# viswavi/speech-anonymization

Measured on AMD Instinct MI355X. Metric: audio frames/sec (node), ConvAE+gender-adv train step, higher is better.
Workload: dtype bf16x3; 1 GPU; ConvAE recon0.1+sex0.9 adversarial train step (L1 recon + NLL), shape M: 32 utt/GPU x 161120 samples (T=1008 frames), Fbank x2 + norm + fwd + bwd + clip + Adam + Noam; batch_per_gpu=32, frames_per_utt=1008, parallelism=dp1

## Files before the change

include/sa_hip.h:

```cpp
#ifndef SA_HIP_H
#define SA_HIP_H
#ifdef __cplusplus
extern "C" {
#endif

#define SA_F32 0
#define SA_BF16 1
#define SA_BF16X3 2
#define SA_BF16X1F 3
#define SA_FP8 4
#define SA_F64 5
#define SA_MAX_TAPS 5
#define SA_COMM_ID_BYTES 128

typedef struct SaTaps {
  int ntaps[2];
  int off[2][SA_MAX_TAPS];
  int widx[2][SA_MAX_TAPS];
} SaTaps;

typedef struct SaConvArgs {
  const void* x;
  const void* wp;
  const float* bias;
  void* y;
  const float* s1; const float* t1;
  const float* s2; const float* t2;
  int swish;
  int relu;
  float* stats;
  int B, Lin, Lout, ntiles;
  int rowmin, nrows, wlo_off;
  SaTaps taps;
  int ep_mode, ep_xp_is_act, ep_bstride;
  const void* ep_x; const void* ep_g2;
  const float* ep_s1; const float* ep_t1; const float* ep_mean; const float* ep_rstd;
  void* a_out;
  const void* nb_x; const float* nb_c1; const float* nb_c2; const float* nb_c3;
  int nb_bstride, nb_relu_mask; float* nb_colsum;
  const float* ep_g2k1; const float* ep_g2k2; const float* ep_g2k3;
  float* pro_stats;
  const float* wscale;
  int tile_rows; int pad2_;
} SaConvArgs;

int sa_conv_gemm(int dtype, int cin, int cout, int sa, int u, const SaConvArgs* a, void* stream);
int sa_abi_sizeof(int which);
int sa_conv_gemm_ntiles(int cin, int cout, int u, int Lout);
int sa_conv_gemm_ntiles_tm(int tile_rows, int u, int Lout);
int sa_conv_gemm_set_tile_rows(int rows);
int sa_conv_gemm_set_impl(int impl);
int sa_conv_gemm_route(int dtype, int cin, int cout, int sa, int u, const SaConvArgs* a);

int sa_pack_weights(int dtype, const float* src, void* dst, int ntaps, int K, int N, int sk, int sn,
                    int st, void* stream);

typedef struct SaPackDesc {
  const float* src; void* dst;
  int dtype, ntaps, K, N, sk, sn, st, pad_;
  float* scale;
} SaPackDesc;
int sa_pack_weights_multi(const SaPackDesc* descs, int n, int blocks_per_image, void* stream);
int sa_pack_scales_multi(const SaPackDesc* descs, int n, void* stream);

typedef struct SaWgradArgs {
  const void* x;
  const void* dy;
  float* slabs;
  const float* s1; const float* t1; const float* s2; const float* t2; int swish;
  int B, Lin, Ldy, Mrows, chunk, nchunk;
  int ntaps; int off[SA_MAX_TAPS]; int ph[SA_MAX_TAPS];
  int x_pre;
  int dy_pre;
} SaWgradArgs;

int sa_wgrad(int dtype, int cin, int cout, int sa, int u, const SaWgradArgs* a, void* stream);
int sa_wgrad_kw(int cin, int cout);
int sa_wgrad_reduce(const float* slabs, float* dst, int nslab, int ntaps, int cin, int cout, int sk,
                    int sn, int st, int accumulate, void* stream);
#define SA_WRED_MAX 8
typedef struct SaWredDesc {
  const float* slabs; float* dst;
  int nslab, ntaps, cin, cout, sk, sn, st, accumulate, vec, pad_;
} SaWredDesc;
typedef struct SaWredMulti { int n, pad_; SaWredDesc d[SA_WRED_MAX]; } SaWredMulti;
int sa_wgrad_reduce_multi(const SaWredMulti* m, void* stream);

int sa_conv1toC(int dtype, const float* x, const float* w, const float* bias, void* y, int B, int L,
                int flip, float* stats, const void* ep_x, const float* ep_s1, const float* ep_t1,
                const float* ep_mean, const float* ep_rstd, void* stream);
int sa_conv1toC_ntiles(int L);
int sa_convCto1(int dtype, const void* x, const float* w, const float* bias, float* y, int B, int L,
                const float* s1, const float* t1, int swish, int flip, void* stream);
int sa_wgrad1C(int dtype, const float* u, const void* v, float* slabs, int B, int L, int chunk,
               int flip, const float* s1, const float* t1, int swish, void* stream);
int sa_wgrad1C_nchunk(int L, int chunk);
int sa_bwd1C(int dtype, const float* u, const void* v, const float* w, void* g, float* stats, float* slabs,
             int B, int L, int chunk, int flip, const float* s1, const float* t1, const float* mean,
             const float* rstd, void* stream);
int sa_sum_slabs(const float* slabs, float* dst, int nslab, int n, int accumulate, void* stream);

typedef struct SaEwArgs {
  const void* g; const void* g2; const void* x; void* out;
  const float* s1; const float* t1;
  const float* mean; const float* rstd;
  const float* c1; const float* c2; const float* c3;
  int actbwd, xp_is_act, relu_mask, bstride;
  float* stats;
  int B, L, ntiles;
} SaEwArgs;

int sa_ew_stats(int dtype, int C, const SaEwArgs* a, void* stream);
int sa_ew_apply(int dtype, int C, const SaEwArgs* a, void* stream);
int sa_ew_ntiles(int L);
int sa_sum_partials(const float* slabs, double* dst, int nbatch, int nslab, int n, void* stream);
int sa_sum_rows_d(const double* src, double* dst, int R, int n, void* stream);
int sa_fin_in_fwd(const double* sums, int B, int C, int n, const float* gamma, const float* beta,
                  float eps, float* mean, float* rstd, float* scale, float* shift, void* stream);
int sa_fin_bn_fwd(const double* sums, int R, int C, double count, const float* gamma, const float* beta,
                  float eps, float momentum, float* run_mean, float* run_var, float* mean,
                  float* rstd, float* scale, float* shift, const double* count_dev, void* stream);
int sa_fin_bn_eval(int C, const float* gamma, const float* beta, float eps, const float* run_mean,
                   const float* run_var, float* mean, float* rstd, float* scale, float* shift,
                   void* stream);
int sa_fin_norm_bwd(const double* sums, const double* lsums, int R, int groups, int C, double n,
                    const float* gamma, const float* mean, const float* rstd, float sign, float* c1,
                    float* c2, float* c3, float* dgamma, float* dbeta, const double* n_dev,
                    void* stream);
int sa_fin_bias(const double* sums, int B, int C, int ncomp, float* db, void* stream);

#define SA_FLATS_MAX 4
typedef struct SaFlat { float* p; long long n; } SaFlat;
typedef struct SaFlats { int n, pad_; SaFlat f[SA_FLATS_MAX]; } SaFlats;
int sa_clip_grads(const SaFlats* f, float max_norm, float eps, double* partials, float* total_norm, void* stream);
#define SA_ADAM_CHUNK 1024
typedef struct SaAdamRec {
  float* p; float* m; float* v; const float* step; const float* g;
  long long goff, n;
  int gbase, pad_;
} SaAdamRec;
int sa_adam_record_bytes(void);
int sa_adam_step(const SaAdamRec* table, int ntensors, const int* map, int nblocks, const SaFlats* bases,
                 const float* lr_dev, double lr, double beta1, double beta2, double eps, void* stream);
#define SA_BIAS_MAX 8
typedef struct SaBiasDesc {
  const float* part; double* rows; float* db;
  int nbatch, nslab, C, ncomp;
} SaBiasDesc;
typedef struct SaBiasMulti { int n, pad_; SaBiasDesc d[SA_BIAS_MAX]; } SaBiasMulti;
int sa_bias_multi(const SaBiasMulti* m, void* stream);

int sa_pool_fwd(int dtype, const void* r, const float* scale, const float* shift, float* part, int B,
                int L, int nseg, void* stream);
int sa_pool_nseg(int B);
int sa_pool_gather(const float* part, int B, int nseg, int L, double* sums, void* stream);
int sa_pool_fin(const double* sums, int B, int n, const float* noise, float eps, float* pooled,
                float* mean, float* stdraw, void* stream);
int sa_pool_gather_fin(const float* part, int B, int nseg, int L, const float* noise, int raw, float eps,
                       float* pooled, float* mean, float* stdraw, void* stream);
int sa_pool_bwd(int dtype, const void* r, const float* scale, const float* shift,
                const float* dpooled, const float* mean, const float* stdraw, void* g, int B, int L,
                const float* bn_mean, const float* bn_rstd, float* stats, void* stream);
int sa_dense(const float* X, int lda, const float* ps, const float* pt, const float* W, int sbk,
             int sbn, const float* bias, float* Y, int ldy, int M, int N, int K, int relu,
             void* stream);
int sa_colsums(const float* X, const float* H, const float* hmean, const float* hrstd, int M, int N,
               double* sums, float* out0, float* out1, void* stream);
int sa_bn2d_bwd(const float* G, const float* H, const double* sums, double count, const float* gamma,
                const float* mean, const float* rstd, int relu_mask, int M, int N, float* dH,
                const double* count_dev, void* stream);
int sa_dense_wgrad(const float* dY, const float* X, const float* ps, const float* pt, int M, int N,
                   int K, float* dW, void* stream);
int sa_log_softmax(const float* X, float* Y, int M, int N, void* stream);
int sa_log_softmax_bwd(const float* dY, const float* Y, float* dX, int M, int N, void* stream);
int sa_loss_workspace_bytes(void);
int sa_recon_loss(const float* a, const float* b, long long n, int kind, float* grad, float* loss,
                  void* workspace, void* stream);
int sa_cls_losses(const float* logp, const long long* label, int B, int NC, float* out, float* dnll,
                  float* dconf, void* stream);
int sa_cosine_loss(const float* x1, const float* x2, int B, int S, int D, float* rowloss,
                   float* loss, float* dx1, void* stream);
int sa_recon_loss_part(const float* a, const float* b, long long n, int kind, float* grad, float gscale,
                       void* workspace, void* stream);
int sa_step_loss(const void* workspace, long long n, const float* logp, const long long* label, int B, int NC,
                 float w_recon, float w_sex, float* out, float* dlogp, int* nonfinite, void* stream);

int sa_head_fwd(const float* pooled, const float* w1, const float* b1, const float* g1, const float* be1,
                float* rm1, float* rv1, const float* w2, const float* b2, const float* g2, const float* be2,
                float* rm2, float* rv2, const float* w3, const float* b3, float* h1, float* f1, float* h2,
                float* f2, float* logp, int M, float eps, float momentum, void* stream);
int sa_head_bwd(const float* dlogp, const float* logp, const float* pooled, const float* h1, const float* f1,
                const float* h2, const float* f2, const float* w1, const float* g1, const float* w2,
                const float* g2, const float* w3, float* dw1, float* db1, float* dg1, float* dbe1, float* dw2,
                float* db2, float* dg2, float* dbe2, float* dw3, float* db3, float* dpooled, int M, void* stream);
int sa_head_bwd_wide(const float* dlogp, const float* logp, const float* pooled, const float* h1, const float* f1,
                     const float* h2, const float* f2, const float* w1, const float* g1, const float* w2,
                     const float* g2, const float* w3, float* dw1, float* db1, float* dg1, float* dbe1, float* dw2,
                     float* db2, float* dg2, float* dbe2, float* dw3, float* db3, float* dpooled, int M,
                     void* stream);
int sa_head_max_rows(void);

int sa_tdnn_fwd(const float* x, const void* wp, const float* bias, const float* bn_s, const float* bn_t,
                float* y, int B, int T, int Cin, int Cout, int Npad, int K, int dil, float slope,
                unsigned char* mask, void* stream);
int sa_time_pool(const float* x, const float* lens, const float* noise, int B, int T, int C, float eps,
                 float* out, void* stream);
int sa_leaky_affine(const float* x, const float* s, const float* t, float slope, int M, int C, float* y,
                    void* stream);
int sa_tdnn_bwd_input(const float* dy, const unsigned char* mask, const float* bn_s, const void* wp,
                      float* dxe, int B, int T, int Cy, int Cred, int Cin, int Npad, int K, int dil,
                      float slope, void* stream);
int sa_tdnn_fold(const float* dxe, float* dx, int B, int T, int C, int pad, void* stream);
int sa_time_pool_bwd(const float* x, const float* lens, const float* g, const float* pooled, int B,
                     int T, int C, float eps, float* dx, void* stream);
int sa_leaky_affine_bwd(const float* dy, const float* x, const float* s, float slope, int M, int C,
                        float* dx, void* stream);

int sa_xv_tdnn_fwd_train(const float* x, const float* s_in, const float* t_in, const void* wp, const float* bias,
                         float* z, float* part, int B, int T, int Cin, int Cout, int Npad, int K, int dil,
                         float slope, void* stream);
int sa_xv_tdnn_ntiles(int T);
int sa_xv_colsums(const float* G, const float* H, const float* hmean, const float* hrstd, const float* c1,
                  const float* c2, const float* c3, float slope, float* out, int M, int N, int rows_per,
                  double* part, void* stream);
int sa_xv_tdnn_wgrad(const float* dpre, const float* x, const float* s_in, const float* t_in, float* part, int B,
                     int T, int Cin, int Cout, int K, int dil, int nsplit, int rows_per, void* stream);
int sa_xv_wgrad_reduce(const float* part, int nsplit, int K, int Cout, int Cin, float* dW, void* stream);
int sa_xv_tdnn_dgrad(const float* dpre, const void* wp, float* dxe, int B, int T, int Cy, int Cred, int Cin,
                     int Npad, int K, int dil, void* stream);
int sa_xv_pool_affine(const float* pz, const float* s, const float* t, const float* noise, int B, int C,
                      float eps, float* pooled, void* stream);
int sa_xv_pool_affine_bwd(const float* g, const float* s, int B, int C, float* gz, void* stream);

int sa_fc_tiles(int T);
int sa_fc_groups(int B, int T);
int sa_fc_nparam(void);
int sa_fc_nhead(void);
int sa_fc_max_rows(void);
int sa_fc_enc_fwd(const float* feats, const void* const* wb, float* h1, float* h2, float* z, double* bnpart,
                  int B, int T, void* stream);
int sa_fc_bn_fin(const double* bnpart, int npart, const float* gamma, const float* beta, float* run_mean,
                 float* run_var, float* bnf, int B, int T, int train, float eps, float momentum, void* stream);
int sa_fc_mid_fwd(const float* z, const float* bnf, const void* const* wb, float* a1, float* u, float* d1,
                  float* d2, float* recon, double* poolpart, int B, int T, void* stream);
int sa_fc_recon_fwd(const float* feats, const void* const* wb, float* recon, int B, int T, void* stream);
int sa_fc_head_fwd(const double* poolpart, const float* noise, const void* const* hw, float* pooled, float* pst,
                   float* h1, float* f1, float* h2, float* h3, float* f2, float* logp, int B, int T, int train,
                   float eps, float momentum, void* stream);
int sa_fc_head_bwd(const float* dlogp, const float* logp, const float* pooled, const float* h1,
                   const float* h2, const float* h3, const void* const* hw, float* dhead,
                   float* dpooled, int B, int train, float eps, void* stream);
int sa_fc_mid_bwd(const float* d_recon, const float* dpooled, const float* pst, const float* z, const float* bnf,
                  const float* a1, const float* u, const float* d1, const float* d2, const void* const* wb,
                  float* dzn, float* dzdec, float* wpart, double* bnbpart, int B, int T, void* stream);
int sa_fc_bn_bwd_fin(const double* bnbpart, int npart, const float* gamma, const float* bnf, float* coef,
                     float* dgamma, float* dbeta, int B, int T, int train, void* stream);
int sa_fc_enc_bwd(const float* feats, const float* h1, const float* h2, const float* z, const float* dzn,
                  const float* dzdec, const float* coef, const void* const* wb, float* wpart, int B, int T,
                  void* stream);
int sa_fc_wreduce(const float* wpart, int G, float* grads, void* stream);

int sa_cluster_mi(const float* X, const long long* y, const long long* idx, int iters, int n, int D,
                  int ncls, int k, float* mi, void* stream);

int sa_fbank(const float* wav, int B, int N, const float* window, const void* dft,
             const void* mel, float* feats, float* tilemax, void* stream);
int sa_fbank_table_elems(int which);
int sa_fbank_ntiles(int T);
int sa_fbank_scratch_bytes(int B);
int sa_fbank_normalize(const float* feats, const float* tilemax, int B, int T, int Tp,
                       const float* lens, float top_db, int batch_max, int update, int epoch,
                       int update_until_epoch, float* state, float* scratch, float* out,
                       void* stream);
int sa_fbank_normalize_pair(const float* feats, const float* tilemax, int B, int T, int Tp,
                            const float* lens, float top_db, int batch_max, int update, int epoch,
                            int update_until_epoch, float* state, float* scratch, float* snap,
                            float* out1, float* out2, void* stream);

int sa_wav_augment_tile(void);
int sa_wav_augment_max_chunks(void);
int sa_wav_abs_sums(const float* wav, const float* noise, int B, int L, double* sums, void* stream);
int sa_noise_scales(const double* sums, const float* lens, const float* snr, int B, int L, float* scales,
                    void* stream);
int sa_wav_augment(const float* wav, const float* noise, const float* scales, const void* plan, int B, int L, int R,
                   int Lp, int S_in, int S_out, int W, int first_min, int first_max, float* out, void* stream);

int sa_specaug_warp_sums(const float* x, const void* plan, int B, int T, int F, float* out, double* part,
                         void* stream);
int sa_specaug_finalize(const double* part, const void* plan, int B, int T, int F, float* vals, void* stream);
int sa_specaug_fill(const void* plan, const float* vals, int B, int T, int F, float* out, void* stream);

int sa_gl_tile(void);
int sa_mel_to_mag(const float* x, const float* mean, const float* stdv, const float* M, int B, int T, int Tf,
                  float* S, void* stream);
int sa_gl_istft(const void* C, const float* window, const float* twiddle, int B, int T, float* y, void* stream);
int sa_gl_project(const float* y, const float* S, const void* Tprev, float momentum_ratio, const float* window,
                  const float* twiddle, int B, int T, void* C_new, void* R, void* stream);

int sa_yin_dim(int which);
int sa_yin_f0(const float* wav, int B, int N, float threshold, float* f0, float* dprime, void* stream);
int sa_pitch_ratio(const float* f0, const float* lens, int B, int T, int N, float target, float r_min, float r_max,
                   int min_voiced, float* ratio, float* mean, int* voiced, void* stream);
int sa_pitch_stretch_mag(const void* R, const float* ratio, int B, int T, int Tout, float* S, void* stream);
int sa_pitch_resample(const float* y, const float* ratio, const int* n_valid, int B, int Nin, int Nout, float* out,
                      void* stream);

int sa_env_dim(int which);
int sa_env_warp(const float* S, const float* q, int B, int T, int n_c, float floor_rel, float max_gain_ln,
                float* out, float* env, void* stream);

int sa_mcadams_dim(int which);
int sa_mcadams(const float* wav, const float* alpha, const int* n_valid, int B, int N, int level, float* out,
               void* ws, int* status, float* gain, void* stream);

int sa_stoi_dim(int which);
int sa_stoi(const float* ref, const float* deg, const int* n_valid, int B, int N, const double* taps,
            float* stoi, float* estoi, int* frames, int* segments, void* ws, void* stream);

int sa_pv_dim(int which);
long long sa_pv_workspace_bytes(int B, int Tout);
int sa_pv_synth(const void* R, const float* S, const float* ratio, int B, int T, int Tout, void* C, double* phase,
                void* ws, void* stream);

int sa_contour_dim(int which);
int sa_pitch_contour(const float* f0, const float* lens, int B, int T, int N, float target, float gamma, int smooth,
                     float r_min, float r_max, int min_voiced, int* rho_q, long long* Q, int* Tq, float* mean,
                     int* voiced, void* stream);
int sa_pv_synth_map(const void* R, const float* M, const int* rho_q, const long long* Q, int B, int T, int Tout,
                    void* C, double* phase, void* ws, void* stream);
int sa_env_warp_frames(const float* S, const float* q, int B, int T, int n_c, float floor_rel, float max_gain_ln,
                       float* out, float* env, void* stream);
int sa_pitch_resample_map(const float* y, const int* rho_q, const long long* Q, const int* n_valid, int B, int Nin,
                          int Nout, int T, float* out, void* stream);

int sa_f0v_dim(int which);
int sa_f0_candidates(const float* dprime, int B, int T, int* cand_tau, int* cand_q, void* stream);
int sa_f0_viterbi(const float* dprime, const int* cand_tau, const int* cand_q, const float* lens, const int* log_q,
                  int B, int T, int N, float voicing_cost, float switch_cost, float jump_cost, float lag_bias,
                  unsigned char* psi, int* path, float* f0, void* stream);

int sa_f0cmp_dim(int which);
int sa_f0_compare(const float* f0_ref, const float* f0_deg, const int* frames, int B, int T, int max_lag,
                  int min_common, float* rho, int* lag, int* common, float* shift_st, float* dev_st, float* voicing,
                  void* stream);

int sa_mcd_dim(int which);
int sa_mcd(const float* mel_ref, const float* mel_deg, const int* n_ref, const int* n_deg, int B, int T_ref, int T_deg,
           int n_mels, int order, int band, void* ws, float* mcd, float* mcd_sync, int* frames, void* stream);

int sa_psola_dim(int which);
long long sa_psola_workspace_bytes(int B, int N);
int sa_psola_marks(const float* wav, const float* f0, const int* n_valid, int B, int N, int T, int* marks, int* count,
                   void* stream);
int sa_psola_plan(const int* marks, const int* count, const float* f0, const int* rho_q, const int* n_valid, int B,
                  int N, int T, void* ws, int* syn_pos, int* syn_src, int* syn_count, void* stream);
int sa_psola_ola(const float* wav, const int* marks, const int* count, const int* syn_pos, const int* syn_src,
                 const int* syn_count, const int* n_valid, int B, int N, float* out, void* stream);

int sa_formant_dim(int which);
int sa_formant_tracks(const float* wav, const int* n_valid, int B, int N, float* freq, float* bw, int* status,
                      void* stream);
int sa_formant_compare(const float* F_ref, const float* F_deg, const int* st_ref, const int* st_deg,
                       const float* f0_ref, const float* f0_deg, const int* frames, int B, int T, int min_common,
                       float* med, float* ratio, float* shift, int* common, void* stream);

int sa_pole_warp_dim(int which);
int sa_pole_warp(const float* wav, const float* q, const int* n_valid, int B, int N, int level, float* out, void* ws,
                 int* status, float* gain, void* stream);
int sa_formant_centre(const float* freq, const int* status, const float* f0, const int* frames, int B, int T, float t1,
                      float t2, float t3, float q_min, float q_max, int min_frames, float* med, float* q, int* count,
                      void* stream);

int sa_srcfilt_dim(int which);
long long sa_srcfilt_workspace_bytes(int B, int N);
int sa_srcfilt_pulses(const float* f0, const int* rho_q, const int* n_valid, int B, int N, int T, long long* pos_q,
                      int* period_q, int* count, void* stream);
int sa_srcfilt_excite(const float* f0, const long long* pos_q, const int* period_q, const int* count, const int* seed,
                      const int* n_valid, int B, int N, int T, float aspiration, float* exc, void* stream);
int sa_srcfilt_synth(const float* wav, const float* exc, const int* n_valid, int B, int N, int level, float* out,
                     void* ws, int* status, float* gain, void* stream);

int sa_add_layernorm_fwd(const void* x, const void* r, const void* gamma, const void* beta, void* y, void* s_out,
                         float* stat, int rows, int d, float eps, void* stream);
int sa_layernorm_bwd(const void* dy, const void* s, const float* stat, const void* gamma, void* ds, int rows,
                     int d, void* stream);
int sa_ln_leaky_fwd(const void* x, const void* gamma, const void* beta, void* y, float* stat, int rows, int d,
                    float eps, float slope, void* stream);
int sa_ln_leaky_bwd(const void* dy, const void* x, const float* stat, const void* gamma, const void* beta, void* dx,
                    int rows, int d, float slope, void* stream);
int sa_asr_block0_fwd(const void* x, const void* w, const void* bias, const void* gamma, const void* beta, void* y,
                      float* stat, int B, int T, int F, int C, float eps, float slope, void* stream);
int sa_asr_block0_bwd(const void* dy, const void* x, const void* w, const void* bias, const void* gamma,
                      const void* beta, const float* stat, float* part, void* dx, int B, int T, int F, int C,
                      float slope, void* stream);
int sa_reflect_pad_fwd(const void* x, void* y, int B, int T, int F, int C, void* stream);
int sa_reflect_pad_bwd(const void* dy, void* dx, int B, int T, int F, int C, void* stream);

int sa_comm_unique_id(void* id128);
int sa_comm_init(int rank, int world, const void* id128, int device);
int sa_comm_world(void);
int sa_comm_allreduce(void* buf, long long n, int dtype, int avg, void* producer_stream);
int sa_comm_allreduce_inline(void* buf, long long n, int dtype, int avg, void* stream);
int sa_comm_join(void* consumer_stream);
int sa_comm_ncalls(void);
int sa_comm_destroy(void);

#ifdef __cplusplus
}
#endif
#endif
```

speech-anonymization_amd/_lib.py:

```python
import ctypes as C
import os

import torch

_HERE = os.path.dirname(os.path.abspath(__file__))
LIB_PATH = os.environ.get("SA_HIP_LIB") or os.path.join(_HERE, "libsa_hip.so")

F32, BF16, BF16X3, BF16X1F, FP8, F64 = 0, 1, 2, 3, 4, 5
MAX_TAPS = 5

c_fp = C.POINTER(C.c_float)
vp = C.c_void_p


class SaTaps(C.Structure):
    _fields_ = [("ntaps", C.c_int * 2), ("off", (C.c_int * MAX_TAPS) * 2),
                ("widx", (C.c_int * MAX_TAPS) * 2)]


class SaConvArgs(C.Structure):
    _fields_ = [("x", vp), ("wp", vp), ("bias", vp), ("y", vp),
                ("s1", vp), ("t1", vp), ("s2", vp), ("t2", vp),
                ("swish", C.c_int), ("relu", C.c_int), ("stats", vp),
                ("B", C.c_int), ("Lin", C.c_int), ("Lout", C.c_int), ("ntiles", C.c_int),
                ("rowmin", C.c_int), ("nrows", C.c_int), ("wlo_off", C.c_int), ("taps", SaTaps),
                ("ep_mode", C.c_int), ("ep_xp_is_act", C.c_int), ("ep_bstride", C.c_int),
                ("ep_x", vp), ("ep_g2", vp), ("ep_s1", vp), ("ep_t1", vp), ("ep_mean", vp), ("ep_rstd", vp),
                ("a_out", vp),
                ("nb_x", vp), ("nb_c1", vp), ("nb_c2", vp), ("nb_c3", vp),
                ("nb_bstride", C.c_int), ("nb_relu_mask", C.c_int), ("nb_colsum", vp),
                ("ep_g2k1", vp), ("ep_g2k2", vp), ("ep_g2k3", vp), ("pro_stats", vp), ("wscale", vp),
                ("tile_rows", C.c_int), ("pad2_", C.c_int)]


class SaPackDesc(C.Structure):
    _fields_ = [("src", vp), ("dst", vp), ("dtype", C.c_int), ("ntaps", C.c_int), ("K", C.c_int),
                ("N", C.c_int), ("sk", C.c_int), ("sn", C.c_int), ("st", C.c_int), ("pad_", C.c_int),
                ("scale", vp)]


class SaWgradArgs(C.Structure):
    _fields_ = [("x", vp), ("dy", vp), ("slabs", vp),
                ("s1", vp), ("t1", vp), ("s2", vp), ("t2", vp), ("swish", C.c_int),
                ("B", C.c_int), ("Lin", C.c_int), ("Ldy", C.c_int), ("Mrows", C.c_int),
                ("chunk", C.c_int), ("nchunk", C.c_int),
                ("ntaps", C.c_int), ("off", C.c_int * MAX_TAPS), ("ph", C.c_int * MAX_TAPS),
                ("x_pre", C.c_int), ("dy_pre", C.c_int)]


class SaEwArgs(C.Structure):
    _fields_ = [("g", vp), ("g2", vp), ("x", vp), ("out", vp),
                ("s1", vp), ("t1", vp), ("mean", vp), ("rstd", vp),
                ("c1", vp), ("c2", vp), ("c3", vp),
                ("actbwd", C.c_int), ("xp_is_act", C.c_int), ("relu_mask", C.c_int),
                ("bstride", C.c_int), ("stats", vp),
                ("B", C.c_int), ("L", C.c_int), ("ntiles", C.c_int)]


BIAS_MAX = 8


class SaBiasDesc(C.Structure):
    _fields_ = [("part", vp), ("rows", vp), ("db", vp),
                ("nbatch", C.c_int), ("nslab", C.c_int), ("C", C.c_int), ("ncomp", C.c_int)]


class SaBiasMulti(C.Structure):
    _fields_ = [("n", C.c_int), ("pad_", C.c_int), ("d", SaBiasDesc * BIAS_MAX)]


WRED_MAX = 8
FLATS_MAX = 4


class SaFlat(C.Structure):
    _fields_ = [("p", vp), ("n", C.c_longlong)]


class SaFlats(C.Structure):
    _fields_ = [("n", C.c_int), ("pad_", C.c_int), ("f", SaFlat * FLATS_MAX)]



class SaAdamRec(C.Structure):
    _fields_ = [("p", vp), ("m", vp), ("v", vp), ("step", vp), ("g", vp),
                ("goff", C.c_longlong), ("n", C.c_longlong), ("gbase", C.c_int), ("pad_", C.c_int)]


ADAM_CHUNK = 1024


class SaWredDesc(C.Structure):
    _fields_ = [("slabs", vp), ("dst", vp)] + [(k, C.c_int) for k in ("nslab", "ntaps", "cin", "cout", "sk", "sn", "st",
                                                                      "accumulate", "vec", "pad_")]


class SaWredMulti(C.Structure):
    _fields_ = [("n", C.c_int), ("pad_", C.c_int), ("d", SaWredDesc * WRED_MAX)]


SYMBOLS = [
    "sa_conv_gemm", "sa_abi_sizeof", "sa_conv_gemm_ntiles", "sa_conv_gemm_ntiles_tm", "sa_conv_gemm_set_tile_rows",
    "sa_conv_gemm_set_impl", "sa_conv_gemm_route", "sa_pack_weights", "sa_pack_weights_multi", "sa_pack_scales_multi", "sa_wgrad", "sa_wgrad_kw", "sa_wgrad_reduce",
    "sa_conv1toC", "sa_conv1toC_ntiles", "sa_convCto1", "sa_wgrad1C", "sa_wgrad1C_nchunk", "sa_bwd1C",
    "sa_sum_slabs", "sa_ew_stats", "sa_ew_apply", "sa_ew_ntiles",
    "sa_sum_partials", "sa_sum_rows_d", "sa_fin_in_fwd", "sa_fin_bn_fwd", "sa_fin_bn_eval", "sa_fin_norm_bwd", "sa_fin_bias",
    "sa_pool_fwd", "sa_pool_nseg", "sa_pool_gather", "sa_pool_fin", "sa_pool_gather_fin", "sa_pool_bwd", "sa_dense", "sa_colsums",
    "sa_bn2d_bwd", "sa_dense_wgrad", "sa_log_softmax", "sa_log_softmax_bwd",
    "sa_loss_workspace_bytes", "sa_recon_loss", "sa_cls_losses", "sa_cosine_loss", "sa_recon_loss_part", "sa_step_loss",
    "sa_tdnn_fwd", "sa_time_pool", "sa_leaky_affine", "sa_tdnn_bwd_input", "sa_tdnn_fold", "sa_time_pool_bwd",
    "sa_leaky_affine_bwd", "sa_cluster_mi", "sa_fbank", "sa_fbank_table_elems", "sa_fbank_ntiles", "sa_fbank_scratch_bytes", "sa_fbank_normalize", "sa_fbank_normalize_pair",
    "sa_comm_unique_id", "sa_comm_init", "sa_comm_world", "sa_comm_allreduce", "sa_comm_allreduce_inline", "sa_comm_join", "sa_comm_ncalls",
    "sa_comm_destroy", "sa_head_fwd", "sa_head_bwd", "sa_head_bwd_wide", "sa_head_max_rows",
    "sa_add_layernorm_fwd", "sa_layernorm_bwd", "sa_reflect_pad_fwd", "sa_reflect_pad_bwd", "sa_ln_leaky_fwd", "sa_ln_leaky_bwd", "sa_bias_multi", "sa_asr_block0_fwd", "sa_asr_block0_bwd", "sa_wgrad_reduce_multi", "sa_clip_grads",
    "sa_adam_record_bytes", "sa_adam_step",
    "sa_xv_tdnn_fwd_train", "sa_xv_tdnn_ntiles", "sa_xv_colsums", "sa_xv_tdnn_wgrad", "sa_xv_wgrad_reduce",
    "sa_xv_tdnn_dgrad", "sa_xv_pool_affine", "sa_xv_pool_affine_bwd",
    "sa_fc_tiles", "sa_fc_groups", "sa_fc_nparam", "sa_fc_nhead", "sa_fc_max_rows", "sa_fc_enc_fwd", "sa_fc_bn_fin",
    "sa_fc_mid_fwd", "sa_fc_head_fwd", "sa_fc_head_bwd", "sa_fc_mid_bwd", "sa_fc_bn_bwd_fin", "sa_fc_enc_bwd",
    "sa_fc_wreduce", "sa_fc_recon_fwd",
    "sa_wav_augment_tile", "sa_wav_augment_max_chunks", "sa_wav_abs_sums", "sa_noise_scales", "sa_wav_augment",
    "sa_specaug_warp_sums", "sa_specaug_finalize", "sa_specaug_fill",
    "sa_gl_tile", "sa_mel_to_mag", "sa_gl_istft", "sa_gl_project",
    "sa_yin_dim", "sa_yin_f0", "sa_pitch_ratio", "sa_pitch_stretch_mag", "sa_pitch_resample",
    "sa_env_dim", "sa_env_warp",
    "sa_mcadams_dim", "sa_mcadams",
    "sa_stoi_dim", "sa_stoi",
    "sa_pv_dim", "sa_pv_synth",
    "sa_contour_dim", "sa_pitch_contour", "sa_pv_synth_map", "sa_env_warp_frames", "sa_pitch_resample_map",
    "sa_f0v_dim", "sa_f0_candidates", "sa_f0_viterbi",
    "sa_f0cmp_dim", "sa_f0_compare",
    "sa_mcd_dim", "sa_mcd",
    "sa_psola_dim", "sa_psola_marks", "sa_psola_plan", "sa_psola_ola",
    "sa_formant_dim", "sa_formant_tracks", "sa_formant_compare",
    "sa_pole_warp_dim", "sa_pole_warp", "sa_formant_centre",
    "sa_srcfilt_dim", "sa_srcfilt_pulses", "sa_srcfilt_excite", "sa_srcfilt_synth",
]

_lib = None


class SaHipError(RuntimeError):
    pass


def load():
    global _lib
    if _lib is None:
        if not os.path.exists(LIB_PATH):
            raise SaHipError(
                f"{LIB_PATH} not found: build it with `python -c 'import __graft_entry__ as g; "
                "g.build()'` (hipcc --offload-arch=gfx950). There is no CPU fallback.")
        _lib = C.CDLL(LIB_PATH)
        for s in SYMBOLS:
            getattr(_lib, s).restype = C.c_int
        _lib.sa_pv_workspace_bytes.restype = C.c_longlong
        _lib.sa_psola_workspace_bytes.restype = C.c_longlong
        _lib.sa_srcfilt_workspace_bytes.restype = C.c_longlong
        for i, rec in enumerate((SaConvArgs, SaWgradArgs, SaEwArgs, SaPackDesc, SaTaps, SaBiasMulti, SaWredMulti, SaFlats)):
            if _lib.sa_abi_sizeof(i) != C.sizeof(rec):
                raise SaHipError(f"{rec.__name__}: binding has {C.sizeof(rec)} bytes, {LIB_PATH} "
                                 f"{_lib.sa_abi_sizeof(i)} -- rebuild the library (stale build?)")
        if _lib.sa_adam_record_bytes() != C.sizeof(SaAdamRec):
            raise SaHipError(f"SaAdamRec: binding has {C.sizeof(SaAdamRec)} bytes, {LIB_PATH} "
                             f"{_lib.sa_adam_record_bytes()} -- rebuild the library (stale build?)")
    return _lib


def stream():
    return C.c_void_p(torch._C._cuda_getCurrentRawStream(torch._C._cuda_getDevice()))


def ptr(t):
    if t is None:
        return None
    assert t.is_cuda and t.is_contiguous(), "HIP kernels take contiguous device tensors"
    return C.c_void_p(t.data_ptr())


def check(rc, what):
    if rc != 0:
        raise SaHipError(f"{what} failed with code {rc}")


def dt_code(dtype):
    if dtype == torch.float32:
        return F32
    if dtype == torch.bfloat16:
        return BF16
    raise SaHipError(f"unsupported activation dtype {dtype}")


_taps_cache = {}


def make_taps(phases):
    key = tuple(tuple(p) for p in phases)
    t = _taps_cache.get(key)
    if t is not None:
        return t
    t = _taps_cache[key] = SaTaps()
    for ph, lst in enumerate(phases):
        t.ntaps[ph] = len(lst)
        for i, (off, wi) in enumerate(lst):
            t.off[ph][i] = off
            t.widx[ph][i] = wi
    return t
```

speech-anonymization_amd/convae.py:

```python
import functools
import os

import torch
import torch.nn as nn

from . import distributed as sdist
from . import ops
from . import _lib as L
from ._lib import SaHipError


class _ParamOnly(nn.Module):

    def forward(self, x):
        raise SaHipError("parameter container only; use ConvAutoencoder.forward")


class GLU(_ParamOnly):
    pass


class StatisticsPooling(_ParamOnly):
    pass


class TDNNSexClassifier(nn.Module):
    def __init__(self, num_classes=2):
        super().__init__()
        self.tdnn = nn.Sequential(
            nn.Conv1d(128, 128, kernel_size=5, dilation=1), nn.ReLU(), nn.BatchNorm1d(128),
            nn.Conv1d(128, 128, kernel_size=3, dilation=2), nn.ReLU(), nn.BatchNorm1d(128),
            nn.Conv1d(128, 128, kernel_size=3, dilation=3), nn.ReLU(), nn.BatchNorm1d(128),
        )
        self.norm = nn.BatchNorm1d(128)
        self.stats_pooling = StatisticsPooling()
        self.classify = nn.Sequential(
            nn.Linear(256, 128), nn.ReLU(), nn.BatchNorm1d(128),
            nn.Linear(128, 64), nn.ReLU(), nn.BatchNorm1d(64),
            nn.Linear(64, num_classes),
        )

    def forward(self, x):
        raise SaHipError("parameter container only; use ConvAutoencoder.forward")


class ConvAutoencoder(nn.Module):
    def __init__(self, precision="bf16x3", pooling_noise=True, sync_bn=True, dtype=None,
                 cache_wgrad_operand=True):
        super().__init__()
        if dtype is not None:
            precision = {torch.float32: "f32", torch.bfloat16: "bf16"}[dtype]
        if precision not in ops.PRECISIONS:
            raise SaHipError(f"unknown precision {precision!r}")
        self.precision = precision
        self.encoder = nn.Sequential(
            nn.Conv1d(1, 32, 15, 1, 7), GLU(),
            nn.Conv1d(32, 64, 5, 2, 2), nn.InstanceNorm1d(64, affine=True), GLU(),
            nn.Conv1d(64, 64, 5, 1, 2), nn.InstanceNorm1d(64, affine=True), GLU(),
            nn.Conv1d(64, 128, 5, 2, 2), nn.InstanceNorm1d(128, affine=True), GLU(),
            nn.Conv1d(128, 128, 5, 1, 2), nn.InstanceNorm1d(128, affine=True), GLU(),
        )
        self.decoder = nn.Sequential(
            nn.Conv1d(128, 128, 5, 1, 2),
            nn.ConvTranspose1d(128, 64, 5, 2, 2, output_padding=1),
            nn.InstanceNorm1d(64, affine=True), GLU(),
            nn.Conv1d(64, 64, 5, 1, 2),
            nn.ConvTranspose1d(64, 32, 5, 2, 2, output_padding=1),
            nn.InstanceNorm1d(32, affine=True), GLU(),
            nn.Conv1d(32, 1, 15, 1, 7),
        )
        self.sex_classifier = TDNNSexClassifier(2)
        self.lay = ops.conv_layers(self, ("encoder", "sex_classifier.tdnn", "decoder"))
        self.pack_plan = [(ly.key, ly.kinds[i]) for i in (0, 1)
                          for ly in sorted(self.lay.values(), key=lambda ly: ly.transposed)]
        self.act_dtype, self.kcode = ops.PRECISIONS[precision]
        self.dgrad_kcode = ops.DGRAD_CODE[precision]
        self.cache_wgrad_operand = cache_wgrad_operand
        self.pooling_noise = pooling_noise
        self.sync_bn = sync_bn
        self.fused_head = os.environ.get("SA_FUSED_HEAD", "1") == "1"
        self.fused_bwd1c = os.environ.get("SA_FUSED_BWD1C", "1") == "1"
        self.fused_pool_fin = os.environ.get("SA_FUSED_POOL_FIN", "1") == "1"
        self.wide_head_bwd = os.environ.get("SA_WIDE_HEAD_BWD", "1") == "1"
        self.dp_batch_sizes = None

    def forward(self, feats):
        names, params = self._named_params()
        return _ConvAEFn.apply(self, names, feats, *params)

    def _named_params(self):
        c = self.__dict__.get("_np_cache")
        if c is None or any(o[n] is not p for o, n, p in c[2]):
            names, params, owners = [], [], []
            for mname, mod in self.named_modules():
                for pname, p in mod._parameters.items():
                    if p is not None:
                        names.append(f"{mname}.{pname}" if mname else pname)
                        params.append(p)
                        owners.append((mod._parameters, pname, p))
            c = self.__dict__["_np_cache"] = (tuple(names), tuple(params), owners)
        return c[0], c[1]

    @torch.no_grad()
    def reconstruct(self, feats):
        if not torch.is_tensor(feats) or feats.dim() != 3:
            raise SaHipError("ConvAutoencoder expects feats [B, T, 80]")
        x0, B, T, Ltot = _input_rows(feats)
        P = dict(zip(*self._named_params()))
        cg, inorm = _launchers(self, P, _packed(self, P), B)
        y, _, _ = _encoder_launches(self, P, cg, inorm, x0, Ltot, False)
        return _decoder_launches(self, P, cg, inorm, y[5], Ltot)[-1].view(B, T, 80)

    def _side_stream(self, device):
        if getattr(self, "_side", None) is None and device.type == "cuda":
            self._side = torch.cuda.Stream(device=device)
        return getattr(self, "_side", None)

    def _bn_syncs(self):
        return self.sync_bn and sdist.dp_active()

    def _bn_allreduce(self, sums):
        if self._bn_syncs():
            sdist.all_reduce_now(sums)
            return sdist.world_size()
        return 1

    def _bn_global_counts(self, counts, device):
        if not self._bn_syncs():
            return None
        key = (tuple(counts), str(device))
        cache = self.__dict__.setdefault("_count_cache", {})
        local = cache.get(key)
        if local is None:
            if len(cache) > 64:
                cache.clear()
            local = cache[key] = torch.tensor(counts, dtype=torch.float64).to(device)
        g = local.clone()
        sdist.all_reduce_now(g)
        return g

    def _bn_rows(self):
        return not self._bn_syncs()

    def _bn_global(self, local_sums):
        if not self._bn_syncs():
            return local_sums, 1
        g = local_sums.clone()
        return g, self._bn_allreduce(g)

    def _head_plan(self, B):
        if not self._bn_syncs() or self.dp_batch_sizes is None:
            return None
        W, r = sdist.world_size(), sdist.rank()
        sizes = [B] * W if isinstance(self.dp_batch_sizes, str) else [int(b) for b in self.dp_batch_sizes]
        if self.dp_batch_sizes != "equal" and isinstance(self.dp_batch_sizes, str):
            raise SaHipError(f"dp_batch_sizes: 'equal', a list of per-rank batch sizes or None, not {self.dp_batch_sizes!r}")
        if len(sizes) != W or sizes[r] != B:
            raise SaHipError(f"dp_batch_sizes {sizes} does not describe rank {r} of {W} holding {B} utterances")
        return sum(sizes[:r]), sum(sizes), W

    @staticmethod
    def _gather_rows(x, plan):
        off, Bg, _ = plan
        g = torch.zeros(Bg, x.shape[1], device=x.device, dtype=x.dtype)
        g[off:off + x.shape[0]].copy_(x)
        sdist.all_reduce_now(g)
        return g


class _W:
    __slots__ = ("img", "code")

    def __init__(self, img, code):
        self.img, self.code = img, code


def _kcode(model, kind):
    return model.dgrad_kcode if kind.endswith("dgrad") else model.kcode


def _packed(model, P):
    items = [((k, kind), P[k], kind, _kcode(model, kind)) for k, kind in model.pack_plan]
    key = tuple(w.data_ptr() for _, w, _, _ in items) + tuple(c for _, _, _, c in items)
    pk = getattr(model, "_pack_cache", None)
    if pk is None or pk[0] != key:
        pk = (key, ops.PackedWeights(items, model.act_dtype))
        model._pack_cache = pk
    pk[1].refresh()
    return {tag: _W(img, code) for tag, (img, code) in pk[1].images.items()}


def _conv(x, w, *args, **kw):
    return ops.conv_gemm(x, w.img, *args, code=w.code, **kw)


class _PendingApply:
    __slots__ = ("g", "y", "c", "per_c", "relu", "bias_key", "wgrads")

    def __init__(self, g, y, c, per_c, relu, bias_key):
        self.g, self.y, self.c, self.per_c, self.relu, self.bias_key = g, y, c, per_c, relu, bias_key
        self.wgrads = []


def _noise(model, B, device):
    return ops.pooling_noise(model.pooling_noise, B, 128, device)


def _input_rows(feats):
    B, T, Fd = feats.shape
    Ltot = T * Fd
    if Fd != 80 or Ltot % 4:
        raise SaHipError("ConvAutoencoder expects feats [B, T, 80] with T*80 divisible by 4")
    if not feats.is_cuda:
        raise SaHipError("ConvAutoencoder runs on the GPU only (no CPU fallback)")
    return feats.detach().reshape(B, Ltot).contiguous().float(), B, T, Ltot


def _in_ep(y, nrm, g2=None):
    mean, rstd, scale, shift = nrm
    d = dict(mode=1, x=y, g2=g2, s1=scale, t1=shift, mean=mean, rstd=rstd)
    if isinstance(g2, _PendingApply):
        d.update(g2=g2.g, g2k=g2.c)
    return d


def _launchers(model, P, W, B, A=None):
    def cg(ly, x, **kw):
        if A is not None and P[ly.key].requires_grad:
            A[ly.key] = kw["a_out"] = torch.empty(x.shape, dtype=torch.bfloat16, device=x.device)
        return _conv(x, W[ly.key, ly.kinds[0]], P[ly.bias], *ly.fwd(x.shape[1]), **kw)

    def inorm(stats, n, prefix, C):
        sums = ops.sum_partials(stats, B)
        return ops.fin_in_fwd(sums, B, C, n, P[prefix + ".weight"], P[prefix + ".bias"])
    return cg, inorm


def _encoder_launches(model, P, cg, inorm, x0, Ltot, want_pro_stats):
    L2, L4, lay = Ltot // 2, Ltot // 4, model.lay
    y0 = ops.conv1toC(x0, P["encoder.0.weight"], P["encoder.0.bias"], model.act_dtype)
    y1, st = cg(lay["encoder.2"], y0, swish=True, want_stats=True)
    n1 = inorm(st, L2, "encoder.3", 64)
    y2, st = cg(lay["encoder.5"], y1, s1=n1[2], t1=n1[3], swish=True, want_stats=True)
    n2 = inorm(st, L2, "encoder.6", 64)
    y3, st = cg(lay["encoder.8"], y2, s1=n2[2], t1=n2[3], swish=True, want_stats=True)
    n3 = inorm(st, L4, "encoder.9", 128)
    y4, st = cg(lay["encoder.11"], y3, s1=n3[2], t1=n3[3], swish=True, want_stats=True)
    n4 = inorm(st, L4, "encoder.12", 128)
    y5 = cg(lay["decoder.0"], y4, s1=n4[2], t1=n4[3], swish=True, want_pro_stats=want_pro_stats)
    a4_stats = None
    if want_pro_stats:
        y5, a4_stats = y5
    return [y0, y1, y2, y3, y4, y5], [n1, n2, n3, n4], a4_stats


def _decoder_launches(model, P, cg, inorm, y5, Ltot):
    L2, lay = Ltot // 2, model.lay
    y6, st = cg(lay["decoder.1"], y5, want_stats=True)
    n6 = inorm(st, L2, "decoder.2", 64)
    y7 = cg(lay["decoder.4"], y6, s1=n6[2], t1=n6[3], swish=True)
    y8, st = cg(lay["decoder.5"], y7, want_stats=True)
    n8 = inorm(st, Ltot, "decoder.6", 32)
    recon = ops.convCto1(y8, P["decoder.8.weight"], P["decoder.8.bias"], n8[2], n8[3], True)
    return y6, n6, y7, y8, n8, recon


class _ConvAEFn(torch.autograd.Function):
    @staticmethod
    def forward(ctx, model, names, feats, *params):
        ctx.set_materialize_grads(False)
        P = dict(zip(names, params))
        train = model.training
        x0, B, T, Ltot = _input_rows(feats)
        L2, L4 = Ltot // 2, Ltot // 4
        S = {}
        W, lay = _packed(model, P), model.lay
        A = {}
        cache_a = (train and model.cache_wgrad_operand and any(ctx.needs_input_grad)
                   and ops.WGRAD_CODE[model.precision] in (L.BF16X1F, L.BF16) and model.kcode != L.FP8)

        cg, inorm = _launchers(model, P, W, B, A if cache_a else None)

        def bn_stats(stats, count, mod, prefix, C, ci):
            sums = ops.sum_partials(stats, 1, rows=model._bn_rows()) if train else None
            return bnorm(sums, count, mod, prefix, C, ci)

        def bnorm(sums, count, mod, prefix, C, ci, local=False):
            if not train:
                return ops.fin_bn_eval(C, P[prefix + ".weight"], P[prefix + ".bias"],
                                       mod.running_mean, mod.running_var)
            if not local:
                model._bn_allreduce(sums)
            out = ops.fin_bn_fwd(sums, C, count, P[prefix + ".weight"], P[prefix + ".bias"],
                                 mod.running_mean, mod.running_var, count_dev=None if local else cdev(ci))
            tracked.append(mod.num_batches_tracked)
            return out

        tracked = []
        enc, dec, cls = model.encoder, model.decoder, model.sex_classifier
        La, Lb, Lc = L4 - 4, L4 - 8, L4 - 14
        gc = model._bn_global_counts([B * L4, B * La, B * Lb, B * Lc, B, B], feats.device) if train else None
        cdev = lambda i: None if gc is None else gc[i:i + 1]
        (y0, y1, y2, y3, y4, y5), (n1, n2, n3, n4), a4_stats = _encoder_launches(model, P, cg, inorm, x0, Ltot, train)
        bn_n = bn_stats(a4_stats if train else None, B * L4, cls.norm, "sex_classifier.norm", 128, 0)
        r0, st = cg(lay["sex_classifier.tdnn.0"], y4, s1=n4[2], t1=n4[3], swish=True, s2=bn_n[2], t2=bn_n[3],
                    relu=True, want_stats=True)
        bn0 = bn_stats(st, B * La, cls.tdnn[2], "sex_classifier.tdnn.2", 128, 1)
        r1, st = cg(lay["sex_classifier.tdnn.3"], r0, s2=bn0[2], t2=bn0[3], relu=True, want_stats=True)
        bn1 = bn_stats(st, B * Lb, cls.tdnn[5], "sex_classifier.tdnn.5", 128, 2)
        r2, st = cg(lay["sex_classifier.tdnn.6"], r1, s2=bn1[2], t2=bn1[3], relu=True, want_stats=True)
        bn2 = bn_stats(st, B * Lc, cls.tdnn[8], "sex_classifier.tdnn.8", 128, 3)
        if model.fused_pool_fin:
            nz, raw = ops.pooling_noise_raw(model.pooling_noise, B, 128, feats.device)
            pooled, pmean, psd = ops.pool_fwd(r2, bn2[2], bn2[3], noise=nz, fused=True, raw=raw)
        else:
            pooled, pmean, psd = ops.pool_fwd(r2, bn2[2], bn2[3], noise=_noise(model, B, feats.device))
        def head_fwd(X, n, local=False):
            H1 = ops.dense(X, P["sex_classifier.classify.0.weight"], P["sex_classifier.classify.0.bias"],
                           128, 256, relu=True)
            f1 = bnorm(ops.colsums(H1) if train else None, n, cls.classify[2], "sex_classifier.classify.2", 128, 4, local)
            H2 = ops.dense(H1, P["sex_classifier.classify.3.weight"], P["sex_classifier.classify.3.bias"],
                           64, 128, ps=f1[2], pt=f1[3], relu=True)
            f2 = bnorm(ops.colsums(H2) if train else None, n, cls.classify[5], "sex_classifier.classify.5", 64, 5, local)
            logits = ops.dense(H2, P["sex_classifier.classify.6.weight"], P["sex_classifier.classify.6.bias"],
                               2, 64, ps=f2[2], pt=f2[3])
            return H1, f1, H2, f2, ops.log_softmax(logits)

        plan = model._head_plan(B) if train else None
        head_in, Bh = (model._gather_rows(pooled, plan), plan[1]) if plan else (pooled, B)
        fused_head = (train and model.fused_head and (plan is not None or not model._bn_syncs())
                      and Bh <= ops.head_max_rows())
        clsP = {k[len("sex_classifier.classify."):]: v for k, v in P.items() if k.startswith("sex_classifier.classify.")}
        if fused_head:
            H1, f1, H2, f2, logp = ops.head_fwd(head_in, clsP, cls.classify[2], cls.classify[5])
            tracked += [cls.classify[2].num_batches_tracked, cls.classify[5].num_batches_tracked]
        else:
            H1, f1, H2, f2, logp = head_fwd(head_in, Bh, plan is not None)
        logp_all = logp
        if plan:
            logp = logp_all[plan[0]:plan[0] + B]
        if tracked:
            torch._foreach_add_(tracked, 1)
        y6, n6, y7, y8, n8, recon = _decoder_launches(model, P, cg, inorm, y5, Ltot)

        S.update(x0=x0, y=[y0, y1, y2, y3, y4, y5, y6, y7, y8], r=[r0, r1, r2],
                 n=[None, n1, n2, n3, n4, None, n6, None, n8], bn=[bn_n, bn0, bn1, bn2], f=[f1, f2],
                 pooled=head_in, pmean=pmean, psd=psd, H1=H1, H2=H2, logp=logp_all, head_plan=plan,
                 dims=(B, T, Ltot, L2, L4, La, Lb, Lc), train=train, W=W, A=A, gc=gc, fused_head=fused_head)
        ctx.S, ctx.model, ctx.names, ctx.params = S, model, names, params
        ctx.need_input_grad = feats.requires_grad
        return recon.view(B, T, 80), logp

    @staticmethod
    def backward(ctx, d_recon, d_logp):
        S, model, names = ctx.S, ctx.model, ctx.names
        if S is None:
            raise SaHipError("ConvAutoencoder backward called twice (saved tensors were released)")
        P = dict(zip(names, ctx.params))
        dt = model.act_dtype
        B, T, Ltot, L2, L4, La, Lb, Lc = S["dims"]
        if not S["train"]:
            raise SaHipError("backward through eval-mode BatchNorm is not implemented")
        y0, y1, y2, y3, y4, y5, y6, y7, y8 = S["y"]
        r0, r1, r2 = S["r"]
        n1, n2, n3, n4, n6, n8 = S["n"][1], S["n"][2], S["n"][3], S["n"][4], S["n"][6], S["n"][8]
        bn_n, bn0, bn1, bn2 = S["bn"]
        f1, f2 = S["f"]
        dev = y0.device
        G = {k: None for k in names}
        need = {k: p.requires_grad for k, p in P.items()}
        need_stage = {st: any(v for k, v in need.items() if k.startswith(st))
                      for st in sdist.StageBuckets.STAGES}
        run_encoder = need_stage["encoder"] or ctx.need_input_grad
        run_decoder = need_stage["decoder"] or run_encoder
        model._last_flats = None
        buckets = sdist.StageBuckets(list(P.items()), dev, model._side_stream(dev))
        newg = buckets.view

        def setg(key, val):
            G[key] = newg(key).copy_(val.reshape(P[key].shape))
        W, A, lay = S["W"], S["A"], model.lay
        gc = S["gc"]
        cdev = lambda i: None if gc is None else gc[i:i + 1]
        pending_wred = []
        wg = functools.partial(ops.wgrad, code=ops.WGRAD_CODE[model.precision], defer=pending_wred)
        fuse = bool(A) and model.dgrad_kcode in (L.BF16X3, L.BF16)

        def cg(ly, gin, **kw):
            p, dy = gin, gin.g if isinstance(gin, _PendingApply) else gin
            w, args = W[ly.key, ly.kinds[1]], (None,) + ly.dgrad(ly.lin(dy.shape[1]))
            if dy is gin:
                return _conv(dy, w, *args, **kw)
            dyc = torch.empty(p.g.shape, dtype=torch.bfloat16, device=p.g.device) if p.wgrads else None
            want_cs = p.bias_key is not None and need[p.bias_key]
            out = _conv(p.g, w, *args, a_out=dyc, nb=dict(x=p.y, c1=p.c[0], c2=p.c[1], c3=p.c[2],
                                                           per_c=p.per_c, relu_mask=p.relu,
                                                           want_colsum=want_cs), **kw)
            if want_cs:
                cs = out[-1]
                out = out[:-1] if len(out) > 2 else out[0]
                nb_, _, cc_ = cs.shape
                G[p.bias_key] = newg(p.bias_key)
                pending_bias.append((cs, nb_, cc_, 1, G[p.bias_key]))
            for f in p.wgrads:
                f(dyc)
            p.wgrads = []
            return out

        def bias_from(stats, key, C):
            if need[key]:
                G[key] = newg(key)
                pending_bias.append((stats, B, C, 2, G[key]))

        pending_bias = []

        def flush_pending():
            if pending_bias:
                ops.bias_multi(pending_bias)
                pending_bias.clear()
            if pending_wred:
                ops.wgrad_reduce_multi(pending_wred)
                pending_wred.clear()

        def in_finish(g, st, y, nrm, C, Ln, prefix, bias_key):
            mean, rstd = nrm[0], nrm[1]
            dg, db = newg(prefix + ".weight"), newg(prefix + ".bias")
            sums = ops.sum_partials(st, B)
            c1, c2, c3 = ops.fin_norm_bwd(sums, sums, B * C, C, Ln, P[prefix + ".weight"], mean, rstd,
                                          dgamma=dg, dbeta=db)
            G[prefix + ".weight"], G[prefix + ".bias"] = dg, db
            if fuse:
                return _PendingApply(g, y, (c1, c2, c3), False, False, bias_key)
            st2 = ops.ew("apply", g, y, C, out=g, c1=c1, c2=c2, c3=c3)
            bias_from(st2, bias_key, C)
            return g

        def bn_ep(r, bn, xp=None):
            d = dict(mode=2, x=r, mean=bn[0], rstd=bn[1], per_c=True)
            if xp:
                d.update(s1=xp[0], t1=xp[1], xp_is_act=True)
            return d

        def bn_finish(g, st, r, bn, Ln, prefix, bias_key, ci, xp=None):
            mean, rstd = bn[0], bn[1]
            kw = dict(s1=xp[0], t1=xp[1], xp_is_act=True) if xp else {}
            dg, db = newg(prefix + ".weight"), newg(prefix + ".bias")
            lsums = ops.sum_partials(st, 1, rows=model._bn_rows())
            gsums, _ = model._bn_global(lsums)
            c1, c2, c3 = ops.fin_norm_bwd(gsums, lsums, 128, 128, float(B * Ln), P[prefix + ".weight"],
                                          mean, rstd, sign=-1.0 if xp else 1.0, dgamma=dg, dbeta=db,
                                          n_dev=cdev(ci))
            G[prefix + ".weight"], G[prefix + ".bias"] = dg, db
            if fuse:
                return _PendingApply(g, r, (c1, c2, c3), True, not xp, bias_key)
            st2 = ops.ew("apply", g, r, 128, out=g, c1=c1, c2=c2, c3=c3, relu_mask=not xp, per_c=True,
                         want_stats=bias_key is not None, **kw)
            if bias_key:
                bias_from(st2, bias_key, 128)
            return g

        def conv_wgrad(ly, x, dy, **pro):
            key = ly.key
            if not need[key]:
                return
            if isinstance(dy, _PendingApply):
                dy.wgrads.append(lambda dyc: conv_wgrad(ly, x, dyc, dy_pre=True))
                return
            if key in A:
                x, pro = A[key], dict(x_pre=True, dy_pre=bool(pro.get("dy_pre")))
            *geo, strides = ly.wgrad(x.shape[1])
            G[key] = wg(x, dy, *geo, newg(key), strides, **pro)

        recon_unused = d_recon is None
        if recon_unused:
            for k in need:
                if k.startswith("decoder"):
                    need[k] = False
            need_stage["decoder"] = False
        if d_logp is None:
            d_logp = torch.zeros(B, 2, device=dev)

        def finish(d_feats=None):
            flush_pending()
            buckets.join()
            ctx.S = None
            model._last_flats = [buckets.flat[st] for st in sdist.StageBuckets.STAGES if need_stage[st]]
            grads = tuple(G[k] if need[k] else None for k in names)
            G.clear()
            buckets.views.clear()
            return (None, None, d_feats) + grads

        def head_bwd():
            c = "sex_classifier.classify."
            plan = S.get("head_plan")
            dlp, Bh = d_logp.contiguous().float(), B
            if plan:
                dlp, Bh = model._gather_rows(dlp, plan), plan[1]
            dP = head_bwd_rows(c, dlp, Bh, plan is not None)
            if plan:
                hg = [G[k] for k in names if k.startswith(c) and k in G]
                if plan[2] > 1 and hg:
                    torch._foreach_mul_(hg, 1.0 / plan[2])
                dP = dP[plan[0]:plan[0] + B]
            return dP

        def head_bwd_rows(c, dlp, n, local):
            if S.get("fused_head"):
                short = ("0.weight", "0.bias", "2.weight", "2.bias", "3.weight", "3.bias", "5.weight", "5.bias",
                         "6.weight", "6.bias")
                views = {}
                for k in short:
                    if need[c + k]:
                        views[k] = G[c + k] = newg(c + k)
                clsP = {k: P[c + k] for k in short}
                return ops.head_bwd(dlp, S["logp"], S["pooled"], S["H1"], f1, S["H2"], f2, clsP, views,
                                    wide=model.wide_head_bwd)
            glob = (lambda l: l) if local else (lambda l: model._bn_global(l)[0])
            cd = (lambda i: None) if local else cdev
            dLG = ops.log_softmax_bwd(dlp, S["logp"])
            H1, H2 = S["H1"], S["H2"]
            G[c + "6.weight"] = ops.dense_wgrad(dLG, H2, newg(c + "6.weight"), ps=f2[2], pt=f2[3])
            G[c + "6.bias"] = newg(c + "6.bias"); ops.colsums(dLG, out0=G[c + "6.bias"])
            dN2 = ops.dense(dLG, P[c + "6.weight"], None, 64, 2, transpose_w=True)
            G[c + "5.weight"], G[c + "5.bias"] = newg(c + "5.weight"), newg(c + "5.bias")
            l2 = ops.colsums(dN2, H2, f2[0], f2[1], out0=G[c + "5.bias"], out1=G[c + "5.weight"])
            dH2 = ops.bn2d_bwd(dN2, H2, glob(l2), n, P[c + "5.weight"], f2[0], f2[1], True, count_dev=cd(5))
            G[c + "3.weight"] = ops.dense_wgrad(dH2, H1, newg(c + "3.weight"), ps=f1[2], pt=f1[3])
            G[c + "3.bias"] = newg(c + "3.bias"); ops.colsums(dH2, out0=G[c + "3.bias"])
            dN1 = ops.dense(dH2, P[c + "3.weight"], None, 128, 64, transpose_w=True)
            G[c + "2.weight"], G[c + "2.bias"] = newg(c + "2.weight"), newg(c + "2.bias")
            l1 = ops.colsums(dN1, H1, f1[0], f1[1], out0=G[c + "2.bias"], out1=G[c + "2.weight"])
            dH1 = ops.bn2d_bwd(dN1, H1, glob(l1), n, P[c + "2.weight"], f1[0], f1[1], True, count_dev=cd(4))
            G[c + "0.weight"] = ops.dense_wgrad(dH1, S["pooled"], newg(c + "0.weight"))
            G[c + "0.bias"] = newg(c + "0.bias"); ops.colsums(dH1, out0=G[c + "0.bias"])
            return ops.dense(dH1, P[c + "0.weight"], None, 256, 128, transpose_w=True)

        def tdnn_bwd(dP):
            t = "sex_classifier.tdnn."
            g, st = ops.pool_bwd(r2, bn2[2], bn2[3], dP, S["pmean"], S["psd"], bn=(bn2[0], bn2[1]))
            g = bn_finish(g, st, r2, bn2, Lc, t + "8", t + "6.bias", 3)
            conv_wgrad(lay[t + "6"], r1, g, s2=bn1[2], t2=bn1[3])
            g, st = cg(lay[t + "6"], g, want_stats=True, ep=bn_ep(r1, bn1))
            g = bn_finish(g, st, r1, bn1, Lb, t + "5", t + "3.bias", 2)
            conv_wgrad(lay[t + "3"], r0, g, s2=bn0[2], t2=bn0[3])
            g, st = cg(lay[t + "3"], g, want_stats=True, ep=bn_ep(r0, bn0))
            g = bn_finish(g, st, r0, bn0, La, t + "2", t + "0.bias", 1)
            conv_wgrad(lay[t + "0"], y4, g, s1=n4[2], t1=n4[3], swish=True, s2=bn_n[2], t2=bn_n[3])
            xp4 = (n4[2], n4[3])
            g, st = cg(lay[t + "0"], g, want_stats=True, ep=bn_ep(y4, bn_n, xp4))
            da = bn_finish(g, st, y4, bn_n, L4, "sex_classifier.norm", None, 0, xp=xp4)
            flush_pending()
            if need_stage["sex_classifier"]:
                buckets.reduce_stage("sex_classifier")
            return da

        def decoder_bwd():
            d_rec = torch.zeros(B, T, 80, device=dev) if recon_unused else d_recon
            g_rec = d_rec.reshape(B, Ltot).contiguous().float()
            if need["decoder.8.bias"]:
                setg("decoder.8.bias", ops.sum_partials(g_rec.view(4 * B, Ltot // 4), 1, n=Ltot // 4).sum())
            if need["decoder.8.weight"] and model.fused_bwd1c:
                g, st, G["decoder.8.weight"] = ops.bwd1C(g_rec, y8, P["decoder.8.weight"], newg("decoder.8.weight"),
                                                         n8[2], n8[3], n8[0], n8[1])
            else:
                if need["decoder.8.weight"]:
                    G["decoder.8.weight"] = ops.wgrad1C(g_rec, y8, newg("decoder.8.weight"), flip=True,
                                                        s1=n8[2], t1=n8[3], swish=True)
                g, st = ops.conv1toC(g_rec, P["decoder.8.weight"], None, dt, flip=True, want_stats=True,
                                     ep=dict(x=y8, s1=n8[2], t1=n8[3], mean=n8[0], rstd=n8[1]))
            g = in_finish(g, st, y8, n8, 32, Ltot, "decoder.6", "decoder.5.bias")
            conv_wgrad(lay["decoder.5"], y7, g)
            g, st = cg(lay["decoder.5"], g, want_stats=True)
            bias_from(st, "decoder.4.bias", 64)
            conv_wgrad(lay["decoder.4"], y6, g, s1=n6[2], t1=n6[3], swish=True)
            g, st = cg(lay["decoder.4"], g, want_stats=True, ep=_in_ep(y6, n6))
            g = in_finish(g, st, y6, n6, 64, L2, "decoder.2", "decoder.1.bias")
            conv_wgrad(lay["decoder.1"], y5, g)
            g, st = cg(lay["decoder.1"], g, want_stats=True)
            bias_from(st, "decoder.0.bias", 128)
            conv_wgrad(lay["decoder.0"], y4, g, s1=n4[2], t1=n4[3], swish=True)
            flush_pending()
            if need_stage["decoder"]:
                buckets.reduce_stage("decoder")
            return g

        da4_cls = tdnn_bwd(head_bwd())
        if not run_decoder:
            return finish()
        g = decoder_bwd()
        if not run_encoder:
            return finish()

        g, st = cg(lay["decoder.0"], g, want_stats=True, ep=_in_ep(y4, n4, g2=da4_cls))
        for conv, norm, y, nrm, x, nx in (("encoder.11", "encoder.12", y4, n4, y3, n3),
                                          ("encoder.8", "encoder.9", y3, n3, y2, n2),
                                          ("encoder.5", "encoder.6", y2, n2, y1, n1),
                                          ("encoder.2", "encoder.3", y1, n1, y0, None)):
            ly = lay[conv]
            g = in_finish(g, st, y, nrm, ly.cout, y.shape[1], norm, ly.bias)
            conv_wgrad(ly, x, g, swish=True, **(dict(s1=nx[2], t1=nx[3]) if nx else {}))
            g, st = cg(ly, g, want_stats=True, ep=_in_ep(x, nx) if nx else dict(mode=1, x=x))
        bias_from(st, "encoder.0.bias", 32)
        if need["encoder.0.weight"]:
            G["encoder.0.weight"] = ops.wgrad1C(S["x0"], g, newg("encoder.0.weight"))
        d_feats = None
        if ctx.need_input_grad:
            d_feats = ops.convCto1(g, P["encoder.0.weight"], None, flip=True).view(B, T, 80)
        flush_pending()
        if need_stage["encoder"]:
            buckets.reduce_stage("encoder")
        return finish(d_feats)
```

speech-anonymization_amd/csrc/sa_common.h:

```cpp
#pragma once
#include <hip/hip_runtime.h>
#include <stdint.h>
#include "../../include/sa_hip.h"

typedef __bf16 bf16_t;
typedef __bf16 bf16x8 __attribute__((ext_vector_type(8)));
typedef float f32x16 __attribute__((ext_vector_type(16)));
typedef float f32x4 __attribute__((ext_vector_type(4)));

#define SA_WAVE 64


template <typename T> struct Tr;

template <> struct Tr<float> {
  static constexpr int VEC = 4;
  static constexpr int KS = 2;
  typedef float Frag;
  __device__ static inline void unpack(const uint4& u, float* f) {
    f[0] = __uint_as_float(u.x); f[1] = __uint_as_float(u.y);
    f[2] = __uint_as_float(u.z); f[3] = __uint_as_float(u.w);
  }
  __device__ static inline uint4 pack(const float* f) {
    return make_uint4(__float_as_uint(f[0]), __float_as_uint(f[1]),
                      __float_as_uint(f[2]), __float_as_uint(f[3]));
  }
  __device__ static inline float to_f(float v) { return v; }
  __device__ static inline float from_f(float v) { return v; }
  __device__ static inline f32x16 mfma(Frag a, Frag b, f32x16 c) {
    return __builtin_amdgcn_mfma_f32_32x32x2f32(a, b, c, 0, 0, 0);
  }
};

__device__ static inline uint32_t sa_pack_bf16x2(float lo, float hi) {
  union { bf16_t b[2]; uint32_t u; } cv;
  cv.b[0] = (bf16_t)lo; cv.b[1] = (bf16_t)hi;
  return cv.u;
}

template <> struct Tr<bf16_t> {
  static constexpr int VEC = 8;
  static constexpr int KS = 16;
  typedef bf16x8 Frag;
  __device__ static inline void unpack(const uint4& u, float* f) {
    f[0] = __uint_as_float(u.x << 16); f[1] = __uint_as_float(u.x & 0xffff0000u);
    f[2] = __uint_as_float(u.y << 16); f[3] = __uint_as_float(u.y & 0xffff0000u);
    f[4] = __uint_as_float(u.z << 16); f[5] = __uint_as_float(u.z & 0xffff0000u);
    f[6] = __uint_as_float(u.w << 16); f[7] = __uint_as_float(u.w & 0xffff0000u);
  }
  __device__ static inline uint4 pack(const float* f) {
    return make_uint4(sa_pack_bf16x2(f[0], f[1]), sa_pack_bf16x2(f[2], f[3]),
                      sa_pack_bf16x2(f[4], f[5]), sa_pack_bf16x2(f[6], f[7]));
  }
  __device__ static inline float to_f(bf16_t v) { return (float)v; }
  __device__ static inline bf16_t from_f(float v) { return (bf16_t)v; }
  __device__ static inline f32x16 mfma(Frag a, Frag b, f32x16 c) {
    return __builtin_amdgcn_mfma_f32_32x32x16_bf16(a, b, c, 0, 0, 0);
  }
};

__device__ static inline float sa_swish(float v) { return v * __builtin_amdgcn_rcpf(1.0f + __expf(-v)); }
__device__ static inline float sa_swish_grad(float v) {
  const float s = __builtin_amdgcn_rcpf(1.0f + __builtin_amdgcn_exp2f(v * -1.4426950408889634f));
  const float t = 1.0f - s;
  const float u = fmaf(v, t, 1.0f);
  return s * u;
}

__device__ static inline int sa_acc_row(int reg, int lane) {
  return (reg & 3) + 8 * (reg >> 2) + 4 * (lane >> 5);
}

__device__ static inline float sa_wave_sum(float v) {
#pragma unroll
  for (int o = 32; o > 0; o >>= 1) v += __shfl_xor(v, o, 64);
  return v;
}
__device__ static inline double sa_wave_sum_d(double v) {
#pragma unroll
  for (int o = 32; o > 0; o >>= 1) v += __shfl_xor(v, o, 64);
  return v;
}
__device__ static inline float sa_wave_max(float v) {
#pragma unroll
  for (int o = 32; o > 0; o >>= 1) v = fmaxf(v, __shfl_xor(v, o, 64));
  return v;
}

static inline int sa_div_up(int a, int b) { return (a + b - 1) / b; }

struct bf16x3_t {};
struct bf16x1f_t {};

struct fp8_t {};
typedef long fp8x8;

template <typename T> struct Pol;
template <> struct Pol<float> {
  typedef float store_t; typedef float lds_t; typedef float Frag;
  static constexpr int NPL = 1, VEC = 4, KS = 2, PAD = 1;
};
template <> struct Pol<bf16_t> {
  typedef bf16_t store_t; typedef bf16_t lds_t; typedef bf16x8 Frag;
  static constexpr int NPL = 1, VEC = 8, KS = 16, PAD = 8;
};
template <> struct Pol<bf16x1f_t> {
  typedef float store_t; typedef bf16_t lds_t; typedef bf16x8 Frag;
  static constexpr int NPL = 1, VEC = 4, KS = 16, PAD = 8;
};
template <> struct Pol<bf16x3_t> {
  typedef float store_t; typedef bf16_t lds_t; typedef bf16x8 Frag;
  static constexpr int NPL = 2, VEC = 4, KS = 16, PAD = 8;
};

template <> struct Pol<fp8_t> {
  typedef bf16_t store_t; typedef unsigned char lds_t; typedef fp8x8 Frag;
  static constexpr int NPL = 1, VEC = 8, KS = 16, PAD = 8;
};
template <> struct Tr<unsigned char> {
  __device__ static inline f32x16 mfma(fp8x8 a, fp8x8 b, f32x16 c) {
    return __builtin_amdgcn_mfma_f32_32x32x16_fp8_fp8(a, b, c, 0, 0, 0);
  }
};
__device__ static inline uint2 sa_pack_fp8x8(const float* f) {
  float c[8];
#pragma unroll
  for (int j = 0; j < 8; ++j) c[j] = __builtin_amdgcn_fmed3f(f[j], -448.0f, 448.0f);
  int lo = 0, hi = 0;
  lo = __builtin_amdgcn_cvt_pk_fp8_f32(c[0], c[1], lo, false);
  lo = __builtin_amdgcn_cvt_pk_fp8_f32(c[2], c[3], lo, true);
  hi = __builtin_amdgcn_cvt_pk_fp8_f32(c[4], c[5], hi, false);
  hi = __builtin_amdgcn_cvt_pk_fp8_f32(c[6], c[7], hi, true);
  return make_uint2((unsigned)lo, (unsigned)hi);
}

__device__ static inline uint2 sa_pack_bf16x4(const float* f) {
  return make_uint2(sa_pack_bf16x2(f[0], f[1]), sa_pack_bf16x2(f[2], f[3]));
}
__device__ static inline void sa_split4(const float* f, uint2& hi, uint2& lo) {
  float h[4], l[4];
#pragma unroll
  for (int j = 0; j < 4; ++j) {
    const bf16_t hb = (bf16_t)f[j];
    h[j] = (float)hb;
    l[j] = f[j] - h[j];
  }
  hi = sa_pack_bf16x4(h);
  lo = sa_pack_bf16x4(l);
}
```

speech-anonymization_amd/csrc/sa_elementwise.hip:

```cpp
#include "sa_common.h"


#define SA_EW_ROWS 256

template <typename T, int C, bool APPLY>
__global__ __launch_bounds__(256) void sa_ew_kernel(SaEwArgs a) {
  typedef Tr<T> tr;
  constexpr int VEC = tr::VEC, CH = C / VEC, RPP = 256 / CH;
  __shared__ float red[RPP][C][2];
  const int tid = threadIdx.x, b = blockIdx.y, tile = blockIdx.x;
  const int c = tid % CH, r0 = tid / CH;
  const size_t cb1 = (size_t)b * C + c * VEC;
  const size_t cbn = (size_t)b * a.bstride + c * VEC;
  float s1[VEC], t1[VEC], mu[VEC], rs[VEC], k1[VEC], k2[VEC], k3[VEC], acc0[VEC], acc1[VEC];
#pragma unroll
  for (int j = 0; j < VEC; ++j) {
    s1[j] = a.s1 ? a.s1[cb1 + j] : 1.0f;
    t1[j] = a.t1 ? a.t1[cb1 + j] : 0.0f;
    mu[j] = a.mean ? a.mean[cbn + j] : 0.0f;
    rs[j] = a.rstd ? a.rstd[cbn + j] : 1.0f;
    k1[j] = (APPLY && a.c1) ? a.c1[cbn + j] : 1.0f;
    k2[j] = (APPLY && a.c2) ? a.c2[cbn + j] : 0.0f;
    k3[j] = (APPLY && a.c3) ? a.c3[cbn + j] : 0.0f;
    acc0[j] = 0.0f; acc1[j] = 0.0f;
  }
  const size_t base = (size_t)b * a.L * C + c * VEC;
  const T* gp = reinterpret_cast<const T*>(a.g) + base;
  const T* g2p = a.g2 ? reinterpret_cast<const T*>(a.g2) + base : nullptr;
  const T* xp = reinterpret_cast<const T*>(a.x) + base;
  T* op = a.out ? reinterpret_cast<T*>(a.out) + base : nullptr;
  const int lbeg = tile * SA_EW_ROWS;
  for (int r = r0; r < SA_EW_ROWS; r += RPP) {
    const int l = lbeg + r;
    if (l >= a.L) break;
    float g[VEC], x[VEC], o[VEC];
    tr::unpack(*reinterpret_cast<const uint4*>(gp + (size_t)l * C), g);
    tr::unpack(*reinterpret_cast<const uint4*>(xp + (size_t)l * C), x);
    if (g2p) {
      float g2[VEC];
      tr::unpack(*reinterpret_cast<const uint4*>(g2p + (size_t)l * C), g2);
#pragma unroll
      for (int j = 0; j < VEC; ++j) g[j] += g2[j];
    }
#pragma unroll
    for (int j = 0; j < VEC; ++j) {
      const float z = fmaf(x[j], s1[j], t1[j]);
      const float xv = a.xp_is_act ? sa_swish(z) : x[j];
      if (APPLY) {
        float v = fmaf(k1[j], g[j], fmaf(k2[j], xv, k3[j]));
        if (a.relu_mask && !(x[j] > 0.0f)) v = 0.0f;
        o[j] = v;
      } else {
        o[j] = a.actbwd ? g[j] * sa_swish_grad(z) : g[j];
      }
    }
    uint4 u = tr::pack(o);
    if (op) *reinterpret_cast<uint4*>(op + (size_t)l * C) = u;
    if (a.stats) {
      tr::unpack(u, o);
#pragma unroll
      for (int j = 0; j < VEC; ++j) {
        acc0[j] += o[j];
        if (!APPLY) {
          const float z = fmaf(x[j], s1[j], t1[j]);
          const float xv = a.xp_is_act ? sa_swish(z) : x[j];
          acc1[j] = fmaf(o[j], (xv - mu[j]) * rs[j], acc1[j]);
        }
      }
    }
  }
  if (a.stats) {
#pragma unroll
    for (int j = 0; j < VEC; ++j) { red[r0][c * VEC + j][0] = acc0[j]; red[r0][c * VEC + j][1] = acc1[j]; }
    __syncthreads();
    if (tid < C) {
      float s = 0.f, q = 0.f;
      for (int r = 0; r < RPP; ++r) { s += red[r][tid][0]; q += red[r][tid][1]; }
      float* d = a.stats + (((size_t)b * a.ntiles + tile) * C + tid) * 2;
      d[0] = s; d[1] = q;
    }
  }
}

extern "C" int sa_ew_ntiles(int L) { return sa_div_up(L, SA_EW_ROWS); }

template <bool APPLY>
static int launch_ew(int dtype, int C, const SaEwArgs& a0, hipStream_t st) {
  SaEwArgs a = a0;
  a.ntiles = sa_div_up(a.L, SA_EW_ROWS);
  dim3 grid(a.ntiles, a.B);
#define SA_EW_CASE(CC)                                                                      \
  if (C == CC) {                                                                            \
    if (dtype == SA_BF16) hipLaunchKernelGGL((sa_ew_kernel<bf16_t, CC, APPLY>), grid, dim3(256), 0, st, a); \
    else hipLaunchKernelGGL((sa_ew_kernel<float, CC, APPLY>), grid, dim3(256), 0, st, a);   \
    hipError_t e = hipGetLastError();                                                       \
    return e == hipSuccess ? 0 : -(int)e;                                                   \
  }
  SA_EW_CASE(32) SA_EW_CASE(64) SA_EW_CASE(128)
  return -38;
}

extern "C" int sa_ew_stats(int dtype, int C, const SaEwArgs* a, void* stream) {
  if (!a || !a->g || !a->x || a->B <= 0 || a->L <= 0) return -22;
  return launch_ew<false>(dtype, C, *a, reinterpret_cast<hipStream_t>(stream));
}
extern "C" int sa_ew_apply(int dtype, int C, const SaEwArgs* a, void* stream) {
  if (!a || !a->g || !a->x || !a->out || a->B <= 0 || a->L <= 0) return -22;
  return launch_ew<true>(dtype, C, *a, reinterpret_cast<hipStream_t>(stream));
}

#define SA_SP_LANES 16
__global__ __launch_bounds__(32 * SA_SP_LANES) void sa_sum_partials_kernel(const float* __restrict__ slabs,
                                                                           double* __restrict__ dst,
                                                                           int nslab, int n) {
  __shared__ double part[SA_SP_LANES][33];
  const int bb = blockIdx.y, o = threadIdx.x & 31, q = threadIdx.x >> 5;
  const int i = blockIdx.x * 32 + o;
  double s = 0.0;
  if (i < n) {
    const float* p = slabs + (size_t)bb * nslab * n + i;
#pragma unroll 16
    for (int k = q; k < nslab; k += SA_SP_LANES) s += (double)p[(size_t)k * n];
  }
  part[q][o] = s;
  __syncthreads();
  if (q == 0 && i < n) {
    double t = 0.0;
#pragma unroll
    for (int r = 0; r < SA_SP_LANES; ++r) t += part[r][o];
    dst[(size_t)bb * n + i] = t;
  }
}

extern "C" int sa_sum_partials(const float* slabs, double* dst, int nbatch, int nslab, int n,
                               void* stream) {
  if (!slabs || !dst || nbatch <= 0 || nslab <= 0 || n <= 0) return -22;
  hipLaunchKernelGGL(sa_sum_partials_kernel, dim3(sa_div_up(n, 32), nbatch), dim3(32 * SA_SP_LANES), 0,
                     reinterpret_cast<hipStream_t>(stream), slabs, dst, nslab, n);
  hipError_t e = hipGetLastError();
  return e == hipSuccess ? 0 : -(int)e;
}

__global__ void sa_sum_rows_d_kernel(const double* __restrict__ src, double* __restrict__ dst, int R, int n) {
  const int i = blockIdx.x * blockDim.x + threadIdx.x;
  if (i >= n) return;
  double s = 0.0;
#pragma unroll 8
  for (int r = 0; r < R; ++r) s += src[(size_t)r * n + i];
  dst[i] = s;
}

extern "C" int sa_sum_rows_d(const double* src, double* dst, int R, int n, void* stream) {
  if (!src || !dst || R <= 0 || n <= 0) return -22;
  hipLaunchKernelGGL(sa_sum_rows_d_kernel, dim3(sa_div_up(n, 128)), dim3(128), 0,
                     reinterpret_cast<hipStream_t>(stream), src, dst, R, n);
  hipError_t e = hipGetLastError();
  return e == hipSuccess ? 0 : -(int)e;
}

__global__ void sa_fin_in_fwd_kernel(const double* __restrict__ sums, int BC, int C, float n,
                                     const float* __restrict__ gamma, const float* __restrict__ beta,
                                     float eps, float* mean, float* rstd, float* scale, float* shift) {
  const int i = blockIdx.x * blockDim.x + threadIdx.x;
  if (i >= BC) return;
  const double m = (double)sums[2 * i] / n;
  double var = (double)sums[2 * i + 1] / n - m * m;
  if (var < 0.0) var = 0.0;
  const float r = (float)(1.0 / sqrt(var + (double)eps));
  const float sc = gamma[i % C] * r;
  mean[i] = (float)m; rstd[i] = r; scale[i] = sc; shift[i] = beta[i % C] - (float)m * sc;
}

extern "C" int sa_fin_in_fwd(const double* sums, int B, int C, int n, const float* gamma,
                             const float* beta, float eps, float* mean, float* rstd, float* scale,
                             float* shift, void* stream) {
  if (!sums || !gamma || !beta || !mean || !rstd || !scale || !shift) return -22;
  hipLaunchKernelGGL(sa_fin_in_fwd_kernel, dim3(sa_div_up(B * C, 256)), dim3(256), 0,
                     reinterpret_cast<hipStream_t>(stream), sums, B * C, C, (float)n, gamma, beta,
                     eps, mean, rstd, scale, shift);
  hipError_t e = hipGetLastError();
  return e == hipSuccess ? 0 : -(int)e;
}

__global__ void sa_fin_bn_fwd_kernel(const double* __restrict__ sums, int R, int C, double count,
                                     const float* __restrict__ gamma, const float* __restrict__ beta,
                                     float eps, float momentum, float* run_mean, float* run_var,
                                     float* mean, float* rstd, float* scale, float* shift,
                                     const double* __restrict__ count_dev) {
  const int i = blockIdx.x * blockDim.x + threadIdx.x;
  if (i >= C) return;
  if (count_dev) count = *count_dev;
  double S = 0.0, Q = 0.0;
#pragma unroll 8
  for (int r = 0; r < R; ++r) { S += sums[2 * ((size_t)r * C + i)]; Q += sums[2 * ((size_t)r * C + i) + 1]; }
  const double m = S / count;
  double var = Q / count - m * m;
  if (var < 0.0) var = 0.0;
  const float r = (float)(1.0 / sqrt(var + (double)eps));
  const float sc = gamma[i] * r;
  mean[i] = (float)m; rstd[i] = r; scale[i] = sc; shift[i] = beta[i] - (float)m * sc;
  if (run_mean) {
    const double unb = count > 1.0 ? var * count / (count - 1.0) : var;
    run_mean[i] = (1.0f - momentum) * run_mean[i] + momentum * (float)m;
    run_var[i] = (1.0f - momentum) * run_var[i] + momentum * (float)unb;
  }
}

extern "C" int sa_fin_bn_fwd(const double* sums, int R, int C, double count, const float* gamma,
                             const float* beta, float eps, float momentum, float* run_mean,
                             float* run_var, float* mean, float* rstd, float* scale, float* shift,
                             const double* count_dev, void* stream) {
  if (!sums || !gamma || !beta || !mean || !rstd || !scale || !shift || (!count_dev && count <= 0) || R < 1) return -22;
  hipLaunchKernelGGL(sa_fin_bn_fwd_kernel, dim3(sa_div_up(C, 128)), dim3(128), 0,
                     reinterpret_cast<hipStream_t>(stream), sums, R, C, count, gamma, beta, eps,
                     momentum, run_mean, run_var, mean, rstd, scale, shift, count_dev);
  hipError_t e = hipGetLastError();
  return e == hipSuccess ? 0 : -(int)e;
}

__global__ void sa_fin_bn_eval_kernel(int C, const float* __restrict__ gamma, const float* __restrict__ beta,
                                      float eps, const float* __restrict__ rm, const float* __restrict__ rv,
                                      float* mean, float* rstd, float* scale, float* shift) {
  const int i = blockIdx.x * blockDim.x + threadIdx.x;
  if (i >= C) return;
  const float r = 1.0f / sqrtf(rv[i] + eps), sc = gamma[i] * r;
  mean[i] = rm[i]; rstd[i] = r; scale[i] = sc; shift[i] = beta[i] - rm[i] * sc;
}

extern "C" int sa_fin_bn_eval(int C, const float* gamma, const float* beta, float eps,
                              const float* run_mean, const float* run_var, float* mean, float* rstd,
                              float* scale, float* shift, void* stream) {
  if (!gamma || !beta || !run_mean || !run_var || !mean || !rstd || !scale || !shift) return -22;
  hipLaunchKernelGGL(sa_fin_bn_eval_kernel, dim3(sa_div_up(C, 128)), dim3(128), 0,
                     reinterpret_cast<hipStream_t>(stream), C, gamma, beta, eps, run_mean, run_var,
                     mean, rstd, scale, shift);
  hipError_t e = hipGetLastError();
  return e == hipSuccess ? 0 : -(int)e;
}

__global__ void sa_fin_norm_bwd_kernel(const double* __restrict__ sums, const double* __restrict__ lsums,
                                       int R, int G, int C, double n, const float* __restrict__ gamma,
                                       const float* __restrict__ mean, const float* __restrict__ rstd,
                                       float sign, float* c1, float* c2, float* c3, float* dgamma,
                                       float* dbeta, int nb, int coef_blocks,
                                       const double* __restrict__ n_dev) {
  if (n_dev) n = *n_dev;
  if ((int)blockIdx.x < coef_blocks) {
    const int i = blockIdx.x * blockDim.x + threadIdx.x;
    if (i < G) {
      double S1 = 0.0, S2 = 0.0;
#pragma unroll 8
      for (int r = 0; r < R; ++r) { S1 += sums[2 * ((size_t)r * G + i)]; S2 += sums[2 * ((size_t)r * G + i) + 1]; }
      const double r = rstd[i], m = mean[i];
      const double k1 = (double)gamma[i % C] * r;
      c1[i] = sign * (float)k1;
      c2[i] = sign * (float)(-k1 * r * S2 / n);
      c3[i] = sign * (float)(k1 * (-S1 / n + m * r * S2 / n));
    }
    return;
  }
  __shared__ double part[8][32][2];
  const int ch = ((int)blockIdx.x - coef_blocks) * 32 + (threadIdx.x & 31), q = threadIdx.x >> 5;
  double a = 0.0, bsum = 0.0;
  if (ch < C) {
    const int tot = R * nb;
#pragma unroll 4
    for (int e = q; e < tot; e += 8) {
      const int r = e / nb, b = e % nb;
      const size_t at = 2 * ((size_t)r * G + (size_t)b * C + ch);
      bsum += lsums[at]; a += lsums[at + 1];
    }
  }
  part[q][threadIdx.x & 31][0] = bsum; part[q][threadIdx.x & 31][1] = a;
  __syncthreads();
  if (q == 0 && ch < C) {
    double s0 = 0.0, s1 = 0.0;
#pragma unroll
    for (int k = 0; k < 8; ++k) { s0 += part[k][threadIdx.x][0]; s1 += part[k][threadIdx.x][1]; }
    dbeta[ch] = (float)s0; dgamma[ch] = (float)s1;
  }
}

extern "C" int sa_fin_norm_bwd(const double* sums, const double* lsums, int R, int groups, int C, double n,
                               const float* gamma, const float* mean, const float* rstd, float sign,
                               float* c1, float* c2, float* c3, float* dgamma, float* dbeta,
                               const double* n_dev, void* stream) {
  if (!sums || !gamma || !mean || !rstd || !c1 || !c2 || !c3 || groups % C || R < 1) return -22;
  if ((dgamma == nullptr) != (dbeta == nullptr)) return -22;
  const int coef_blocks = sa_div_up(groups, 256);
  const int grid = coef_blocks + (dgamma ? sa_div_up(C, 32) : 0);
  hipLaunchKernelGGL(sa_fin_norm_bwd_kernel, dim3(grid), dim3(256), 0,
                     reinterpret_cast<hipStream_t>(stream), sums, lsums ? lsums : sums, R, groups, C,
                     n, gamma, mean, rstd, sign, c1, c2, c3, dgamma, dbeta, groups / C, coef_blocks, n_dev);
  hipError_t e = hipGetLastError();
  return e == hipSuccess ? 0 : -(int)e;
}

__global__ void sa_fin_bias_kernel(const double* __restrict__ sums, int B, int C, int ncomp, float* db) {
  const int i = blockIdx.x * blockDim.x + threadIdx.x;
  if (i >= C) return;
  double s = 0.0;
#pragma unroll 8
  for (int b = 0; b < B; ++b) s += sums[(size_t)ncomp * ((size_t)b * C + i)];
  db[i] = (float)s;
}

extern "C" int sa_fin_bias(const double* sums, int B, int C, int ncomp, float* db, void* stream) {
  if (!sums || !db || ncomp < 1) return -22;
  hipLaunchKernelGGL(sa_fin_bias_kernel, dim3(sa_div_up(C, 128)), dim3(128), 0,
                     reinterpret_cast<hipStream_t>(stream), sums, B, C, ncomp, db);
  hipError_t e = hipGetLastError();
  return e == hipSuccess ? 0 : -(int)e;
}

__global__ __launch_bounds__(32 * SA_SP_LANES) void sa_bias_multi_l1_kernel(SaBiasMulti m) {
  __shared__ double part[SA_SP_LANES][33];
  const SaBiasDesc& d = m.d[blockIdx.z];
  const int bb = blockIdx.y, o = threadIdx.x & 31, q = threadIdx.x >> 5;
  const int i = blockIdx.x * 32 + o;
  if (bb >= d.nbatch || blockIdx.x * 32 >= d.C) return;
  double s = 0.0;
  const int n = d.C * d.ncomp;
  if (i < d.C) {
    const float* p = d.part + (size_t)bb * d.nslab * n + (size_t)i * d.ncomp;
#pragma unroll 16
    for (int k = q; k < d.nslab; k += SA_SP_LANES) s += (double)p[(size_t)k * n];
  }
  part[q][o] = s;
  __syncthreads();
  if (q == 0 && i < d.C) {
    double t = 0.0;
#pragma unroll
    for (int r = 0; r < SA_SP_LANES; ++r) t += part[r][o];
    d.rows[(size_t)bb * d.C + i] = t;
  }
}

__global__ void sa_bias_multi_l2_kernel(SaBiasMulti m) {
  const SaBiasDesc& d = m.d[blockIdx.y];
  const int i = blockIdx.x * blockDim.x + threadIdx.x;
  if (i >= d.C) return;
  double s = 0.0;
#pragma unroll 8
  for (int b = 0; b < d.nbatch; ++b) s += d.rows[(size_t)b * d.C + i];
  d.db[i] = (float)s;
}

extern "C" int sa_bias_multi(const SaBiasMulti* m, void* stream) {
  if (!m || m->n <= 0 || m->n > SA_BIAS_MAX) return -22;
  int maxC = 0, maxB = 0;
  for (int j = 0; j < m->n; ++j) {
    const SaBiasDesc& d = m->d[j];
    if (!d.part || !d.rows || !d.db || d.nbatch <= 0 || d.nslab <= 0 || d.C <= 0 || d.ncomp < 1) return -22;
    maxC = d.C > maxC ? d.C : maxC;
    maxB = d.nbatch > maxB ? d.nbatch : maxB;
  }
  hipStream_t st = reinterpret_cast<hipStream_t>(stream);
  hipLaunchKernelGGL(sa_bias_multi_l1_kernel, dim3(sa_div_up(maxC, 32), maxB, m->n), dim3(32 * SA_SP_LANES), 0, st, *m);
  hipLaunchKernelGGL(sa_bias_multi_l2_kernel, dim3(sa_div_up(maxC, 128), m->n), dim3(128), 0, st, *m);
  hipError_t e = hipGetLastError();
  return e == hipSuccess ? 0 : -(int)e;
}

#define SA_CLIP_BLKS 64
__global__ __launch_bounds__(256) void sa_clip_sumsq_kernel(SaFlats f, double* __restrict__ partials) {
  __shared__ double red[4];
  const float* p = f.f[blockIdx.y].p;
  const long long n = f.f[blockIdx.y].n;
  float s = 0.f;
  for (long long i = (long long)blockIdx.x * 256 + threadIdx.x; i < n; i += (long long)SA_CLIP_BLKS * 256) s = fmaf(p[i], p[i], s);
  double d = (double)s;
#pragma unroll
  for (int o = 32; o > 0; o >>= 1) d += __shfl_xor(d, o, 64);
  if ((threadIdx.x & 63) == 0) red[threadIdx.x >> 6] = d;
  __syncthreads();
  if (threadIdx.x == 0) partials[blockIdx.y * SA_CLIP_BLKS + blockIdx.x] = (red[0] + red[1]) + (red[2] + red[3]);
}

__global__ __launch_bounds__(256) void sa_clip_scale_kernel(SaFlats f, const double* __restrict__ partials, float max_norm,
                                                            float eps, float* __restrict__ total_norm) {
  __shared__ float coef_s;
  __shared__ double red[4];
  double d = (int)threadIdx.x < f.n * SA_CLIP_BLKS ? partials[threadIdx.x] : 0.0;
#pragma unroll
  for (int o = 32; o > 0; o >>= 1) d += __shfl_xor(d, o, 64);
  if ((threadIdx.x & 63) == 0) red[threadIdx.x >> 6] = d;
  __syncthreads();
  if (threadIdx.x == 0) {
    const float tn = (float)sqrt((red[0] + red[1]) + (red[2] + red[3]));
    float c = max_norm / (tn + eps);
    coef_s = (c < 1.0f || c != c) ? c : 1.0f;
    if (blockIdx.x == 0 && blockIdx.y == 0 && total_norm) *total_norm = tn;
  }
  __syncthreads();
  const float c = coef_s;
  if (c >= 1.0f) return;
  float* p = f.f[blockIdx.y].p;
  const long long n = f.f[blockIdx.y].n;
  for (long long i = (long long)blockIdx.x * 256 + threadIdx.x; i < n; i += (long long)SA_CLIP_BLKS * 256) p[i] *= c;
}

extern "C" int sa_clip_grads(const SaFlats* f, float max_norm, float eps, double* partials, float* total_norm,
                             void* stream) {
  if (!f || f->n <= 0 || f->n > SA_FLATS_MAX || !partials) return -22;
  for (int j = 0; j < f->n; ++j)
    if (!f->f[j].p || f->f[j].n <= 0) return -22;
  hipStream_t st = reinterpret_cast<hipStream_t>(stream);
  hipLaunchKernelGGL(sa_clip_sumsq_kernel, dim3(SA_CLIP_BLKS, f->n), dim3(256), 0, st, *f, partials);
  hipLaunchKernelGGL(sa_clip_scale_kernel, dim3(SA_CLIP_BLKS, f->n), dim3(256), 0, st, *f, partials, max_norm, eps, total_norm);
  hipError_t e = hipGetLastError();
  return e == hipSuccess ? 0 : -(int)e;
}
```

speech-anonymization_amd/csrc/sa_small.hip:

```cpp
#include "sa_common.h"

#define SA_K15 15
#define SA_C32 32

template <typename T>
__global__ __launch_bounds__(256) void sa_conv1toC_kernel(const float* __restrict__ x,
                                                          const float* __restrict__ w,
                                                          const float* __restrict__ bias,
                                                          T* __restrict__ y, int L, int flip,
                                                          float* __restrict__ stats, int ntiles,
                                                          const T* __restrict__ ep_x,
                                                          const float* __restrict__ ep_s1,
                                                          const float* __restrict__ ep_t1,
                                                          const float* __restrict__ ep_mean,
                                                          const float* __restrict__ ep_rstd) {
  constexpr int VEC = Tr<T>::VEC, CH = SA_C32 / VEC, PPP = 256 / CH, TILE = 512;
  __shared__ float xs[TILE + SA_K15 - 1];
  __shared__ __attribute__((aligned(16))) float ws[SA_K15][SA_C32];
  __shared__ float red[PPP][SA_C32][2];
  const int tid = threadIdx.x, b = blockIdx.y, l0 = blockIdx.x * TILE;
  for (int i = tid; i < TILE + SA_K15 - 1; i += 256) {
    const int g = l0 + i - 7;
    xs[i] = (g >= 0 && g < L) ? x[(size_t)b * L + g] : 0.0f;
  }
// ... 142 lines not shown
  }
  __syncthreads();
  const int l = l0 + tid;
  if (tid < TILE && l < L) {
    float acc = bias ? bias[0] : 0.0f;
#pragma unroll
    for (int k = 0; k < SA_K15; ++k) acc += tp[(tid + k) * TP + k];
    y[(size_t)b * L + l] = acc;
  }
}

extern "C" int sa_convCto1(int dtype, const void* x, const float* w, const float* bias, float* y,
                           int B, int L, const float* s1, const float* t1, int swish, int flip,
                           void* stream) {
  if (!x || !w || !y || B <= 0 || L <= 0) return -22;
  hipStream_t st = reinterpret_cast<hipStream_t>(stream);
  dim3 grid(sa_div_up(L, 128), B);
  if (dtype == SA_BF16)
    hipLaunchKernelGGL(sa_convCto1_kernel<bf16_t>, grid, dim3(256), 0, st,
                       reinterpret_cast<const bf16_t*>(x), w, bias, y, L, s1, t1, swish, flip);
  else
    hipLaunchKernelGGL(sa_convCto1_kernel<float>, grid, dim3(256), 0, st,
                       reinterpret_cast<const float*>(x), w, bias, y, L, s1, t1, swish, flip);
  hipError_t e = hipGetLastError();
  return e == hipSuccess ? 0 : -(int)e;
}

template <typename T>
__global__ __launch_bounds__(256) void sa_wgrad1C_kernel(const float* __restrict__ u,
                                                         const T* __restrict__ v,
                                                         float* __restrict__ slabs, int L,
                                                         int chunk, int flip,
                                                         const float* __restrict__ s1,
                                                         const float* __restrict__ t1, int swish) {
  constexpr int VEC = Tr<T>::VEC, CH = SA_C32 / VEC, RPP = 256 / CH, TILE = 256, PITCH = 33;
  __shared__ float us[TILE + SA_K15 - 1 + 1];
  __shared__ float vs[TILE * PITCH];
  const int tid = threadIdx.x, lane = tid & 63, wave = tid >> 6, b = blockIdx.y;
  const int lbeg = blockIdx.x * chunk;
  int lend = lbeg + chunk; if (lend > L) lend = L;
  const int c = tid % CH, r0 = tid / CH;
  float sc[VEC], sh[VEC];
#pragma unroll
  for (int j = 0; j < VEC; ++j) {
    sc[j] = s1 ? s1[(size_t)b * SA_C32 + c * VEC + j] : 1.0f;
    sh[j] = t1 ? t1[(size_t)b * SA_C32 + c * VEC + j] : 0.0f;
  }
  const bool tr_on = (s1 != nullptr) || swish;
  const int m = lane & 15, j4 = lane >> 4;
  const bool mval = m < SA_K15;
  const int kk = mval ? (flip ? SA_K15 - 1 - m : m) : 0;
  const int qa = wave * 64 + 16 * j4;
  f32x4 acc0 = {0.f, 0.f, 0.f, 0.f}, acc1 = {0.f, 0.f, 0.f, 0.f};
  constexpr int NIT = TILE / RPP, NU = (TILE + SA_K15 - 1 + 255) / 256;
  uint4 raw[NIT];
  float rawu[NU];
  auto issue = [&](int l0) {
#pragma unroll
    for (int i = 0; i < NIT; ++i) {
      const int g = l0 + r0 + i * RPP;
      raw[i] = make_uint4(0, 0, 0, 0);
      if (g < lend) raw[i] = *reinterpret_cast<const uint4*>(v + ((size_t)b * L + g) * SA_C32 + c * VEC);
    }
#pragma unroll
    for (int i = 0; i < NU; ++i) {
      const int g = l0 + tid + i * 256 - 7;
      rawu[i] = (l0 < lend && tid + i * 256 < TILE + SA_K15 - 1 && g >= 0 && g < L) ? u[(size_t)b * L + g] : 0.0f;
    }
  };
  issue(lbeg);
  for (int l0 = lbeg; l0 < lend; l0 += TILE) {
#pragma unroll
    for (int i = 0; i < NU; ++i)
      if (tid + i * 256 < TILE + SA_K15 - 1) us[tid + i * 256] = rawu[i];
#pragma unroll
    for (int i = 0; i < NIT; ++i) {
      const int r = r0 + i * RPP, g = l0 + r;
      float f[VEC];
      Tr<T>::unpack(raw[i], f);
      if (tr_on && g < lend) {
#pragma unroll
        for (int j = 0; j < VEC; ++j) {
          float z = fmaf(f[j], sc[j], sh[j]);
          f[j] = swish ? sa_swish(z) : z;
        }
      }
#pragma unroll
      for (int j = 0; j < VEC; ++j) vs[r * PITCH + c * VEC + j] = f[j];
    }
    __syncthreads();
    issue(l0 + TILE);
#pragma unroll 4
    for (int t = 0; t < 16; ++t) {
      const int q = qa + t;
      const float av = mval ? us[q + kk] : 0.0f;
      const float b0 = vs[q * PITCH + m], b1 = vs[q * PITCH + 16 + m];
      acc0 = __builtin_amdgcn_mfma_f32_16x16x4f32(av, b0, acc0, 0, 0, 0);
      acc1 = __builtin_amdgcn_mfma_f32_16x16x4f32(av, b1, acc1, 0, 0, 0);
    }
    __syncthreads();
  }
  float* part = vs;
#pragma unroll
  for (int i = 0; i < 4; ++i) {
    part[(wave * 16 + 4 * j4 + i) * 32 + m] = acc0[i];
    part[(wave * 16 + 4 * j4 + i) * 32 + 16 + m] = acc1[i];
  }
  __syncthreads();
  for (int o = tid; o < SA_K15 * SA_C32; o += 256) {
    const int k = o / SA_C32, cc = o % SA_C32;
    const float sum = ((part[(0 * 16 + k) * 32 + cc] + part[(1 * 16 + k) * 32 + cc]) +
                       part[(2 * 16 + k) * 32 + cc]) + part[(3 * 16 + k) * 32 + cc];
    slabs[((size_t)b * gridDim.x + blockIdx.x) * (SA_C32 * SA_K15) + cc * SA_K15 + k] = sum;
  }
}

extern "C" int sa_wgrad1C_nchunk(int L, int chunk) { return sa_div_up(L, chunk); }

extern "C" int sa_wgrad1C(int dtype, const float* u, const void* v, float* slabs, int B, int L,
                          int chunk, int flip, const float* s1, const float* t1, int swish,
                          void* stream) {
  if (!u || !v || !slabs || B <= 0 || L <= 0 || chunk <= 0 || chunk % 256) return -22;
  hipStream_t st = reinterpret_cast<hipStream_t>(stream);
  dim3 grid(sa_div_up(L, chunk), B);
  if (dtype == SA_BF16)
    hipLaunchKernelGGL(sa_wgrad1C_kernel<bf16_t>, grid, dim3(256), 0, st, u,
                       reinterpret_cast<const bf16_t*>(v), slabs, L, chunk, flip, s1, t1, swish);
  else
    hipLaunchKernelGGL(sa_wgrad1C_kernel<float>, grid, dim3(256), 0, st, u,
                       reinterpret_cast<const float*>(v), slabs, L, chunk, flip, s1, t1, swish);
  hipError_t e = hipGetLastError();
  return e == hipSuccess ? 0 : -(int)e;
}

template <typename T>
__global__ __launch_bounds__(256, Tr<T>::VEC == 4 ? 3 : 2) void sa_bwd1C_kernel(const float* __restrict__ u,
                                                       const T* __restrict__ v,
                                                       const float* __restrict__ w,
                                                       T* __restrict__ gout, float* __restrict__ stats,
                                                       int ntiles, float* __restrict__ slabs, int L,
                                                       int chunk, int flip,
                                                       const float* __restrict__ s1,
                                                       const float* __restrict__ t1,
                                                       const float* __restrict__ mean,
                                                       const float* __restrict__ rstd) {
  constexpr int VEC = Tr<T>::VEC, CH = SA_C32 / VEC, RPP = 256 / CH, TILE = 256, PITCH = 33;
  __shared__ float us[TILE + SA_K15 - 1 + 1];
  __shared__ float vs[TILE * PITCH];
  __shared__ __attribute__((aligned(16))) float ws[SA_K15][SA_C32];
  __shared__ float red[RPP][SA_C32][2];
  __shared__ __attribute__((aligned(16))) float pv[4][SA_C32];
  const int tid = threadIdx.x, lane = tid & 63, wave = tid >> 6, b = blockIdx.y;
  const int lbeg = blockIdx.x * chunk;
  int lend = lbeg + chunk; if (lend > L) lend = L;
  const int c = tid % CH, r0 = tid / CH;
  float ssum[VEC], ssq[VEC];
#pragma unroll
  for (int j = 0; j < VEC; ++j) { ssum[j] = 0.f; ssq[j] = 0.f; }
  if (tid < 4 * SA_C32) {
    const float* src = tid < 32 ? s1 : tid < 64 ? t1 : tid < 96 ? mean : rstd;
    pv[tid >> 5][tid & 31] = src[(size_t)b * SA_C32 + (tid & 31)];
  }
  for (int i = tid; i < SA_K15 * SA_C32; i += 256) {
    const int k = i / SA_C32, cc = i % SA_C32;
    ws[k][cc] = w[cc * SA_K15 + (flip ? SA_K15 - 1 - k : k)];
  }
  const int m = lane & 15, j4 = lane >> 4;
  const bool mval = m < SA_K15;
  const int kk = mval ? (flip ? SA_K15 - 1 - m : m) : 0;
  const int qa = wave * 64 + 16 * j4;
  f32x4 acc0 = {0.f, 0.f, 0.f, 0.f}, acc1 = {0.f, 0.f, 0.f, 0.f};
  constexpr int NIT = TILE / RPP, NU = (TILE + SA_K15 - 1 + 255) / 256;
  uint4 raw[NIT];
  float rawu[NU];
  auto issue_v = [&](int l0, int i) {
    const int g = l0 + r0 + i * RPP;
    raw[i] = make_uint4(0, 0, 0, 0);
    if (g < lend) raw[i] = *reinterpret_cast<const uint4*>(v + ((size_t)b * L + g) * SA_C32 + c * VEC);
  };
  auto issue_u = [&](int l0) {
#pragma unroll
    for (int i = 0; i < NU; ++i) {
      const int g = l0 + tid + i * 256 - 7;
      rawu[i] = (l0 < lend && tid + i * 256 < TILE + SA_K15 - 1 && g >= 0 && g < L) ? u[(size_t)b * L + g] : 0.0f;
    }
  };
#pragma unroll
  for (int i = 0; i < NIT; ++i) issue_v(lbeg, i);
  issue_u(lbeg);
  __syncthreads();
  for (int l0 = lbeg; l0 < lend; l0 += TILE) {
#pragma unroll
    for (int i = 0; i < NU; ++i)
      if (tid + i * 256 < TILE + SA_K15 - 1) us[tid + i * 256] = rawu[i];
#pragma unroll
    for (int i = 0; i < NIT; ++i) {
      const int r = r0 + i * RPP, g = l0 + r;
      float f[VEC];
      Tr<T>::unpack(raw[i], f);
      if (g < lend) {
        int z0 = c * VEC; asm volatile("" : "+v"(z0));
#pragma unroll
        for (int j = 0; j < VEC; ++j) f[j] = sa_swish(fmaf(f[j], pv[0][z0 + j], pv[1][z0 + j]));
      }
#pragma unroll
      for (int j = 0; j < VEC; ++j) vs[r * PITCH + c * VEC + j] = f[j];
    }
    __syncthreads();
    issue_u(l0 + TILE);
#pragma unroll
    for (int i = 0; i < NIT; ++i) {
      const int r = r0 + i * RPP, g = l0 + r;
      float xv[VEC];
      Tr<T>::unpack(raw[i], xv);
      issue_v(l0 + TILE, i);
      if (g < lend) {
#pragma clang fp contract(off)
        float acc[VEC], xn[VEC];
#pragma unroll
        for (int j = 0; j < VEC; ++j) acc[j] = 0.0f;
#pragma unroll
        for (int k = 0; k < SA_K15; ++k) {
          const float uv = us[r + k];
#pragma unroll
          for (int j = 0; j < VEC; ++j) acc[j] = fmaf(uv, ws[k][c * VEC + j], acc[j]);
        }
        int z0 = c * VEC; asm volatile("" : "+v"(z0));
#pragma unroll
        for (int j = 0; j < VEC; ++j) {
          acc[j] *= sa_swish_grad(fmaf(xv[j], pv[0][z0 + j], pv[1][z0 + j]));
          xn[j] = (xv[j] - pv[2][z0 + j]) * pv[3][z0 + j];
        }
        const uint4 o = Tr<T>::pack(acc);
        *reinterpret_cast<uint4*>(gout + ((size_t)b * L + g) * SA_C32 + c * VEC) = o;
        float f[VEC];
        Tr<T>::unpack(o, f);
#pragma unroll
        for (int j = 0; j < VEC; ++j) { ssum[j] += f[j]; ssq[j] = fmaf(f[j], xn[j], ssq[j]); }
      }
    }
    const bool flush = (((l0 - lbeg) / TILE) & 1) || l0 + TILE >= lend;
    if (flush) {
#pragma unroll
      for (int j = 0; j < VEC; ++j) {
        red[r0][c * VEC + j][0] = ssum[j]; red[r0][c * VEC + j][1] = ssq[j];
        ssum[j] = 0.f; ssq[j] = 0.f;
      }
    }
#pragma unroll 4
    for (int t = 0; t < 16; ++t) {
      const int q = qa + t;
      const float av = mval ? us[q + kk] : 0.0f;
      const float b0 = vs[q * PITCH + m], b1 = vs[q * PITCH + 16 + m];
      acc0 = __builtin_amdgcn_mfma_f32_16x16x4f32(av, b0, acc0, 0, 0, 0);
      acc1 = __builtin_amdgcn_mfma_f32_16x16x4f32(av, b1, acc1, 0, 0, 0);
    }
    __syncthreads();
    if (flush && tid < SA_C32) {
      float s = 0.f, q = 0.f;
      for (int r = 0; r < RPP; ++r) { s += red[r][tid][0]; q += red[r][tid][1]; }
      float* d = stats + (((size_t)b * ntiles + l0 / 512) * SA_C32 + tid) * 2;
      d[0] = s; d[1] = q;
    }
  }
  float* part = vs;
#pragma unroll
  for (int i = 0; i < 4; ++i) {
    part[(wave * 16 + 4 * j4 + i) * 32 + m] = acc0[i];
    part[(wave * 16 + 4 * j4 + i) * 32 + 16 + m] = acc1[i];
  }
  __syncthreads();
  for (int o = tid; o < SA_K15 * SA_C32; o += 256) {
    const int k = o / SA_C32, cc = o % SA_C32;
    const float sum = ((part[(0 * 16 + k) * 32 + cc] + part[(1 * 16 + k) * 32 + cc]) +
                       part[(2 * 16 + k) * 32 + cc]) + part[(3 * 16 + k) * 32 + cc];
    slabs[((size_t)b * gridDim.x + blockIdx.x) * (SA_C32 * SA_K15) + cc * SA_K15 + k] = sum;
  }
}

extern "C" int sa_bwd1C(int dtype, const float* u, const void* v, const float* w, void* g, float* stats,
                        float* slabs, int B, int L, int chunk, int flip, const float* s1,
                        const float* t1, const float* mean, const float* rstd, void* stream) {
  if (!u || !v || !w || !g || !stats || !slabs || B <= 0 || L <= 0 || chunk <= 0 || chunk % 512) return -22;
  if (!s1 || !t1 || !mean || !rstd) return -22;
  hipStream_t st = reinterpret_cast<hipStream_t>(stream);
  const int nt = sa_div_up(L, 512);
  dim3 grid(sa_div_up(L, chunk), B);
  if (dtype == SA_BF16)
    hipLaunchKernelGGL(sa_bwd1C_kernel<bf16_t>, grid, dim3(256), 0, st, u,
                       reinterpret_cast<const bf16_t*>(v), w, reinterpret_cast<bf16_t*>(g), stats, nt,
                       slabs, L, chunk, flip, s1, t1, mean, rstd);
  else
    hipLaunchKernelGGL(sa_bwd1C_kernel<float>, grid, dim3(256), 0, st, u,
                       reinterpret_cast<const float*>(v), w, reinterpret_cast<float*>(g), stats, nt,
                       slabs, L, chunk, flip, s1, t1, mean, rstd);
  hipError_t e = hipGetLastError();
  return e == hipSuccess ? 0 : -(int)e;
}

__global__ __launch_bounds__(256) void sa_sum_slabs_kernel(const float* __restrict__ slabs,
                                                           float* __restrict__ dst, int nslab, int n,
                                                           int accumulate) {
  __shared__ double part[16][17];
  const int o = threadIdx.x & 15, q = threadIdx.x >> 4, i = blockIdx.x * 16 + o;
  double s = 0.0;
  if (i < n) {
#pragma unroll 4
    for (int k = q; k < nslab; k += 16) s += (double)slabs[(size_t)k * n + i];
  }
  part[q][o] = s;
  __syncthreads();
  if (q == 0 && i < n) {
    double t = 0.0;
#pragma unroll
    for (int r = 0; r < 16; ++r) t += part[r][o];
    dst[i] = accumulate ? dst[i] + (float)t : (float)t;
  }
}

extern "C" int sa_sum_slabs(const float* slabs, float* dst, int nslab, int n, int accumulate,
                            void* stream) {
  if (!slabs || !dst || nslab <= 0 || n <= 0) return -22;
  hipLaunchKernelGGL(sa_sum_slabs_kernel, dim3(sa_div_up(n, 16)), dim3(256), 0,
                     reinterpret_cast<hipStream_t>(stream), slabs, dst, nslab, n, accumulate);
  hipError_t e = hipGetLastError();
  return e == hipSuccess ? 0 : -(int)e;
}
```

speech-anonymization_amd/csrc/sa_wgrad.hip:

```cpp
#include "sa_common.h"
#include <type_traits>

typedef __bf16 bf16x4 __attribute__((ext_vector_type(4)));

template <typename T>
__global__ void sa_pack_weights_kernel(const float* __restrict__ src, T* __restrict__ dst,
                                       int ntaps, int K, int N, int sk, int sn, int st) {
  constexpr int KS = Tr<T>::KS;
  constexpr int PER = KS / 2;
  const int total = ntaps * K * N;
  const int NT = N / 32, KSTEPS = K / KS;
  for (int i = blockIdx.x * blockDim.x + threadIdx.x; i < total; i += gridDim.x * blockDim.x) {
    const int j = i % PER;
    int r = i / PER;
    const int lane = r % 64; r /= 64;
    const int nt = r % NT; r /= NT;
    const int ks = r % KSTEPS;
    const int t = r / KSTEPS;
    const int k = ks * KS + PER * (lane >> 5) + j;
    const int n = nt * 32 + (lane & 31);
    dst[i] = Tr<T>::from_f(src[(size_t)k * sk + (size_t)n * sn + (size_t)t * st]);
  }
}

// ... 274 lines not shown
    }
  };
  auto stage = [&](LT* At, const RegSet& rs, int m0) {
    LT* Bt = At + C::AEL;
    if constexpr (XPRE) {
#pragma unroll
      for (int i = 0; i < C::NITA; ++i) {
        const int r = ra0 + i * RSA;
        if (r < C::RA) *reinterpret_cast<uint4*>(At + (size_t)r * PA + ca * VECA) = rs.a[i];
      }
    } else {
      float s1r[VEC], t1r[VEC], s2r[VEC], t2r[VEC];
      if (has1 || has2) {
#pragma unroll
        for (int j = 0; j < VEC; ++j) {
          s1r[j] = coef[ca * VEC + j]; t1r[j] = coef[CIN + ca * VEC + j];
          s2r[j] = coef[2 * CIN + ca * VEC + j]; t2r[j] = coef[3 * CIN + ca * VEC + j];
        }
      }
#pragma unroll
      for (int i = 0; i < C::NITA; ++i) {
        const int r = ra0 + i * RSA;
        if (r < C::RA) {
          const int g = m0 * SA + offmin + r;
          float f[VEC];
          tr::unpack(rs.a[i], f);
          if ((has1 || has2 || sw) && g >= 0 && g < a.Lin) {
#pragma unroll
            for (int j = 0; j < VEC; ++j) {
              float v = f[j];
              if (has1) v = fmaf(v, s1r[j], t1r[j]);
              if (sw) v = sa_swish(v);
              if (has2) v = fmaf(v, s2r[j], t2r[j]);
              f[j] = v;
            }
          }
          put(At, C::RA * PA, PA, r, ca, f);
        }
      }
    }
    if constexpr (YPRE) {
#pragma unroll
      for (int i = 0; i < C::NITB; ++i) {
        const int r = rb0 + i * RSB;
        if (r < C::RB) *reinterpret_cast<uint4*>(Bt + (size_t)r * PB + cb * VECB) = rs.b[i];
      }
    } else {
#pragma unroll
      for (int i = 0; i < C::NITB; ++i) {
        const int r = rb0 + i * RSB;
        if (r < C::RB) {
          float f[VEC];
          tr::unpack(rs.b[i], f);
          put(Bt, C::RB * PB, PB, r, cb, f);
        }
      }
    }
  };

  const int g4 = lane >> 4, i16 = lane & 15;
  const int trow = 8 * (g4 >> 1) + (i16 >> 2);
  const int tcol = 16 * (g4 & 1) + 4 * (i16 & 3);

  auto mfma_tile = [&](const LT* At) {
    const LT* Bt = At + C::AEL;
    for (int ks = kw; ks < KT / KS; ks += C::KW) {
      if constexpr (sizeof(LT) == 2) {
        Frag bh[PPW][U], bl[PPW][U];
#pragma unroll
        for (int q = 0; q < PPW; ++q)
#pragma unroll
          for (int ph = 0; ph < U; ++ph) {
            const LT* p = Bt + (size_t)((ks * 16 + trow) * U + ph) * PB + (nt0 + q) * 32 + tcol;
            bh[q][ph] = sa_tr_frag(p, U * PB);
            if constexpr (NPL == 2) bl[q][ph] = sa_tr_frag(p + C::RB * PB, U * PB);
          }
#pragma unroll
        for (int t = 0; t < SA_MAX_TAPS; ++t) {
          if (t < a.ntaps) {
            const LT* p = At + (size_t)((ks * 16 + trow) * SA + a.off[t] - offmin) * PA + mt * 32 + tcol;
            const Frag ah = sa_tr_frag(p, SA * PA);
            const int ph = U == 1 ? 0 : a.ph[t];
            Frag al;
            if constexpr (NPL == 2) al = sa_tr_frag(p + C::RA * PA, SA * PA);
#pragma unroll
            for (int q = 0; q < PPW; ++q) {
              if constexpr (NPL == 2) {
                acc[q][t] = __builtin_amdgcn_mfma_f32_32x32x16_bf16(al, ph ? bh[q][U - 1] : bh[q][0], acc[q][t], 0, 0, 0);
                acc[q][t] = __builtin_amdgcn_mfma_f32_32x32x16_bf16(ah, ph ? bl[q][U - 1] : bl[q][0], acc[q][t], 0, 0, 0);
              }
              acc[q][t] = __builtin_amdgcn_mfma_f32_32x32x16_bf16(ah, ph ? bh[q][U - 1] : bh[q][0], acc[q][t], 0, 0, 0);
            }
          }
        }
      } else {
        float bv[PPW][U];
#pragma unroll
        for (int q = 0; q < PPW; ++q)
#pragma unroll
          for (int ph = 0; ph < U; ++ph)
            bv[q][ph] = Bt[(size_t)((ks * 2 + (lane >> 5)) * U + ph) * PB + (nt0 + q) * 32 + (lane & 31)];
#pragma unroll
        for (int t = 0; t < SA_MAX_TAPS; ++t) {
          if (t < a.ntaps) {
            const float av = At[(size_t)((ks * 2 + (lane >> 5)) * SA + a.off[t] - offmin) * PA + mt * 32 + (lane & 31)];
            const int ph = U == 1 ? 0 : a.ph[t];
#pragma unroll
            for (int q = 0; q < PPW; ++q)
              acc[q][t] = __builtin_amdgcn_mfma_f32_32x32x2f32(av, ph ? bv[q][U - 1] : bv[q][0], acc[q][t], 0, 0, 0);
          }
        }
      }
    }
  };

  issue(set0, mbeg);
  if constexpr (NSETS == 2) issue(set1, mbeg + KT);
  __syncthreads();
  stage(tiles, set0, mbeg);
  issue(set0, mbeg + NSETS * KT);
  __syncthreads();
  const bool stage_first = wave < C::NW / 2;
  auto step = [&](RegSet& rs, int m0, int cur) {
    LT* now = tiles + (size_t)cur * C::BUFEL;
    LT* nxt = tiles + (size_t)(cur ^ 1) * C::BUFEL;
    const bool more = m0 + KT < mend;
    if (stage_first) {
      if (more) { stage(nxt, rs, m0 + KT); issue(rs, m0 + KT + NSETS * KT); }
      mfma_tile(now);
    } else {
      mfma_tile(now);
      if (more) { stage(nxt, rs, m0 + KT); issue(rs, m0 + KT + NSETS * KT); }
    }
    __syncthreads();
  };
  for (int m0 = mbeg; m0 < mend; m0 += 2 * KT) {
    step(NSETS == 2 ? set1 : set0, m0, 0);
    if (m0 + KT < mend) step(set0, m0 + KT, 1);
  }

  float* slab = a.slabs + ((((size_t)b * a.nchunk + chunk) * C::KW + kw) * a.ntaps) * CIN * COUT;
#pragma unroll
  for (int q = 0; q < PPW; ++q)
#pragma unroll
    for (int t = 0; t < SA_MAX_TAPS; ++t) {
      if (t < a.ntaps) {
#pragma unroll
        for (int r = 0; r < 16; ++r)
          slab[((size_t)t * CIN + mt * 32 + sa_acc_row(r, lane)) * COUT + (nt0 + q) * 32 + (lane & 31)] = acc[q][t][r];
      }
    }
}

extern "C" int sa_wgrad_kw(int cin, int cout) {
  const int np = (cin / 32) * (cout / 32);
  const int nw = np >= 8 ? 8 : 4, ppw = np > nw ? np / nw : 1;
  return nw / (np / ppw);
}

template <typename T, int CIN, int COUT, int SA, int U, bool XPRE = false, bool YPRE = false>
static int launch_wgrad(const SaWgradArgs& a, hipStream_t st) {
  typedef WgCfg<T, CIN, COUT, SA, U, XPRE, YPRE> C;
  int omin = a.off[0], omax = a.off[0];
  for (int t = 1; t < a.ntaps; ++t) {
    omin = a.off[t] < omin ? a.off[t] : omin;
    omax = a.off[t] > omax ? a.off[t] : omax;
  }
  if (omax - omin > C::HALO) return -22;
  for (int t = 0; t < a.ntaps; ++t) if (a.ph[t] < 0 || a.ph[t] >= U) return -22;
  if (C::LDS > 160 * 1024) return -12;
  auto kern = sa_wgrad_kernel<T, CIN, COUT, SA, U, XPRE, YPRE>;
  static bool attr_set = false;
  if (!attr_set) {
    hipError_t e = hipFuncSetAttribute(reinterpret_cast<const void*>(kern),
                                       hipFuncAttributeMaxDynamicSharedMemorySize, 160 * 1024);
    if (e != hipSuccess) return -(int)e;
    attr_set = true;
  }
  dim3 grid(a.nchunk * a.B);
  hipLaunchKernelGGL(kern, grid, dim3(C::NTHR), C::LDS, st, a);
  hipError_t e = hipGetLastError();
  return e == hipSuccess ? 0 : -(int)e;
}

#define SA_WG_CASE(CI, CO, S, UU)                                               \
  if (cin == CI && cout == CO && sa == S && u == UU)                            \
    return dtype == SA_BF16 ? (a->dy_pre ? launch_wgrad<bf16_t, CI, CO, S, UU, true, true>(*a, st)    \
                               : a->x_pre ? launch_wgrad<bf16_t, CI, CO, S, UU, true>(*a, st)       \
                                          : launch_wgrad<bf16_t, CI, CO, S, UU>(*a, st))            \
           : dtype == SA_BF16X3 ? launch_wgrad<bf16x3_t, CI, CO, S, UU>(*a, st) \
           : dtype == SA_BF16X1F ? (a->dy_pre ? launch_wgrad<bf16x1f_t, CI, CO, S, UU, true, true>(*a, st) \
                                    : a->x_pre ? launch_wgrad<bf16x1f_t, CI, CO, S, UU, true>(*a, st)     \
                                             : launch_wgrad<bf16x1f_t, CI, CO, S, UU>(*a, st)) \
                                : launch_wgrad<float, CI, CO, S, UU>(*a, st);

extern "C" int sa_wgrad(int dtype, int cin, int cout, int sa, int u, const SaWgradArgs* a,
                        void* stream) {
  hipStream_t st = reinterpret_cast<hipStream_t>(stream);
  if (!a || !a->x || !a->dy || !a->slabs || a->ntaps < 1 || a->ntaps > SA_MAX_TAPS ||
      a->chunk <= 0 || a->chunk % 64 || a->nchunk * a->chunk < a->Mrows ||
      (a->x_pre && dtype != SA_BF16X1F && dtype != SA_BF16) || (a->dy_pre && !a->x_pre))
    return -22;
  SA_WG_CASE(32, 64, 2, 1)
  SA_WG_CASE(64, 64, 1, 1)
  SA_WG_CASE(64, 128, 2, 1)
  SA_WG_CASE(128, 128, 1, 1)
  SA_WG_CASE(128, 64, 1, 2)
  SA_WG_CASE(64, 32, 1, 2)
  return -38;
}

template <int VEC>
__device__ __forceinline__ void wred_body(const float* __restrict__ slabs, float* __restrict__ dst, int nslab,
                                          int ntaps, int CIN, int COUT, int sk, int sn, int st, int accumulate,
                                          int bx, double (*part)[64 * 4]) {
  const int per = ntaps * CIN * COUT;
  const int lane = threadIdx.x & 63, q = threadIdx.x >> 6;
  const int i0 = (bx * 64 + lane) * VEC;
  double s[VEC];
#pragma unroll
  for (int j = 0; j < VEC; ++j) s[j] = 0.0;
  if (i0 < per) {
    const float* p = slabs + i0;
    int k = q;
    for (; k + 28 < nslab; k += 32) {
      float v[8][VEC];
#pragma unroll
      for (int u = 0; u < 8; ++u) {
        const float* r = p + (size_t)(k + 4 * u) * per;
        if constexpr (VEC == 4) { const float4 t = *reinterpret_cast<const float4*>(r); v[u][0] = t.x; v[u][1] = t.y; v[u][2] = t.z; v[u][3] = t.w; }
        else if constexpr (VEC == 2) { const float2 t = *reinterpret_cast<const float2*>(r); v[u][0] = t.x; v[u][1] = t.y; }
        else v[u][0] = *r;
      }
#pragma unroll
      for (int u = 0; u < 8; ++u)
#pragma unroll
        for (int j = 0; j < VEC; ++j) s[j] += (double)v[u][j];
    }
    for (; k < nslab; k += 4) {
      const float* r = p + (size_t)k * per;
#pragma unroll
      for (int j = 0; j < VEC; ++j) s[j] += (double)r[j];
    }
  }
  if (q > 0) {
#pragma unroll
    for (int j = 0; j < VEC; ++j) part[q - 1][lane * VEC + j] = s[j];
  }
  __syncthreads();
  if (q == 0 && i0 < per) {
#pragma unroll
    for (int j = 0; j < VEC; ++j) {
      const double t = ((s[j] + part[0][lane * VEC + j]) + part[1][lane * VEC + j]) + part[2][lane * VEC + j];
      const int i = i0 + j;
      const int co = i % COUT, ci = (i / COUT) % CIN, tp = i / (COUT * CIN);
      const size_t d = (size_t)ci * sk + (size_t)co * sn + (size_t)tp * st;
      dst[d] = accumulate ? dst[d] + (float)t : (float)t;
    }
  }
}

template <int VEC>
__global__ __launch_bounds__(256) void sa_wgrad_reduce_kernel(const float* __restrict__ slabs,
                                                              float* __restrict__ dst, int nslab,
                                                              int ntaps, int CIN, int COUT, int sk,
                                                              int sn, int st, int accumulate) {
  __shared__ double part[3][64 * 4];
  wred_body<VEC>(slabs, dst, nslab, ntaps, CIN, COUT, sk, sn, st, accumulate, blockIdx.x, part);
}

__global__ __launch_bounds__(256) void sa_wgrad_reduce_multi_kernel(SaWredMulti m) {
  __shared__ double part[3][64 * 4];
  const SaWredDesc& d = m.d[blockIdx.y];
  const int per = d.ntaps * d.cin * d.cout;
  if ((int)blockIdx.x * 64 * d.vec >= per) return;
  if (d.vec == 4) wred_body<4>(d.slabs, d.dst, d.nslab, d.ntaps, d.cin, d.cout, d.sk, d.sn, d.st, d.accumulate, blockIdx.x, part);
  else if (d.vec == 2) wred_body<2>(d.slabs, d.dst, d.nslab, d.ntaps, d.cin, d.cout, d.sk, d.sn, d.st, d.accumulate, blockIdx.x, part);
  else wred_body<1>(d.slabs, d.dst, d.nslab, d.ntaps, d.cin, d.cout, d.sk, d.sn, d.st, d.accumulate, blockIdx.x, part);
}

static int wred_vec(int per) {
  if (per % 4 == 0 && per >= 4 * 64 * 256) return 4;
  if (per % 2 == 0 && per >= 2 * 64 * 256) return 2;
  return 1;
}

extern "C" int sa_wgrad_reduce_multi(const SaWredMulti* m, void* stream) {
  if (!m || m->n <= 0 || m->n > SA_WRED_MAX) return -22;
  SaWredMulti mm = *m;
  int gx = 0;
  for (int j = 0; j < mm.n; ++j) {
    SaWredDesc& d = mm.d[j];
    if (!d.slabs || !d.dst || d.nslab <= 0 || d.ntaps <= 0 || d.cin <= 0 || d.cout <= 0) return -22;
    const int per = d.ntaps * d.cin * d.cout;
    d.vec = wred_vec(per);
    const int nb = sa_div_up(per, 64 * d.vec);
    gx = nb > gx ? nb : gx;
  }
  hipLaunchKernelGGL(sa_wgrad_reduce_multi_kernel, dim3(gx, mm.n), dim3(256), 0, reinterpret_cast<hipStream_t>(stream), mm);
  hipError_t e = hipGetLastError();
  return e == hipSuccess ? 0 : -(int)e;
}

extern "C" int sa_wgrad_reduce(const float* slabs, float* dst, int nslab, int ntaps, int cin,
                               int cout, int sk, int sn, int st, int accumulate, void* stream) {
  if (!slabs || !dst || nslab <= 0) return -22;
  const int per = ntaps * cin * cout;
  hipStream_t s_ = reinterpret_cast<hipStream_t>(stream);
  if (per % 4 == 0 && per >= 4 * 64 * 256)
    hipLaunchKernelGGL(sa_wgrad_reduce_kernel<4>, dim3(sa_div_up(per, 256)), dim3(256), 0, s_, slabs, dst,
                       nslab, ntaps, cin, cout, sk, sn, st, accumulate);
  else if (per % 2 == 0 && per >= 2 * 64 * 256)
    hipLaunchKernelGGL(sa_wgrad_reduce_kernel<2>, dim3(sa_div_up(per, 128)), dim3(256), 0, s_, slabs, dst,
                       nslab, ntaps, cin, cout, sk, sn, st, accumulate);
  else
    hipLaunchKernelGGL(sa_wgrad_reduce_kernel<1>, dim3(sa_div_up(per, 64)), dim3(256), 0, s_, slabs, dst,
                       nslab, ntaps, cin, cout, sk, sn, st, accumulate);
  hipError_t e = hipGetLastError();
  return e == hipSuccess ? 0 : -(int)e;
}
```

speech-anonymization_amd/ops.py:

```python
import collections
import ctypes as C
import functools
import sys

import torch

from . import _lib as L

UP2 = [[(1, 0), (0, 2), (-1, 4)], [(1, 1), (0, 3)]]


def taps_conv(K, dil, pad):
    return [[(k * dil - pad, k) for k in range(K)]]


def taps_conv_dgrad_s1(K, dil, pad):
    return [[(pad - k * dil, k) for k in range(K)]]


def taps_convT_dgrad(K=5, pad=2):
    return [[(k - pad, k) for k in range(K)]]


CONVT_WG_TAPS = [(1, 0), (1, 1), (0, 0), (0, 1), (-1, 0)]
# ... 15 lines not shown
    def lout(self, Lin):
        if self.transposed:
            return 2 * Lin
        return Lin // 2 if self.stride == 2 else Lin + 2 * self.pad - self.dil * (self.K - 1)

    def lin(self, Lout):
        if self.transposed:
            return Lout // 2
        return 2 * Lout if self.stride == 2 else Lout - 2 * self.pad + self.dil * (self.K - 1)

    @functools.lru_cache(maxsize=256)
    def fwd(self, Lin):
        if self.transposed:
            return self.cin, self.cout, 1, 2, UP2, 2 * Lin
        return self.cin, self.cout, self.stride, 1, taps_conv(self.K, self.dil, self.pad), self.lout(Lin)

    @functools.lru_cache(maxsize=256)
    def dgrad(self, Lin):
        if self.transposed:
            return self.cout, self.cin, 2, 1, taps_convT_dgrad(), Lin
        if self.stride == 2:
            return self.cout, self.cin, 1, 2, UP2, Lin
        return self.cout, self.cin, 1, 1, taps_conv_dgrad_s1(self.K, self.dil, self.pad), Lin

    @functools.lru_cache(maxsize=256)
    def wgrad(self, Lin):
        if self.transposed:
            return self.cin, self.cout, 1, 2, CONVT_WG_TAPS, Lin, (self.cout * self.K, self.K, 1)
        return (self.cin, self.cout, self.stride, 1, [(k * self.dil - self.pad, 0) for k in range(self.K)],
                self.lout(Lin), (self.K, self.cin * self.K, 1))


def conv_layers(model, roots):
    return {f"{r}.{n}": ConvGeom.of(f"{r}.{n}", m) for r in roots for n, m in model.get_submodule(r).named_children()
            if isinstance(m, (torch.nn.Conv1d, torch.nn.ConvTranspose1d)) and min(m.in_channels, m.out_channels) > 1}


def _f(t):
    return L.ptr(t)


class _Profile:

    def __init__(self):
        self.key, self.kinds = None, {}

    def enable(self, key):
        self.key, self.kinds = key, {}

    def start(self, key):
        if key != self.key:
            return None
        e = torch.cuda.Event(enable_timing=True)
        e.record()
        return e

    def stop(self, e0, nbytes, flops, alg_bytes=None, kind=""):
        e1 = torch.cuda.Event(enable_timing=True)
        e1.record()
        k = self.kinds.setdefault(kind, {"ev": [], "bytes": 0, "alg_bytes": 0, "flops": 0})
        k["ev"].append((e0, e1))
        k["bytes"] += nbytes
        k["alg_bytes"] += nbytes if alg_bytes is None else alg_bytes
        k["flops"] += flops

    def collect(self):
        torch.cuda.synchronize()
        out = []
        for kind, k in self.kinds.items():
            out.append({"kernel": kind or self.key, "family": self.key, "launches": len(k["ev"]),
                        "ms": sum(a.elapsed_time(b) for a, b in k["ev"]), "bytes": k["bytes"],
                        "alg_bytes": k["alg_bytes"], "flops": k["flops"]})
        out.sort(key=lambda r: -r["ms"])
        self.key, self.kinds = None, {}
        return out


PROFILE = _Profile()


PRECISIONS = {"f32": (torch.float32, L.F32), "bf16": (torch.bfloat16, L.BF16),
              "bf16x3": (torch.float32, L.BF16X3), "bf16x1f": (torch.float32, L.BF16X1F),
              "fp8": (torch.bfloat16, L.FP8)}
WGRAD_CODE = {"f32": L.F32, "bf16": L.BF16, "bf16x3": L.BF16X1F, "bf16x1f": L.BF16X1F, "fp8": L.BF16}
DGRAD_CODE = {"f32": L.F32, "bf16": L.BF16, "bf16x3": L.BF16X3, "bf16x1f": L.BF16X1F, "fp8": L.BF16}


def _pack_geometry(shape, kind):
    if kind in ("conv_fwd", "conv_dgrad"):
        Cout, Cin, Kw = shape
        if kind == "conv_fwd":
            return Kw, Cin, Cout, Kw, Cin * Kw
        return Kw, Cout, Cin, Cin * Kw, Kw
    Cin, Cout, Kw = shape
    if kind == "convT_fwd":
        return Kw, Cin, Cout, Cout * Kw, Kw
    return Kw, Cout, Cin, Kw, Cout * Kw


def _image_buffer(code, dtype, n, device):
    if code == L.FP8:
        return torch.empty(n + 4, dtype=torch.uint8, device=device)
    if code == L.BF16X3:
        return torch.empty(2 * n, dtype=torch.bfloat16, device=device)
    if code in (L.BF16X1F, L.BF16):
        return torch.empty(n, dtype=torch.bfloat16, device=device)
    return torch.empty(n, dtype=torch.float32, device=device)


def pack_weights(w, kind, dtype, code=None):
    lib = L.load()
    code = L.dt_code(dtype) if code is None else code
    Kw, K, N, sk, sn = _pack_geometry(w.shape, kind)
    out = _image_buffer(code, dtype, Kw * K * N, w.device)
    L.check(lib.sa_pack_weights(code, _f(w), _f(out), Kw, K, N, sk, sn, 1, L.stream()),
            "sa_pack_weights")
    return out


class PackedWeights:

    def __init__(self, items, dtype):
        self.images, descs = {}, (L.SaPackDesc * len(items))()
        dev = items[0][1].device
        for d, (tag, w, kind, code) in zip(descs, items):
            Kw, K, N, sk, sn = _pack_geometry(w.shape, kind)
            img = _image_buffer(code, dtype, Kw * K * N, dev)
            self.images[tag] = (img, code)
            d.src, d.dst, d.dtype = w.data_ptr(), img.data_ptr(), code
            d.ntaps, d.K, d.N, d.sk, d.sn, d.st = Kw, K, N, sk, sn, 1
            d.scale = img.data_ptr() + Kw * K * N if code == L.FP8 else None
            self.fp8 = getattr(self, "fp8", False) or code == L.FP8
        raw = torch.frombuffer(bytearray(bytes(descs)), dtype=torch.uint8)
        self.table = raw.to(dev)
        self.n = len(items)
        self.key = tuple(w.data_ptr() for _, w, _, _ in items)

    def refresh(self):
        if getattr(self, "fp8", False):
            L.check(L.load().sa_pack_scales_multi(_f(self.table), self.n, L.stream()), "sa_pack_scales_multi")
        L.check(L.load().sa_pack_weights_multi(_f(self.table), self.n, 64, L.stream()),
                "sa_pack_weights_multi")


@functools.lru_cache(maxsize=None)
def _conv_geometry(cin, cout, u, Lout):
    return L.load().sa_conv_gemm_ntiles(cin, cout, u, Lout)


def conv_impl(pingpong=False, tile_rows=0, ws=True):
    if pingpong:
        raise L.SaHipError("the ping-pong conv kernel was removed (it tied the one-tile kernel forward and lost "
                           "on the fused data gradients: DESIGN.md section 4); use ws=True or ws=False")
    lib = L.load()
    L.check(lib.sa_conv_gemm_set_impl(2 if ws else 0), "sa_conv_gemm_set_impl")
    L.check(lib.sa_conv_gemm_set_tile_rows(int(tile_rows)), "sa_conv_gemm_set_tile_rows")
    _conv_geometry.cache_clear()


def conv_gemm(x, wp, bias, cin, cout, sa, u, phases, Lout, s1=None, t1=None, s2=None, t2=None,
              swish=False, relu=False, want_stats=False, out=None, code=None, ep=None, a_out=None,
              nb=None, want_pro_stats=False):
    lib = L.load()
    B, Lin, _ = x.shape
    assert x.shape[2] == cin
    y = out if out is not None else torch.empty(B, Lout, cout, dtype=x.dtype, device=x.device)
    kc = L.dt_code(x.dtype) if code is None else code
    nt = _conv_geometry(cin, cout, u, Lout)
    stats = torch.empty(B, nt, cout, 2, dtype=torch.float32, device=x.device) if want_stats else None
    a = L.SaConvArgs()
    a.x, a.wp, a.bias, a.y = _f(x), _f(wp), _f(bias), _f(y)
    a.s1, a.t1, a.s2, a.t2 = _f(s1), _f(t1), _f(s2), _f(t2)
    a.swish, a.relu, a.stats = int(swish), int(relu), _f(stats)
    a.B, a.Lin, a.Lout = B, Lin, Lout
    a.taps = L.make_taps(phases)
    if kc == L.FP8:
        a.wscale = C.c_void_p(wp.data_ptr() + wp.numel() - 4)
    if a_out is not None:
        assert a_out.dtype == torch.bfloat16 and a_out.shape == x.shape
        a.a_out = _f(a_out)
    pro_stats = None
    if want_pro_stats:
        pro_stats = torch.empty(B, nt, cin, 2, dtype=torch.float32, device=x.device)
        a.pro_stats = _f(pro_stats)
    colsum = None
    if nb:
        assert nb["x"].shape == x.shape and nb["x"].dtype == x.dtype
        a.nb_x, a.nb_c1, a.nb_c2, a.nb_c3 = _f(nb["x"]), _f(nb["c1"]), _f(nb["c2"]), _f(nb["c3"])
        a.nb_bstride, a.nb_relu_mask = (0 if nb.get("per_c") else cin), int(bool(nb.get("relu_mask")))
        if nb.get("want_colsum"):
            colsum = torch.empty(B, nt, cin, dtype=torch.float32, device=x.device)
            a.nb_colsum = _f(colsum)
    if ep:
        a.ep_mode, a.ep_xp_is_act = int(ep["mode"]), int(bool(ep.get("xp_is_act")))
        a.ep_bstride = 0 if ep.get("per_c") else cout
        a.ep_x, a.ep_g2 = _f(ep["x"]), _f(ep.get("g2"))
        a.ep_s1, a.ep_t1 = _f(ep.get("s1")), _f(ep.get("t1"))
        a.ep_mean, a.ep_rstd = _f(ep.get("mean")), _f(ep.get("rstd"))
        if ep.get("g2k") is not None:
            a.ep_g2k1, a.ep_g2k2, a.ep_g2k3 = (_f(t) for t in ep["g2k"])
    e0 = PROFILE.start(f"conv_gemm({cin},{cout},{sa},{u})") if PROFILE.key else None
    L.check(lib.sa_conv_gemm(kc, cin, cout, sa, u, C.byref(a), L.stream()),
            f"sa_conv_gemm({cin},{cout},{sa},{u})")
    if e0 is not None:
        ntap = sum(len(p) for p in phases)
        esz = x.element_size()
        extra = (a_out.numel() * 2 if a_out is not None else 0)
        if ep:
            extra += y.numel() * esz * (2 if ep.get("g2") is not None else 1)
        if nb:
            extra += x.numel() * esz
        io = (x.numel() + y.numel()) * esz
        route = lib.sa_conv_gemm_route(kc, cin, cout, sa, u, C.byref(a))
        tname = {L.F32: "float", L.BF16: "bf16_t", L.BF16X3: "bf16x3_t", L.BF16X1F: "bf16x1f_t", L.FP8: "fp8_t"}[kc]
        ws_mode = (5 if s2 is not None else 0) if s1 is None else 3 if want_pro_stats else 4 if s2 is not None else 1
        kind = (f"sa_conv_wsd_kernel ({tname}, {cin}->{cout}; 5 instances)" if route == 3 else
                f"sa_conv_ws_kernel<{ws_mode},{ntap}> ({tname}, {cin}->{cout})" if route == 2 else
                f"sa_conv_gemm_kernel<{tname},{cin},{cout},{sa},{u}{',nb prologue' if nb else ''}>")
        PROFILE.stop(e0, io + ntap * cin * cout * esz + extra,
                     2 * B * (-(-Lout // u)) * ntap * cin * cout,
                     alg_bytes=io + (y.numel() * esz if ep else 0), kind=kind)
    out_t = (y, stats) if want_stats else (y,)
    if nb and nb.get("want_colsum"):
        out_t = out_t + (colsum,)
    if want_pro_stats:
        out_t = out_t + (pro_stats,)
    return out_t if len(out_t) > 1 else y


WGRAD_TARGET_WGS = {True: 256, False: 512}


def wgrad(x, dy, cin, cout, sa, u, taps, Mrows, dst, dst_strides, s1=None, t1=None, s2=None,
          t2=None, swish=False, accumulate=False, target_wgs=None, code=None, x_pre=False,
          dy_pre=False, defer=None):
    lib = L.load()
    B, Lin, _ = x.shape
    Ldy = dy.shape[1]
    if x_pre:
        assert x.dtype == torch.bfloat16 and code in (L.BF16X1F, L.BF16)
    nt = len(taps)
    kw = lib.sa_wgrad_kw(cin, cout)
    if target_wgs is None:
        target_wgs = WGRAD_TARGET_WGS[(cin // 32) * (cout // 32) >= 8]
    chunk = max(64, -(-Mrows * B // target_wgs))
    chunk = -(-chunk // 64) * 64
    nchunk = -(-Mrows // chunk)
    slabs = torch.empty(B * nchunk * kw * nt * cin * cout, dtype=torch.float32, device=x.device)
    a = L.SaWgradArgs()
    a.x, a.dy, a.slabs = _f(x), _f(dy), _f(slabs)
    a.s1, a.t1, a.s2, a.t2, a.swish = _f(s1), _f(t1), _f(s2), _f(t2), int(swish)
    a.B, a.Lin, a.Ldy, a.Mrows, a.chunk, a.nchunk, a.ntaps = B, Lin, Ldy, Mrows, chunk, nchunk, nt
    for i, (off, ph) in enumerate(taps):
        a.off[i], a.ph[i] = off, ph
    a.x_pre, a.dy_pre = int(x_pre), int(dy_pre)
    if dy_pre:
        assert x_pre and dy.dtype == torch.bfloat16
    L.check(lib.sa_wgrad((L.BF16X1F if dy_pre else L.dt_code(dy.dtype)) if code is None else code, cin, cout, sa, u,
                         C.byref(a), L.stream()),
            f"sa_wgrad({cin},{cout},{sa},{u})")
    sk, sn, st = dst_strides
    if defer is not None:
        defer.append((slabs, dst, B * nchunk * kw, nt, cin, cout, sk, sn, st, int(accumulate)))
        return dst
    L.check(lib.sa_wgrad_reduce(_f(slabs), _f(dst), B * nchunk * kw, nt, cin, cout, sk, sn, st,
                                int(accumulate), L.stream()), "sa_wgrad_reduce")
    return dst


def wgrad_reduce_multi(items):
    lib = L.load()
    for i0 in range(0, len(items), L.WRED_MAX):
        m = L.SaWredMulti()
        chunk = items[i0:i0 + L.WRED_MAX]
        m.n = len(chunk)
        for d, (slabs, dst, nslab, nt, cin, cout, sk, sn, st, acc) in zip(m.d, chunk):
            d.slabs, d.dst = slabs.data_ptr(), dst.data_ptr()
            d.nslab, d.ntaps, d.cin, d.cout, d.sk, d.sn, d.st, d.accumulate = nslab, nt, cin, cout, sk, sn, st, acc
        L.check(lib.sa_wgrad_reduce_multi(C.byref(m), L.stream()), "sa_wgrad_reduce_multi")


def conv1toC(x, w, bias, dtype, flip=False, want_stats=False, ep=None):
    lib = L.load()
    B, Ln = x.shape
    y = torch.empty(B, Ln, 32, dtype=dtype, device=x.device)
    nt = lib.sa_conv1toC_ntiles(Ln)
    stats = torch.empty(B, nt, 32, 2, dtype=torch.float32, device=x.device) if want_stats else None
    e = ep or {}
    L.check(lib.sa_conv1toC(L.dt_code(dtype), _f(x), _f(w), _f(bias), _f(y), B, Ln, int(flip),
                            _f(stats), _f(e.get("x")), _f(e.get("s1")), _f(e.get("t1")),
                            _f(e.get("mean")), _f(e.get("rstd")), L.stream()), "sa_conv1toC")
    return (y, stats) if want_stats else y


def convCto1(x, w, bias, s1=None, t1=None, swish=False, flip=False):
    lib = L.load()
    B, Ln, _ = x.shape
    y = torch.empty(B, Ln, dtype=torch.float32, device=x.device)
    L.check(lib.sa_convCto1(L.dt_code(x.dtype), _f(x), _f(w), _f(bias), _f(y), B, Ln, _f(s1), _f(t1),
                            int(swish), int(flip), L.stream()), "sa_convCto1")
    return y


def wgrad1C(u, v, dst, flip=False, s1=None, t1=None, swish=False, accumulate=False, chunk=2048):
    lib = L.load()
    B, Ln = u.shape
    nch = lib.sa_wgrad1C_nchunk(Ln, chunk)
    slabs = torch.empty(B * nch, 32 * 15, dtype=torch.float32, device=u.device)
    L.check(lib.sa_wgrad1C(L.dt_code(v.dtype), _f(u), _f(v), _f(slabs), B, Ln, chunk, int(flip),
                           _f(s1), _f(t1), int(swish), L.stream()), "sa_wgrad1C")
    L.check(lib.sa_sum_slabs(_f(slabs), _f(dst), B * nch, 32 * 15, int(accumulate), L.stream()),
            "sa_sum_slabs")
    return dst


def bwd1C(u, v, w, dst, s1, t1, mean, rstd, flip=True, accumulate=False, chunk=2048):
    lib = L.load()
    B, Ln = u.shape
    nch = lib.sa_wgrad1C_nchunk(Ln, chunk)
    g = torch.empty(B, Ln, 32, dtype=v.dtype, device=u.device)
    stats = torch.empty(B, lib.sa_conv1toC_ntiles(Ln), 32, 2, dtype=torch.float32, device=u.device)
    slabs = torch.empty(B * nch, 32 * 15, dtype=torch.float32, device=u.device)
    L.check(lib.sa_bwd1C(L.dt_code(v.dtype), _f(u), _f(v), _f(w), _f(g), _f(stats), _f(slabs), B, Ln, chunk,
                         int(flip), _f(s1), _f(t1), _f(mean), _f(rstd), L.stream()), "sa_bwd1C")
    L.check(lib.sa_sum_slabs(_f(slabs), _f(dst), B * nch, 32 * 15, int(accumulate), L.stream()),
            "sa_sum_slabs")
    return g, stats, dst


def sum_partials(part, nbatch, n=None, rows=False):
    lib = L.load()
    if n is None:
        n = part.shape[-2] * part.shape[-1]
    total = part.numel()
    nslab = total // (nbatch * n)
    if nbatch == 1 and nslab >= 512 and part.dim() == 4 and part.shape[0] > 1:
        R = part.shape[0]
        mid = torch.empty(R, n, dtype=torch.float64, device=part.device)
        L.check(lib.sa_sum_partials(_f(part), _f(mid), R, nslab // R, n, L.stream()), "sa_sum_partials")
        if rows:
            return mid
        out = torch.empty(1, n, dtype=torch.float64, device=part.device)
        L.check(lib.sa_sum_rows_d(_f(mid), _f(out), R, n, L.stream()), "sa_sum_rows_d")
        return out
    out = torch.empty(nbatch, n, dtype=torch.float64, device=part.device)
    L.check(lib.sa_sum_partials(_f(part), _f(out), nbatch, nslab, n, L.stream()), "sa_sum_partials")
    return out


def fin_in_fwd(sums, B, Cc, n, gamma, beta, eps=1e-5):
    lib = L.load()
    o = torch.empty(4, B, Cc, dtype=torch.float32, device=sums.device)
    L.check(lib.sa_fin_in_fwd(_f(sums), B, Cc, n, _f(gamma), _f(beta), C.c_float(eps), _f(o[0]),
                              _f(o[1]), _f(o[2]), _f(o[3]), L.stream()), "sa_fin_in_fwd")
    return o[0], o[1], o[2], o[3]


def fin_bn_fwd(sums, Cc, count, gamma, beta, run_mean=None, run_var=None, eps=1e-5, momentum=0.1,
               count_dev=None):
    lib = L.load()
    o = torch.empty(4, Cc, dtype=torch.float32, device=sums.device)
    L.check(lib.sa_fin_bn_fwd(_f(sums), sums.numel() // (2 * Cc), Cc, C.c_double(count), _f(gamma), _f(beta), C.c_float(eps),
                              C.c_float(momentum), _f(run_mean), _f(run_var), _f(o[0]), _f(o[1]),
                              _f(o[2]), _f(o[3]), _f(count_dev), L.stream()), "sa_fin_bn_fwd")
    return o[0], o[1], o[2], o[3]


def fin_bn_eval(Cc, gamma, beta, run_mean, run_var, eps=1e-5):
    lib = L.load()
    o = torch.empty(4, Cc, dtype=torch.float32, device=gamma.device)
    L.check(lib.sa_fin_bn_eval(Cc, _f(gamma), _f(beta), C.c_float(eps), _f(run_mean), _f(run_var),
                               _f(o[0]), _f(o[1]), _f(o[2]), _f(o[3]), L.stream()), "sa_fin_bn_eval")
    return o[0], o[1], o[2], o[3]


def fin_norm_bwd(sums, lsums, groups, Cc, n, gamma, mean, rstd, sign=1.0, dgamma=None, dbeta=None,
                 n_dev=None):
    lib = L.load()
    o = torch.empty(3, groups, dtype=torch.float32, device=sums.device)
    R = sums.numel() // (2 * groups)
    assert lsums is None or lsums.numel() == sums.numel()
    L.check(lib.sa_fin_norm_bwd(_f(sums), _f(lsums), R, groups, Cc, C.c_double(n), _f(gamma), _f(mean),
                                _f(rstd), C.c_float(sign), _f(o[0]), _f(o[1]), _f(o[2]), _f(dgamma),
                                _f(dbeta), _f(n_dev), L.stream()), "sa_fin_norm_bwd")
    return o[0], o[1], o[2]


def bias_multi(items):
    lib = L.load()
    dev = items[0][0].device
    rows = torch.empty(sum(nb * cc for _, nb, cc, _, _ in items), dtype=torch.float64, device=dev)
    rp, esz = rows.data_ptr(), 8
    for i0 in range(0, len(items), L.BIAS_MAX):
        m = L.SaBiasMulti()
        chunk = items[i0:i0 + L.BIAS_MAX]
        m.n = len(chunk)
        for d, (part, nb, cc, ncomp, db) in zip(m.d, chunk):
            d.part, d.rows, d.db = part.data_ptr(), rp, db.data_ptr()
            d.nbatch, d.nslab, d.C, d.ncomp = nb, part.numel() // (nb * cc * ncomp), cc, ncomp
            rp += nb * cc * esz
        L.check(lib.sa_bias_multi(C.byref(m), L.stream()), "sa_bias_multi")


def fin_bias(sums, B, Cc, db, ncomp=2):
    L.check(L.load().sa_fin_bias(_f(sums), B, Cc, ncomp, _f(db), L.stream()), "sa_fin_bias")
    return db


def ew(kind, g, x, Cc, out=None, g2=None, s1=None, t1=None, mean=None, rstd=None, c1=None, c2=None,
       c3=None, actbwd=False, xp_is_act=False, relu_mask=False, per_c=False, want_stats=True):
    lib = L.load()
    B, Ln, _ = x.shape
    nt = lib.sa_ew_ntiles(Ln)
    stats = torch.empty(B, nt, Cc, 2, dtype=torch.float32, device=x.device) if want_stats else None
    a = L.SaEwArgs()
    a.g, a.g2, a.x, a.out = _f(g), _f(g2), _f(x), _f(out)
    a.s1, a.t1, a.mean, a.rstd = _f(s1), _f(t1), _f(mean), _f(rstd)
    a.c1, a.c2, a.c3 = _f(c1), _f(c2), _f(c3)
    a.actbwd, a.xp_is_act, a.relu_mask = int(actbwd), int(xp_is_act), int(relu_mask)
    a.bstride = 0 if per_c else Cc
    a.stats, a.B, a.L = _f(stats), B, Ln
    fn = lib.sa_ew_stats if kind == "stats" else lib.sa_ew_apply
    L.check(fn(L.dt_code(x.dtype), Cc, C.byref(a), L.stream()), f"sa_ew_{kind}")
    return stats


def pooling_noise(setting, B, Cc, device):
    if setting is None or setting is False:
        return None
    if torch.is_tensor(setting):
        return setting.to(device=device, dtype=torch.float32).contiguous()
    g = torch.randn(B, Cc, device=device)
    g = g - g.min()
    return (g / g.max()).contiguous()


def pooling_noise_raw(setting, B, Cc, device):
    if setting is True:
        return torch.randn(B, Cc, device=device), True
    return pooling_noise(setting, B, Cc, device), False


def pool_fwd(r, scale, shift, noise=None, eps=1e-5, fused=False, raw=False):
    lib = L.load()
    B, Ln, _ = r.shape
    nseg = lib.sa_pool_nseg(B)
    part = torch.empty(B, nseg, 128, 128, 2, dtype=torch.float32, device=r.device)
    L.check(lib.sa_pool_fwd(L.dt_code(r.dtype), _f(r), _f(scale), _f(shift), _f(part), B, Ln, nseg,
                            L.stream()), "sa_pool_fwd")
    pooled = torch.empty(B, 256, dtype=torch.float32, device=r.device)
    mean = torch.empty(B, 128, dtype=torch.float32, device=r.device)
    sd = torch.empty(B, 128, dtype=torch.float32, device=r.device)
    if fused:
        if noise is not None and (noise.numel() != B * 128 or noise.dtype != torch.float32):
            raise L.SaHipError(f"pooling noise must be fp32 [{B}, 128], got {noise.dtype} {tuple(noise.shape)}")
        L.check(lib.sa_pool_gather_fin(_f(part), B, nseg, Ln, _f(noise), int(bool(raw)), C.c_float(eps), _f(pooled),
                                       _f(mean), _f(sd), L.stream()), "sa_pool_gather_fin")
        return pooled, mean, sd
    if raw:
        raise L.SaHipError("raw pooling noise needs fused=True")
    sums = torch.empty(B, 128, 2, dtype=torch.float64, device=r.device)
    L.check(lib.sa_pool_gather(_f(part), B, nseg, Ln, _f(sums), L.stream()), "sa_pool_gather")
    L.check(lib.sa_pool_fin(_f(sums), B, Ln, _f(noise), C.c_float(eps), _f(pooled), _f(mean), _f(sd),
                            L.stream()), "sa_pool_fin")
    return pooled, mean, sd


def pool_bwd(r, scale, shift, dpooled, mean, sd, bn=None):
    lib = L.load()
    B, Ln, _ = r.shape
    g = torch.empty_like(r)
    st = torch.empty(B, -(-Ln // 256), 128, 2, dtype=torch.float32, device=r.device) if bn else None
    L.check(lib.sa_pool_bwd(L.dt_code(r.dtype), _f(r), _f(scale), _f(shift), _f(dpooled), _f(mean),
                            _f(sd), _f(g), B, Ln, _f(bn[0]) if bn else None, _f(bn[1]) if bn else None,
                            _f(st), L.stream()), "sa_pool_bwd")
    return (g, st) if bn else g


def dense(X, W, bias, N, K, ps=None, pt=None, relu=False, transpose_w=False):
    lib = L.load()
    M = X.shape[0]
    Y = torch.empty(M, N, dtype=torch.float32, device=X.device)
    sbk, sbn = (W.shape[1], 1) if transpose_w else (1, W.shape[1])
    L.check(lib.sa_dense(_f(X), X.shape[1], _f(ps), _f(pt), _f(W), sbk, sbn, _f(bias), _f(Y), N, M, N,
                         K, int(relu), L.stream()), "sa_dense")
    return Y


def colsums(X, H=None, hmean=None, hrstd=None, out0=None, out1=None):
    lib = L.load()
    M, N = X.shape
    s = torch.empty(N, 2, dtype=torch.float64, device=X.device)
    for o in (out0, out1):
        assert o is None or (o.dtype == torch.float32 and o.numel() == N and o.is_contiguous())
    L.check(lib.sa_colsums(_f(X), _f(H), _f(hmean), _f(hrstd), M, N, _f(s), _f(out0), _f(out1), L.stream()),
            "sa_colsums")
    return s


def bn2d_bwd(G, H, sums, count, gamma, mean, rstd, relu_mask, count_dev=None):
    lib = L.load()
    M, N = G.shape
    dH = torch.empty_like(G)
    L.check(lib.sa_bn2d_bwd(_f(G), _f(H), _f(sums), C.c_double(count), _f(gamma), _f(mean), _f(rstd),
                            int(relu_mask), M, N, _f(dH), _f(count_dev), L.stream()), "sa_bn2d_bwd")
    return dH


def dense_wgrad(dY, X, dW, ps=None, pt=None):
    lib = L.load()
    M, N = dY.shape
    K = X.shape[1]
    L.check(lib.sa_dense_wgrad(_f(dY), _f(X), _f(ps), _f(pt), M, N, K, _f(dW), L.stream()),
            "sa_dense_wgrad")
    return dW


def head_max_rows():
    return L.load().sa_head_max_rows()


def head_fwd(pooled, P, bn1, bn2, eps=1e-5, momentum=0.1):
    M = pooled.shape[0]
    dev = pooled.device
    H1 = torch.empty(M, 128, dtype=torch.float32, device=dev)
    H2 = torch.empty(M, 64, dtype=torch.float32, device=dev)
    f1 = torch.empty(4, 128, dtype=torch.float32, device=dev)
    f2 = torch.empty(4, 64, dtype=torch.float32, device=dev)
    logp = torch.empty(M, 2, dtype=torch.float32, device=dev)
    L.check(L.load().sa_head_fwd(_f(pooled), _f(P["0.weight"]), _f(P["0.bias"]), _f(P["2.weight"]), _f(P["2.bias"]),
                                 _f(bn1.running_mean), _f(bn1.running_var), _f(P["3.weight"]), _f(P["3.bias"]),
                                 _f(P["5.weight"]), _f(P["5.bias"]), _f(bn2.running_mean), _f(bn2.running_var),
                                 _f(P["6.weight"]), _f(P["6.bias"]), _f(H1), _f(f1), _f(H2), _f(f2), _f(logp), M,
                                 C.c_float(eps), C.c_float(momentum), L.stream()), "sa_head_fwd")
    return H1, tuple(f1[i] for i in range(4)), H2, tuple(f2[i] for i in range(4)), logp


def head_bwd(dlogp, logp, pooled, H1, f1, H2, f2, P, grads, wide=False):
    M = pooled.shape[0]
    dpooled = torch.empty(M, 256, dtype=torch.float32, device=pooled.device)
    g = lambda k: _f(grads.get(k))
    lib = L.load()
    entry, name = (lib.sa_head_bwd_wide, "sa_head_bwd_wide") if wide else (lib.sa_head_bwd, "sa_head_bwd")
    L.check(entry(_f(dlogp), _f(logp), _f(pooled), _f(H1), _f(f1[0]), _f(H2), _f(f2[0]),
                  _f(P["0.weight"]), _f(P["2.weight"]), _f(P["3.weight"]), _f(P["5.weight"]),
                  _f(P["6.weight"]), g("0.weight"), g("0.bias"), g("2.weight"), g("2.bias"),
                  g("3.weight"), g("3.bias"), g("5.weight"), g("5.bias"), g("6.weight"), g("6.bias"),
                  _f(dpooled), M, L.stream()), name)
    return dpooled


def log_softmax(X):
    Y = torch.empty_like(X)
    L.check(L.load().sa_log_softmax(_f(X), _f(Y), X.shape[0], X.shape[1], L.stream()), "sa_log_softmax")
    return Y


def log_softmax_bwd(dY, Y):
    dX = torch.empty_like(Y)
    L.check(L.load().sa_log_softmax_bwd(_f(dY), _f(Y), _f(dX), Y.shape[0], Y.shape[1], L.stream()),
            "sa_log_softmax_bwd")
    return dX


def recon_loss(a, b, kind, want_grad=True):
    lib = L.load()
    n = a.numel()
    if a.data_ptr() % 16:
        a = a.clone()
    if b.data_ptr() % 16:
        b = b.clone()
    loss = torch.empty(1, dtype=torch.float32, device=a.device)
    grad = torch.empty_like(a) if want_grad else None
    ws = torch.empty(lib.sa_loss_workspace_bytes() // 8, dtype=torch.float64, device=a.device)
    L.check(lib.sa_recon_loss(_f(a), _f(b), C.c_longlong(n), 0 if kind == "l1" else 1, _f(grad),
                              _f(loss), _f(ws), L.stream()), "sa_recon_loss")
    return loss, grad


def cls_losses(logp, label, want_grad=True):
    lib = L.load()
    B, NC = logp.shape
    out = torch.empty(2, dtype=torch.float32, device=logp.device)
    dn = torch.empty_like(logp) if want_grad else None
    dc = torch.empty_like(logp) if want_grad else None
    L.check(lib.sa_cls_losses(_f(logp), _f(label), B, NC, _f(out), _f(dn), _f(dc), L.stream()),
            "sa_cls_losses")
    return out, dn, dc


def step_loss(pred, target, kind, logp, label, w_recon, w_sex, nonfinite=None):
    lib = L.load()
    n = pred.numel()
    if pred.data_ptr() % 16:
        pred = pred.clone()
    if target.data_ptr() % 16:
        target = target.clone()
    B, NC = logp.shape
    dev = pred.device
    ws = torch.empty(lib.sa_loss_workspace_bytes() // 8, dtype=torch.float64, device=dev)
    d_pred = torch.empty_like(pred)
    d_logp = torch.empty_like(logp)
    out = torch.empty(3, dtype=torch.float32, device=dev)
    L.check(lib.sa_recon_loss_part(_f(pred), _f(target), C.c_longlong(n), 0 if kind == "l1" else 1, _f(d_pred),
                                   C.c_float(w_recon), _f(ws), L.stream()), "sa_recon_loss_part")
    L.check(lib.sa_step_loss(_f(ws), C.c_longlong(n), _f(logp), _f(label), B, NC, C.c_float(w_recon),
                             C.c_float(w_sex), _f(out), _f(d_logp), _f(nonfinite), L.stream()), "sa_step_loss")
    return out, d_pred, d_logp


def cosine_loss(x1, x2, want_grad=False):
    lib = L.load()
    B, S, D = x1.shape
    rl = torch.empty(B * S, dtype=torch.float32, device=x1.device)
    loss = torch.empty(1, dtype=torch.float32, device=x1.device)
    dx1 = torch.empty_like(x1) if want_grad else None
    L.check(lib.sa_cosine_loss(_f(x1), _f(x2), B, S, D, _f(rl), _f(loss), _f(dx1), L.stream()),
            "sa_cosine_loss")
    return loss, dx1


def cosine_rows(x1, x2):
    lib = L.load()
    B, D = x1.shape
    x1, x2 = x1.contiguous().float(), x2.contiguous().float()
    rl = torch.empty(B, dtype=torch.float32, device=x1.device)
    loss = torch.empty(1, dtype=torch.float32, device=x1.device)
    L.check(lib.sa_cosine_loss(_f(x1), _f(x2), B, 1, D, _f(rl), _f(loss), None, L.stream()),
            "sa_cosine_loss")
    return 1.0 - rl


def cluster_mi(X, y, idx=None, ncls=2, k=3):
    lib = L.load()
    iters, n = (idx.shape if idx is not None else (1, X.shape[0]))
    mi = torch.empty(iters, dtype=torch.float32, device=X.device)
    L.check(lib.sa_cluster_mi(_f(X), _f(y), _f(idx), iters, n, X.shape[1], ncls, k, _f(mi), L.stream()),
            "sa_cluster_mi")
    return mi


def add_layernorm(x, r, gamma, beta, eps, save):
    d = x.shape[-1]
    rows = x.numel() // d
    y = torch.empty_like(x)
    s = torch.empty_like(x) if save else None
    stat = torch.empty(rows, 2, dtype=torch.float32, device=x.device) if save else None
    L.check(L.load().sa_add_layernorm_fwd(_f(x), _f(r), _f(gamma), _f(beta), _f(y), _f(s), _f(stat), rows, d,
                                          C.c_float(eps), L.stream()), "sa_add_layernorm_fwd")
    return y, s, stat


def layernorm_bwd(dy, s, stat, gamma):
    d = s.shape[-1]
    ds = torch.empty_like(s)
    L.check(L.load().sa_layernorm_bwd(_f(dy), _f(s), _f(stat), _f(gamma), _f(ds), s.numel() // d, d, L.stream()),
            "sa_layernorm_bwd")
    return ds
# ... 1024 lines not shown
```

Before: 4.024 million frames/s.

## Fuse instance-norm stat reduction with finalize and batch stage-tail reductions

Instance-norm forward and backward now reduce per-slab partial stats and compute normalization coefficients in one kernel, replacing the separate sum_partials and finalize launches. The dgamma/dbeta reductions, the 1-to-C weight-gradient slab sums, bias reductions and weight-gradient reductions pending at each stage are gathered into a single multi-job stage_tail launch. The aim is fewer small kernel launches and fewer intermediate fp64 round trips. In exchange the gradient reductions are deferred until the stage flush, and the combined kernel sizes its grid for the largest job.

```diff
diff --git a/include/sa_hip.h b/include/sa_hip.h
--- a/include/sa_hip.h
+++ b/include/sa_hip.h
@@ -149,6 +149,18 @@
 } SaBiasDesc;
 typedef struct SaBiasMulti { int n, pad_; SaBiasDesc d[SA_BIAS_MAX]; } SaBiasMulti;
 int sa_bias_multi(const SaBiasMulti* m, void* stream);
+
+int sa_in_fwd_fused(const float* stats, int B, int nslab, int C, int n, const float* gamma, const float* beta,
+                    float eps, float* mean, float* rstd, float* scale, float* shift, void* stream);
+int sa_in_bwd_fused(const float* stats, int B, int nslab, int C, double n, const float* gamma, const float* mean,
+                    const float* rstd, float sign, float* c1, float* c2, float* c3, double* sums, void* stream);
+#define SA_TAIL_IN_MAX 4
+#define SA_TAIL_SLAB_MAX 2
+typedef struct SaTailIn { const double* sums; float* dgamma; float* dbeta; int B, C; } SaTailIn;
+typedef struct SaTailSlab { const float* slabs; float* dst; int nslab, n, accumulate, pad_; } SaTailSlab;
+typedef struct SaTailMisc { int nin, nslab; SaTailIn in[SA_TAIL_IN_MAX]; SaTailSlab sl[SA_TAIL_SLAB_MAX]; } SaTailMisc;
+int sa_stage_tail_record_bytes(void);
+int sa_stage_tail(const SaBiasMulti* bias, const SaWredMulti* wred, const SaTailMisc* misc, void* stream);
 
 int sa_pool_fwd(int dtype, const void* r, const float* scale, const float* shift, float* part, int B,
                 int L, int nseg, void* stream);
diff --git a/speech-anonymization_amd/_lib.py b/speech-anonymization_amd/_lib.py
--- a/speech-anonymization_amd/_lib.py
+++ b/speech-anonymization_amd/_lib.py
@@ -97,6 +97,22 @@
 
 class SaWredMulti(C.Structure):
     _fields_ = [("n", C.c_int), ("pad_", C.c_int), ("d", SaWredDesc * WRED_MAX)]
+
+
+TAIL_IN_MAX, TAIL_SLAB_MAX = 4, 2
+
+
+class SaTailIn(C.Structure):
+    _fields_ = [("sums", vp), ("dgamma", vp), ("dbeta", vp), ("B", C.c_int), ("C", C.c_int)]
+
+
+class SaTailSlab(C.Structure):
+    _fields_ = [("slabs", vp), ("dst", vp), ("nslab", C.c_int), ("n", C.c_int), ("accumulate", C.c_int),
+                ("pad_", C.c_int)]
+
+
+class SaTailMisc(C.Structure):
+    _fields_ = [("nin", C.c_int), ("nslab", C.c_int), ("in_", SaTailIn * TAIL_IN_MAX), ("sl", SaTailSlab * TAIL_SLAB_MAX)]
 
 
 SYMBOLS = [
@@ -114,6 +130,7 @@
     "sa_comm_destroy", "sa_head_fwd", "sa_head_bwd", "sa_head_bwd_wide", "sa_head_max_rows",
     "sa_add_layernorm_fwd", "sa_layernorm_bwd", "sa_reflect_pad_fwd", "sa_reflect_pad_bwd", "sa_ln_leaky_fwd", "sa_ln_leaky_bwd", "sa_bias_multi", "sa_asr_block0_fwd", "sa_asr_block0_bwd", "sa_wgrad_reduce_multi", "sa_clip_grads",
     "sa_adam_record_bytes", "sa_adam_step",
+    "sa_in_fwd_fused", "sa_in_bwd_fused", "sa_stage_tail_record_bytes", "sa_stage_tail",
     "sa_xv_tdnn_fwd_train", "sa_xv_tdnn_ntiles", "sa_xv_colsums", "sa_xv_tdnn_wgrad", "sa_xv_wgrad_reduce",
     "sa_xv_tdnn_dgrad", "sa_xv_pool_affine", "sa_xv_pool_affine_bwd",
     "sa_fc_tiles", "sa_fc_groups", "sa_fc_nparam", "sa_fc_nhead", "sa_fc_max_rows", "sa_fc_enc_fwd", "sa_fc_bn_fin",
@@ -164,6 +181,9 @@
         if _lib.sa_adam_record_bytes() != C.sizeof(SaAdamRec):
             raise SaHipError(f"SaAdamRec: binding has {C.sizeof(SaAdamRec)} bytes, {LIB_PATH} "
                              f"{_lib.sa_adam_record_bytes()} -- rebuild the library (stale build?)")
+        if _lib.sa_stage_tail_record_bytes() != C.sizeof(SaTailMisc):
+            raise SaHipError(f"SaTailMisc: binding has {C.sizeof(SaTailMisc)} bytes, {LIB_PATH} "
+                             f"{_lib.sa_stage_tail_record_bytes()} -- rebuild the library (stale build?)")
     return _lib
 
 
diff --git a/speech-anonymization_amd/convae.py b/speech-anonymization_amd/convae.py
--- a/speech-anonymization_amd/convae.py
+++ b/speech-anonymization_amd/convae.py
@@ -80,6 +80,8 @@
         self.sync_bn = sync_bn
         self.fused_head = os.environ.get("SA_FUSED_HEAD", "1") == "1"
         self.fused_bwd1c = os.environ.get("SA_FUSED_BWD1C", "1") == "1"
+        self.fold_in = os.environ.get("SA_FOLD_IN", "1") == "1"
+        self.fold_stage = os.environ.get("SA_FOLD_STAGE", "1") == "1"
         self.fused_pool_fin = os.environ.get("SA_FUSED_POOL_FIN", "1") == "1"
         self.wide_head_bwd = os.environ.get("SA_WIDE_HEAD_BWD", "1") == "1"
         self.dp_batch_sizes = None
@@ -231,6 +233,8 @@
         return _conv(x, W[ly.key, ly.kinds[0]], P[ly.bias], *ly.fwd(x.shape[1]), **kw)
 
     def inorm(stats, n, prefix, C):
+        if model.fold_in:
+            return ops.in_fwd_fused(stats, B, C, n, P[prefix + ".weight"], P[prefix + ".bias"])
         sums = ops.sum_partials(stats, B)
         return ops.fin_in_fwd(sums, B, C, n, P[prefix + ".weight"], P[prefix + ".bias"])
     return cg, inorm
@@ -414,20 +418,35 @@
 
         pending_bias = []
 
+        pending_in = []
+        pending_slab = [] if model.fold_stage else None
+
         def flush_pending():
-            if pending_bias:
-                ops.bias_multi(pending_bias)
-                pending_bias.clear()
-            if pending_wred:
-                ops.wgrad_reduce_multi(pending_wred)
-                pending_wred.clear()
+            if model.fold_stage:
+                if pending_bias or pending_wred or pending_in or pending_slab:
+                    ops.stage_tail(pending_bias, pending_wred, pending_in, pending_slab)
+                pending_slab.clear()
+            else:
+                if pending_bias:
+                    ops.bias_multi(pending_bias)
+                if pending_wred:
+                    ops.wgrad_reduce_multi(pending_wred)
+                if pending_in:
+                    ops.stage_tail(norms=pending_in)
+            pending_bias.clear()
+            pending_wred.clear()
+            pending_in.clear()
 
         def in_finish(g, st, y, nrm, C, Ln, prefix, bias_key):
             mean, rstd = nrm[0], nrm[1]
             dg, db = newg(prefix + ".weight"), newg(prefix + ".bias")
-            sums = ops.sum_partials(st, B)
-            c1, c2, c3 = ops.fin_norm_bwd(sums, sums, B * C, C, Ln, P[prefix + ".weight"], mean, rstd,
-                                          dgamma=dg, dbeta=db)
+            if model.fold_in:
+                (c1, c2, c3), sums = ops.in_bwd_fused(st, B, C, Ln, P[prefix + ".weight"], mean, rstd)
+                pending_in.append((sums, B, C, dg, db))
+            else:
+                sums = ops.sum_partials(st, B)
+                c1, c2, c3 = ops.fin_norm_bwd(sums, sums, B * C, C, Ln, P[prefix + ".weight"], mean, rstd,
+                                              dgamma=dg, dbeta=db)
             G[prefix + ".weight"], G[prefix + ".bias"] = dg, db
             if fuse:
                 return _PendingApply(g, y, (c1, c2, c3), False, False, bias_key)
@@ -561,11 +580,11 @@
                 setg("decoder.8.bias", ops.sum_partials(g_rec.view(4 * B, Ltot // 4), 1, n=Ltot // 4).sum())
             if need["decoder.8.weight"] and model.fused_bwd1c:
                 g, st, G["decoder.8.weight"] = ops.bwd1C(g_rec, y8, P["decoder.8.weight"], newg("decoder.8.weight"),
-                                                         n8[2], n8[3], n8[0], n8[1])
+                                                         n8[2], n8[3], n8[0], n8[1], defer=pending_slab)
             else:
                 if need["decoder.8.weight"]:
                     G["decoder.8.weight"] = ops.wgrad1C(g_rec, y8, newg("decoder.8.weight"), flip=True,
-                                                        s1=n8[2], t1=n8[3], swish=True)
+                                                        s1=n8[2], t1=n8[3], swish=True, defer=pending_slab)
                 g, st = ops.conv1toC(g_rec, P["decoder.8.weight"], None, dt, flip=True, want_stats=True,
                                      ep=dict(x=y8, s1=n8[2], t1=n8[3], mean=n8[0], rstd=n8[1]))
             g = in_finish(g, st, y8, n8, 32, Ltot, "decoder.6", "decoder.5.bias")
@@ -602,7 +621,7 @@
             g, st = cg(ly, g, want_stats=True, ep=_in_ep(x, nx) if nx else dict(mode=1, x=x))
         bias_from(st, "encoder.0.bias", 32)
         if need["encoder.0.weight"]:
-            G["encoder.0.weight"] = ops.wgrad1C(S["x0"], g, newg("encoder.0.weight"))
+            G["encoder.0.weight"] = ops.wgrad1C(S["x0"], g, newg("encoder.0.weight"), defer=pending_slab)
         d_feats = None
         if ctx.need_input_grad:
             d_feats = ops.convCto1(g, P["encoder.0.weight"], None, flip=True).view(B, T, 80)
diff --git a/speech-anonymization_amd/csrc/sa_common.h b/speech-anonymization_amd/csrc/sa_common.h
--- a/speech-anonymization_amd/csrc/sa_common.h
+++ b/speech-anonymization_amd/csrc/sa_common.h
@@ -89,6 +89,57 @@
 
 static inline int sa_div_up(int a, int b) { return (a + b - 1) / b; }
 
+__device__ __forceinline__ void sa_bias_l2_body(const SaBiasDesc& d, int i) {
+  if (i >= d.C) return;
+  double s = 0.0;
+#pragma unroll 8
+  for (int b = 0; b < d.nbatch; ++b) s += d.rows[(size_t)b * d.C + i];
+  d.db[i] = (float)s;
+}
+
+__device__ __forceinline__ void sa_norm_dgdb_body(const double* __restrict__ lsums, int R, int G, int C, int nb,
+                                                  int blk, float* dgamma, float* dbeta, double (*part)[32][2]) {
+  const int ch = blk * 32 + (threadIdx.x & 31), q = threadIdx.x >> 5;
+  double a = 0.0, bsum = 0.0;
+  if (ch < C) {
+    const int tot = R * nb;
+#pragma unroll 4
+    for (int e = q; e < tot; e += 8) {
+      const int r = e / nb, b = e % nb;
+      const size_t at = 2 * ((size_t)r * G + (size_t)b * C + ch);
+      bsum += lsums[at]; a += lsums[at + 1];
+    }
+  }
+  part[q][threadIdx.x & 31][0] = bsum; part[q][threadIdx.x & 31][1] = a;
+  __syncthreads();
+  if (q == 0 && ch < C) {
+    double s0 = 0.0, s1 = 0.0;
+#pragma unroll
+    for (int k = 0; k < 8; ++k) { s0 += part[k][threadIdx.x][0]; s1 += part[k][threadIdx.x][1]; }
+    dbeta[ch] = (float)s0; dgamma[ch] = (float)s1;
+  }
+}
+
+__device__ __forceinline__ void sa_sum_slabs_body(const float* __restrict__ slabs, float* __restrict__ dst,
+                                                  int nslab, int n, int accumulate, int blk, double (*part)[17]) {
+  const int o = threadIdx.x & 15, q = threadIdx.x >> 4, i = blk * 16 + o;
+  double s = 0.0;
+  if (i < n) {
+#pragma unroll 4
+    for (int k = q; k < nslab; k += 16) s += (double)slabs[(size_t)k * n + i];
+  }
+  part[q][o] = s;
+  __syncthreads();
+  if (q == 0 && i < n) {
+    double t = 0.0;
+#pragma unroll
+    for (int r = 0; r < 16; ++r) t += part[r][o];
+    dst[i] = accumulate ? dst[i] + (float)t : (float)t;
+  }
+}
+
+int sa_bias_multi_level1(const SaBiasMulti* m, hipStream_t st);
+
 struct bf16x3_t {};
 struct bf16x1f_t {};
 
diff --git a/speech-anonymization_amd/csrc/sa_elementwise.hip b/speech-anonymization_amd/csrc/sa_elementwise.hip
--- a/speech-anonymization_amd/csrc/sa_elementwise.hip
+++ b/speech-anonymization_amd/csrc/sa_elementwise.hip
@@ -110,26 +110,32 @@
 }
 
 #define SA_SP_LANES 16
+__device__ __forceinline__ double sa_sp_column_total(const float* __restrict__ slabs, int nslab, int n, int bb,
+                                                     int i, int o, int q, double (*part)[33]) {
+  double s = 0.0;
+  if (i < n) {
+    const float* p = slabs + (size_t)bb * nslab * n + i;
+#pragma unroll 16
+    for (int k = q; k < nslab; k += SA_SP_LANES) s += (double)p[(size_t)k * n];
+  }
+  part[q][o] = s;
+  __syncthreads();
+  double t = 0.0;
+  if (q == 0 && i < n) {
+#pragma unroll
+    for (int r = 0; r < SA_SP_LANES; ++r) t += part[r][o];
+  }
+  return t;
+}
+
 __global__ __launch_bounds__(32 * SA_SP_LANES) void sa_sum_partials_kernel(const float* __restrict__ slabs,
                                                                            double* __restrict__ dst,
                                                                            int nslab, int n) {
   __shared__ double part[SA_SP_LANES][33];
   const int bb = blockIdx.y, o = threadIdx.x & 31, q = threadIdx.x >> 5;
   const int i = blockIdx.x * 32 + o;
-  double s = 0.0;
-  if (i < n) {
-    const float* p = slabs + (size_t)bb * nslab * n + i;
-#pragma unroll 16
-    for (int k = q; k < nslab; k += SA_SP_LANES) s += (double)p[(size_t)k * n];
-  }
-  part[q][o] = s;
-  __syncthreads();
-  if (q == 0 && i < n) {
-    double t = 0.0;
-#pragma unroll
-    for (int r = 0; r < SA_SP_LANES; ++r) t += part[r][o];
-    dst[(size_t)bb * n + i] = t;
-  }
+  const double t = sa_sp_column_total(slabs, nslab, n, bb, i, o, q, part);
+  if (q == 0 && i < n) dst[(size_t)bb * n + i] = t;
 }
 
 extern "C" int sa_sum_partials(const float* slabs, double* dst, int nbatch, int nslab, int n,
@@ -158,17 +164,23 @@
   return e == hipSuccess ? 0 : -(int)e;
 }
 
+__device__ __forceinline__ void sa_in_fwd_coef(double S, double Q, float n, float g, float b, float eps,
+                                               float& mean, float& rstd, float& scale, float& shift) {
+  const double m = S / n;
+  double var = Q / n - m * m;
+  if (var < 0.0) var = 0.0;
+  const float r = (float)(1.0 / sqrt(var + (double)eps));
+  const float sc = g * r;
+  mean = (float)m; rstd = r; scale = sc; shift = b - (float)m * sc;
+}
+
 __global__ void sa_fin_in_fwd_kernel(const double* __restrict__ sums, int BC, int C, float n,
                                      const float* __restrict__ gamma, const float* __restrict__ beta,
                                      float eps, float* mean, float* rstd, float* scale, float* shift) {
   const int i = blockIdx.x * blockDim.x + threadIdx.x;
   if (i >= BC) return;
-  const double m = (double)sums[2 * i] / n;
-  double var = (double)sums[2 * i + 1] / n - m * m;
-  if (var < 0.0) var = 0.0;
-  const float r = (float)(1.0 / sqrt(var + (double)eps));
-  const float sc = gamma[i % C] * r;
-  mean[i] = (float)m; rstd[i] = r; scale[i] = sc; shift[i] = beta[i % C] - (float)m * sc;
+  sa_in_fwd_coef(sums[2 * i], sums[2 * i + 1], n, gamma[i % C], beta[i % C], eps, mean[i], rstd[i], scale[i],
+                 shift[i]);
 }
 
 extern "C" int sa_fin_in_fwd(const double* sums, int B, int C, int n, const float* gamma,
@@ -178,6 +190,34 @@
   hipLaunchKernelGGL(sa_fin_in_fwd_kernel, dim3(sa_div_up(B * C, 256)), dim3(256), 0,
                      reinterpret_cast<hipStream_t>(stream), sums, B * C, C, (float)n, gamma, beta,
                      eps, mean, rstd, scale, shift);
+  hipError_t e = hipGetLastError();
+  return e == hipSuccess ? 0 : -(int)e;
+}
+
+__global__ __launch_bounds__(32 * SA_SP_LANES) void sa_in_fwd_fused_kernel(
+    const float* __restrict__ slabs, int nslab, int C, float n, const float* __restrict__ gamma,
+    const float* __restrict__ beta, float eps, float* mean, float* rstd, float* scale, float* shift) {
+  __shared__ double part[SA_SP_LANES][33];
+  __shared__ double tot[32];
+  const int bb = blockIdx.y, o = threadIdx.x & 31, q = threadIdx.x >> 5;
+  const double t = sa_sp_column_total(slabs, nslab, 2 * C, bb, blockIdx.x * 32 + o, o, q, part);
+  if (q == 0) tot[o] = t;
+  __syncthreads();
+  const int c = blockIdx.x * 16 + threadIdx.x;
+  if (threadIdx.x < 16 && c < C) {
+    const int i = bb * C + c;
+    sa_in_fwd_coef(tot[2 * threadIdx.x], tot[2 * threadIdx.x + 1], n, gamma[c], beta[c], eps, mean[i], rstd[i],
+                   scale[i], shift[i]);
+  }
+}
+
+extern "C" int sa_in_fwd_fused(const float* stats, int B, int nslab, int C, int n, const float* gamma,
+                               const float* beta, float eps, float* mean, float* rstd, float* scale,
+                               float* shift, void* stream) {
+  if (!stats || !gamma || !beta || !mean || !rstd || !scale || !shift || B <= 0 || nslab <= 0 || C <= 0) return -22;
+  hipLaunchKernelGGL(sa_in_fwd_fused_kernel, dim3(sa_div_up(2 * C, 32), B), dim3(32 * SA_SP_LANES), 0,
+                     reinterpret_cast<hipStream_t>(stream), stats, nslab, C, (float)n, gamma, beta, eps, mean,
+                     rstd, scale, shift);
   hipError_t e = hipGetLastError();
   return e == hipSuccess ? 0 : -(int)e;
 }
@@ -238,6 +278,14 @@
   return e == hipSuccess ? 0 : -(int)e;
 }
 
+__device__ __forceinline__ void sa_norm_bwd_coef(double S1, double S2, double r, double m, float g, double n,
+                                                 float sign, float& c1, float& c2, float& c3) {
+  const double k1 = (double)g * r;
+  c1 = sign * (float)k1;
+  c2 = sign * (float)(-k1 * r * S2 / n);
+  c3 = sign * (float)(k1 * (-S1 / n + m * r * S2 / n));
+}
+
 __global__ void sa_fin_norm_bwd_kernel(const double* __restrict__ sums, const double* __restrict__ lsums,
                                        int R, int G, int C, double n, const float* __restrict__ gamma,
                                        const float* __restrict__ mean, const float* __restrict__ rstd,
@@ -251,34 +299,12 @@
       double S1 = 0.0, S2 = 0.0;
 #pragma unroll 8
       for (int r = 0; r < R; ++r) { S1 += sums[2 * ((size_t)r * G + i)]; S2 += sums[2 * ((size_t)r * G + i) + 1]; }
-      const double r = rstd[i], m = mean[i];
-      const double k1 = (double)gamma[i % C] * r;
-      c1[i] = sign * (float)k1;
-      c2[i] = sign * (float)(-k1 * r * S2 / n);
-      c3[i] = sign * (float)(k1 * (-S1 / n + m * r * S2 / n));
+      sa_norm_bwd_coef(S1, S2, rstd[i], mean[i], gamma[i % C], n, sign, c1[i], c2[i], c3[i]);
     }
     return;
   }
   __shared__ double part[8][32][2];
-  const int ch = ((int)blockIdx.x - coef_blocks) * 32 + (threadIdx.x & 31), q = threadIdx.x >> 5;
-  double a = 0.0, bsum = 0.0;
-  if (ch < C) {
-    const int tot = R * nb;
-#pragma unroll 4
-    for (int e = q; e < tot; e += 8) {
-      const int r = e / nb, b = e % nb;
-      const size_t at = 2 * ((size_t)r * G + (size_t)b * C + ch);
-      bsum += lsums[at]; a += lsums[at + 1];
-    }
-  }
-  part[q][threadIdx.x & 31][0] = bsum; part[q][threadIdx.x & 31][1] = a;
-  __syncthreads();
-  if (q == 0 && ch < C) {
-    double s0 = 0.0, s1 = 0.0;
-#pragma unroll
-    for (int k = 0; k < 8; ++k) { s0 += part[k][threadIdx.x][0]; s1 += part[k][threadIdx.x][1]; }
-    dbeta[ch] = (float)s0; dgamma[ch] = (float)s1;
-  }
+  sa_norm_dgdb_body(lsums, R, G, C, nb, (int)blockIdx.x - coef_blocks, dgamma, dbeta, part);
 }
 
 extern "C" int sa_fin_norm_bwd(const double* sums, const double* lsums, int R, int groups, int C, double n,
@@ -292,6 +318,36 @@
   hipLaunchKernelGGL(sa_fin_norm_bwd_kernel, dim3(grid), dim3(256), 0,
                      reinterpret_cast<hipStream_t>(stream), sums, lsums ? lsums : sums, R, groups, C,
                      n, gamma, mean, rstd, sign, c1, c2, c3, dgamma, dbeta, groups / C, coef_blocks, n_dev);
+  hipError_t e = hipGetLastError();
+  return e == hipSuccess ? 0 : -(int)e;
+}
+
+__global__ __launch_bounds__(32 * SA_SP_LANES) void sa_in_bwd_fused_kernel(
+    const float* __restrict__ slabs, int nslab, int C, double n, const float* __restrict__ gamma,
+    const float* __restrict__ mean, const float* __restrict__ rstd, float sign, float* c1, float* c2, float* c3,
+    double* __restrict__ sums) {
+  __shared__ double part[SA_SP_LANES][33];
+  __shared__ double tot[32];
+  const int bb = blockIdx.y, o = threadIdx.x & 31, q = threadIdx.x >> 5;
+  const double t = sa_sp_column_total(slabs, nslab, 2 * C, bb, blockIdx.x * 32 + o, o, q, part);
+  if (q == 0) tot[o] = t;
+  __syncthreads();
+  const int c = blockIdx.x * 16 + threadIdx.x;
+  if (threadIdx.x < 16 && c < C) {
+    const int i = bb * C + c;
+    const double T1 = tot[2 * threadIdx.x], T2 = tot[2 * threadIdx.x + 1];
+    sums[2 * (size_t)i] = T1; sums[2 * (size_t)i + 1] = T2;
+    sa_norm_bwd_coef(0.0 + T1, 0.0 + T2, rstd[i], mean[i], gamma[c], n, sign, c1[i], c2[i], c3[i]);
+  }
+}
+
+extern "C" int sa_in_bwd_fused(const float* stats, int B, int nslab, int C, double n, const float* gamma,
+                               const float* mean, const float* rstd, float sign, float* c1, float* c2, float* c3,
+                               double* sums, void* stream) {
+  if (!stats || !gamma || !mean || !rstd || !c1 || !c2 || !c3 || !sums || B <= 0 || nslab <= 0 || C <= 0) return -22;
+  hipLaunchKernelGGL(sa_in_bwd_fused_kernel, dim3(sa_div_up(2 * C, 32), B), dim3(32 * SA_SP_LANES), 0,
+                     reinterpret_cast<hipStream_t>(stream), stats, nslab, C, n, gamma, mean, rstd, sign, c1, c2, c3,
+                     sums);
   hipError_t e = hipGetLastError();
   return e == hipSuccess ? 0 : -(int)e;
 }
@@ -337,16 +393,10 @@
 }
 
 __global__ void sa_bias_multi_l2_kernel(SaBiasMulti m) {
-  const SaBiasDesc& d = m.d[blockIdx.y];
-  const int i = blockIdx.x * blockDim.x + threadIdx.x;
-  if (i >= d.C) return;
-  double s = 0.0;
-#pragma unroll 8
-  for (int b = 0; b < d.nbatch; ++b) s += d.rows[(size_t)b * d.C + i];
-  d.db[i] = (float)s;
-}
-
-extern "C" int sa_bias_multi(const SaBiasMulti* m, void* stream) {
+  sa_bias_l2_body(m.d[blockIdx.y], blockIdx.x * blockDim.x + threadIdx.x);
+}
+
+int sa_bias_multi_level1(const SaBiasMulti* m, hipStream_t st) {
   if (!m || m->n <= 0 || m->n > SA_BIAS_MAX) return -22;
   int maxC = 0, maxB = 0;
   for (int j = 0; j < m->n; ++j) {
@@ -355,8 +405,14 @@
     maxC = d.C > maxC ? d.C : maxC;
     maxB = d.nbatch > maxB ? d.nbatch : maxB;
   }
+  hipLaunchKernelGGL(sa_bias_multi_l1_kernel, dim3(sa_div_up(maxC, 32), maxB, m->n), dim3(32 * SA_SP_LANES), 0, st, *m);
+  return maxC;
+}
+
+extern "C" int sa_bias_multi(const SaBiasMulti* m, void* stream) {
   hipStream_t st = reinterpret_cast<hipStream_t>(stream);
-  hipLaunchKernelGGL(sa_bias_multi_l1_kernel, dim3(sa_div_up(maxC, 32), maxB, m->n), dim3(32 * SA_SP_LANES), 0, st, *m);
+  const int maxC = sa_bias_multi_level1(m, st);
+  if (maxC < 0) return maxC;
   hipLaunchKernelGGL(sa_bias_multi_l2_kernel, dim3(sa_div_up(maxC, 128), m->n), dim3(128), 0, st, *m);
   hipError_t e = hipGetLastError();
   return e == hipSuccess ? 0 : -(int)e;
diff --git a/speech-anonymization_amd/csrc/sa_small.hip b/speech-anonymization_amd/csrc/sa_small.hip
--- a/speech-anonymization_amd/csrc/sa_small.hip
+++ b/speech-anonymization_amd/csrc/sa_small.hip
@@ -468,20 +468,7 @@
                                                            float* __restrict__ dst, int nslab, int n,
                                                            int accumulate) {
   __shared__ double part[16][17];
-  const int o = threadIdx.x & 15, q = threadIdx.x >> 4, i = blockIdx.x * 16 + o;
-  double s = 0.0;
-  if (i < n) {
-#pragma unroll 4
-    for (int k = q; k < nslab; k += 16) s += (double)slabs[(size_t)k * n + i];
-  }
-  part[q][o] = s;
-  __syncthreads();
-  if (q == 0 && i < n) {
-    double t = 0.0;
-#pragma unroll
-    for (int r = 0; r < 16; ++r) t += part[r][o];
-    dst[i] = accumulate ? dst[i] + (float)t : (float)t;
-  }
+  sa_sum_slabs_body(slabs, dst, nslab, n, accumulate, blockIdx.x, part);
 }
 
 extern "C" int sa_sum_slabs(const float* slabs, float* dst, int nslab, int n, int accumulate,
diff --git a/speech-anonymization_amd/csrc/sa_wgrad.hip b/speech-anonymization_amd/csrc/sa_wgrad.hip
--- a/speech-anonymization_amd/csrc/sa_wgrad.hip
+++ b/speech-anonymization_amd/csrc/sa_wgrad.hip
@@ -600,6 +600,83 @@
   return e == hipSuccess ? 0 : -(int)e;
 }
 
+__global__ __launch_bounds__(256) void sa_stage_tail_kernel(SaBiasMulti bm, SaWredMulti wm, SaTailMisc tm) {
+  __shared__ double sm[3 * 64 * 4];
+  int j = blockIdx.y;
+  if (j < wm.n) {
+    const SaWredDesc& d = wm.d[j];
+    const int per = d.ntaps * d.cin * d.cout;
+    if ((int)blockIdx.x * 64 * d.vec >= per) return;
+    double (*part)[64 * 4] = reinterpret_cast<double (*)[64 * 4]>(sm);
+    if (d.vec == 4) wred_body<4>(d.slabs, d.dst, d.nslab, d.ntaps, d.cin, d.cout, d.sk, d.sn, d.st, d.accumulate, blockIdx.x, part);
+    else if (d.vec == 2) wred_body<2>(d.slabs, d.dst, d.nslab, d.ntaps, d.cin, d.cout, d.sk, d.sn, d.st, d.accumulate, blockIdx.x, part);
+    else wred_body<1>(d.slabs, d.dst, d.nslab, d.ntaps, d.cin, d.cout, d.sk, d.sn, d.st, d.accumulate, blockIdx.x, part);
+    return;
+  }
+  j -= wm.n;
+  if (j < tm.nslab) {
+    const SaTailSlab& d = tm.sl[j];
+    if ((int)blockIdx.x * 16 >= d.n) return;
+    sa_sum_slabs_body(d.slabs, d.dst, d.nslab, d.n, d.accumulate, blockIdx.x, reinterpret_cast<double (*)[17]>(sm));
+    return;
+  }
+  j -= tm.nslab;
+  if (j < tm.nin) {
+    const SaTailIn& d = tm.in[j];
+    if ((int)blockIdx.x * 32 >= d.C) return;
+    sa_norm_dgdb_body(d.sums, 1, d.B * d.C, d.C, d.B, blockIdx.x, d.dgamma, d.dbeta,
+                      reinterpret_cast<double (*)[32][2]>(sm));
+    return;
+  }
+  sa_bias_l2_body(bm.d[j - tm.nin], blockIdx.x * 256 + threadIdx.x);
+}
+
+extern "C" int sa_stage_tail_record_bytes(void) { return (int)sizeof(SaTailMisc); }
+
+extern "C" int sa_stage_tail(const SaBiasMulti* bias, const SaWredMulti* wred, const SaTailMisc* misc, void* stream) {
+  SaBiasMulti bm = {};
+  SaWredMulti wm = {};
+  SaTailMisc tm = {};
+  hipStream_t st = reinterpret_cast<hipStream_t>(stream);
+  int gx = 0;
+  if (wred && wred->n) {
+    if (wred->n < 0 || wred->n > SA_WRED_MAX) return -22;
+    wm = *wred;
+    for (int j = 0; j < wm.n; ++j) {
+      SaWredDesc& d = wm.d[j];
+      if (!d.slabs || !d.dst || d.nslab <= 0 || d.ntaps <= 0 || d.cin <= 0 || d.cout <= 0) return -22;
+      const int per = d.ntaps * d.cin * d.cout;
+      d.vec = wred_vec(per);
+      gx = std::max(gx, sa_div_up(per, 64 * d.vec));
+    }
+  }
+  if (misc) {
+    tm = *misc;
+    if (tm.nin < 0 || tm.nin > SA_TAIL_IN_MAX || tm.nslab < 0 || tm.nslab > SA_TAIL_SLAB_MAX) return -22;
+    for (int j = 0; j < tm.nin; ++j) {
+      const SaTailIn& d = tm.in[j];
+      if (!d.sums || !d.dgamma || !d.dbeta || d.B <= 0 || d.C <= 0) return -22;
+      gx = std::max(gx, sa_div_up(d.C, 32));
+    }
+    for (int j = 0; j < tm.nslab; ++j) {
+      const SaTailSlab& d = tm.sl[j];
+      if (!d.slabs || !d.dst || d.nslab <= 0 || d.n <= 0) return -22;
+      gx = std::max(gx, sa_div_up(d.n, 16));
+    }
+  }
+  if (bias && bias->n) {
+    const int maxC = sa_bias_multi_level1(bias, st);
+    if (maxC < 0) return maxC;
+    bm = *bias;
+    gx = std::max(gx, sa_div_up(maxC, 256));
+  }
+  const int jobs = bm.n + wm.n + tm.nin + tm.nslab;
+  if (jobs == 0) return -22;
+  hipLaunchKernelGGL(sa_stage_tail_kernel, dim3(gx, jobs), dim3(256), 0, st, bm, wm, tm);
+  hipError_t e = hipGetLastError();
+  return e == hipSuccess ? 0 : -(int)e;
+}
+
 extern "C" int sa_wgrad_reduce(const float* slabs, float* dst, int nslab, int ntaps, int cin,
                                int cout, int sk, int sn, int st, int accumulate, void* stream) {
   if (!slabs || !dst || nslab <= 0) return -22;
diff --git a/speech-anonymization_amd/ops.py b/speech-anonymization_amd/ops.py
--- a/speech-anonymization_amd/ops.py
+++ b/speech-anonymization_amd/ops.py
@@ -341,19 +341,22 @@
     return y
 
 
-def wgrad1C(u, v, dst, flip=False, s1=None, t1=None, swish=False, accumulate=False, chunk=2048):
+def wgrad1C(u, v, dst, flip=False, s1=None, t1=None, swish=False, accumulate=False, chunk=2048, defer=None):
     lib = L.load()
     B, Ln = u.shape
     nch = lib.sa_wgrad1C_nchunk(Ln, chunk)
     slabs = torch.empty(B * nch, 32 * 15, dtype=torch.float32, device=u.device)
     L.check(lib.sa_wgrad1C(L.dt_code(v.dtype), _f(u), _f(v), _f(slabs), B, Ln, chunk, int(flip),
                            _f(s1), _f(t1), int(swish), L.stream()), "sa_wgrad1C")
+    if defer is not None:
+        defer.append((slabs, dst, B * nch, 32 * 15, int(accumulate)))
+        return dst
     L.check(lib.sa_sum_slabs(_f(slabs), _f(dst), B * nch, 32 * 15, int(accumulate), L.stream()),
             "sa_sum_slabs")
     return dst
 
 
-def bwd1C(u, v, w, dst, s1, t1, mean, rstd, flip=True, accumulate=False, chunk=2048):
+def bwd1C(u, v, w, dst, s1, t1, mean, rstd, flip=True, accumulate=False, chunk=2048, defer=None):
     lib = L.load()
     B, Ln = u.shape
     nch = lib.sa_wgrad1C_nchunk(Ln, chunk)
@@ -362,6 +365,9 @@
     slabs = torch.empty(B * nch, 32 * 15, dtype=torch.float32, device=u.device)
     L.check(lib.sa_bwd1C(L.dt_code(v.dtype), _f(u), _f(v), _f(w), _f(g), _f(stats), _f(slabs), B, Ln, chunk,
                          int(flip), _f(s1), _f(t1), _f(mean), _f(rstd), L.stream()), "sa_bwd1C")
+    if defer is not None:
+        defer.append((slabs, dst, B * nch, 32 * 15, int(accumulate)))
+        return g, stats, dst
     L.check(lib.sa_sum_slabs(_f(slabs), _f(dst), B * nch, 32 * 15, int(accumulate), L.stream()),
             "sa_sum_slabs")
     return g, stats, dst
@@ -393,6 +399,63 @@
     L.check(lib.sa_fin_in_fwd(_f(sums), B, Cc, n, _f(gamma), _f(beta), C.c_float(eps), _f(o[0]),
                               _f(o[1]), _f(o[2]), _f(o[3]), L.stream()), "sa_fin_in_fwd")
     return o[0], o[1], o[2], o[3]
+
+
+def in_fwd_fused(stats, B, Cc, n, gamma, beta, eps=1e-5):
+    lib = L.load()
+    o = torch.empty(4, B, Cc, dtype=torch.float32, device=stats.device)
+    nslab = stats.numel() // (B * 2 * Cc)
+    assert nslab * B * 2 * Cc == stats.numel()
+    L.check(lib.sa_in_fwd_fused(_f(stats), B, nslab, Cc, n, _f(gamma), _f(beta), C.c_float(eps), _f(o[0]),
+                                _f(o[1]), _f(o[2]), _f(o[3]), L.stream()), "sa_in_fwd_fused")
+    return o[0], o[1], o[2], o[3]
+
+
+def in_bwd_fused(stats, B, Cc, n, gamma, mean, rstd, sign=1.0):
+    lib = L.load()
+    o = torch.empty(3, B * Cc, dtype=torch.float32, device=stats.device)
+    sums = torch.empty(B, 2 * Cc, dtype=torch.float64, device=stats.device)
+    nslab = stats.numel() // (B * 2 * Cc)
+    assert nslab * B * 2 * Cc == stats.numel()
+    L.check(lib.sa_in_bwd_fused(_f(stats), B, nslab, Cc, C.c_double(n), _f(gamma), _f(mean), _f(rstd),
+                                C.c_float(sign), _f(o[0]), _f(o[1]), _f(o[2]), _f(sums), L.stream()),
+            "sa_in_bwd_fused")
+    return (o[0], o[1], o[2]), sums
+
+
+def stage_tail(bias=(), wred=(), norms=(), slabs=()):
+    lib = L.load()
+    rows, rp = None, 0
+    if bias:
+        rows = torch.empty(sum(nb * cc for _, nb, cc, _, _ in bias), dtype=torch.float64, device=bias[0][0].device)
+        rp = rows.data_ptr()
+    i = 0
+    while (i * L.BIAS_MAX < len(bias) or i * L.WRED_MAX < len(wred) or i * L.TAIL_IN_MAX < len(norms)
+           or i * L.TAIL_SLAB_MAX < len(slabs)):
+        bm, wm, tm = L.SaBiasMulti(), L.SaWredMulti(), L.SaTailMisc()
+        chunk = bias[i * L.BIAS_MAX:(i + 1) * L.BIAS_MAX]
+        bm.n = len(chunk)
+        for d, (part, nb, cc, ncomp, db) in zip(bm.d, chunk):
+            d.part, d.rows, d.db = part.data_ptr(), rp, db.data_ptr()
+            d.nbatch, d.nslab, d.C, d.ncomp = nb, part.numel() // (nb * cc * ncomp), cc, ncomp
+            rp += nb * cc * 8
+        chunk = wred[i * L.WRED_MAX:(i + 1) * L.WRED_MAX]
+        wm.n = len(chunk)
+        for d, (sl, dst, nslab, nt, cin, cout, sk, sn, st, acc) in zip(wm.d, chunk):
+            d.slabs, d.dst = sl.data_ptr(), dst.data_ptr()
+            d.nslab, d.ntaps, d.cin, d.cout, d.sk, d.sn, d.st, d.accumulate = nslab, nt, cin, cout, sk, sn, st, acc
+        chunk = norms[i * L.TAIL_IN_MAX:(i + 1) * L.TAIL_IN_MAX]
+        tm.nin = len(chunk)
+        for d, (sums, nb, cc, dg, db) in zip(tm.in_, chunk):
+            assert sums.dtype == torch.float64 and sums.numel() == 2 * nb * cc
+            d.sums, d.dgamma, d.dbeta, d.B, d.C = sums.data_ptr(), dg.data_ptr(), db.data_ptr(), nb, cc
+        chunk = slabs[i * L.TAIL_SLAB_MAX:(i + 1) * L.TAIL_SLAB_MAX]
+        tm.nslab = len(chunk)
+        for d, (sl, dst, nslab, n, acc) in zip(tm.sl, chunk):
+            assert sl.numel() == nslab * n
+            d.slabs, d.dst, d.nslab, d.n, d.accumulate = sl.data_ptr(), dst.data_ptr(), nslab, n, acc
+        L.check(lib.sa_stage_tail(C.byref(bm), C.byref(wm), C.byref(tm), L.stream()), "sa_stage_tail")
+        i += 1
 
 
 def fin_bn_fwd(sums, Cc, count, gamma, beta, run_mean=None, run_var=None, eps=1e-5, momentum=0.1,
```

Measured after the change: 4.043 million frames/s (median of 4 runs). No clear change (+0.5%).
